# FerrisMind/candle-video

Measured on AMD Instinct MI355X. Metric: frames/sec end-to-end LTX-Video-2B 512x768x97; DiT step ms; VAE decode ms, higher is better.
Workload: dtype bf16; 1 GPU; LTX-Video-0.9.8-2B-distilled 512x768x97, 7 steps (configs.rs:223-240), untiled VAE decode; preset=0.9.8-2b-distilled, denoise_steps=7, parallelism=replicas x1 (no data-path collective)

## Files before the change

candle-video_amd/csrc/capi_ops.hip:

```cpp
#include "model_util.h"
#include "../../include/ltxhip_ops.h"

static inline int dtc(int d) { return d == 1 ? LTX_DT_BF16 : LTX_DT_F32; }

extern "C" int ltx_op_linear(const void* x, const void* w, const void* bias, void* y, int M, int N, int K, int dtype, int epi,
                             const void* resid, const float* gate, int rows_per_batch, ltx_stream stream) {
    if (!x || !w || !y) LTX_FAIL(LTX_ERR_ARG, "ltx_op_linear: null tensor");
    if (epi < 0 || epi > 3) LTX_FAIL(LTX_ERR_ARG, "ltx_op_linear: epi must be 0..3");
    if ((epi == 2 || epi == 3) && !resid) LTX_FAIL(LTX_ERR_ARG, "ltx_op_linear: residual epilogue needs resid");
    if (epi == 2 && (!gate || rows_per_batch < 1)) LTX_FAIL(LTX_ERR_ARG, "ltx_op_linear: gated epilogue needs gate");
    GemmArgs g; g.A = x; g.W = w; g.C = y; g.bias = bias; g.resid = resid; g.gate = gate;
    g.M = M; g.N = N; g.K = K; g.lda = K; g.ldc = N; g.ldr = N; g.rows_per_batch = rows_per_batch > 0 ? rows_per_batch : 1; g.gate_stride = N;
    return ltx_launch_gemm(g, dtc(dtype), epi, (hipStream_t)stream);
}

extern "C" int64_t ltx_op_ring_packed_bytes(int N, int K) { return (int64_t)ltx_ring_packed_bytes(N, K); }
extern "C" int ltx_op_ring_pack(const void* w, int N, int K, void* out, ltx_stream stream) { return ltx_pack_ring_weights(w, N, K, out, (hipStream_t)stream); }
extern "C" int ltx_op_linear_packed(const void* x, const void* w, const void* w_packed, const void* bias, void* y, int M, int N, int K, int epi,
                                    const void* resid, const float* gate, int rows_per_batch, ltx_stream stream) {
    if (!x || !w || !w_packed || !y) LTX_FAIL(LTX_ERR_ARG, "ltx_op_linear_packed: null tensor");
    if (epi < 0 || epi > 3) LTX_FAIL(LTX_ERR_ARG, "ltx_op_linear_packed: epi must be 0..3");
    if ((epi == 2 || epi == 3) && !resid) LTX_FAIL(LTX_ERR_ARG, "ltx_op_linear_packed: residual epilogue needs resid");
    if (epi == 2 && (!gate || rows_per_batch < 1)) LTX_FAIL(LTX_ERR_ARG, "ltx_op_linear_packed: gated epilogue needs gate");
    GemmArgs g; g.A = x; g.W = w; g.Wp = w_packed; g.C = y; g.bias = bias; g.resid = resid; g.gate = gate;
// ... 24 lines not shown
    return g;
}
GemmArgs fold_in_args(const void* x, const void* w, void* y, const float* rs_sq, int rs_n, int rs_D, float eps, const float* cvec, int cvec_stride,
                      int M, int N, int K, int rows_per_batch) {
    GemmArgs g; g.A = x; g.W = w; g.C = y; g.M = M; g.N = N; g.K = K; g.lda = K; g.ldc = N;
    g.rows_per_batch = rows_per_batch > 0 ? rows_per_batch : 1;
    g.rs_sq = rs_sq; g.rs_n = rs_n; g.rs_D = rs_D; g.rs_eps = eps; g.cvec = cvec; g.cvec_stride = cvec_stride;
    return g;
}
}

extern "C" int ltx_op_linear_fold_out(const void* x, const void* w, const void* bias, void* y, void* y2, float* rowsq, const float* scale2, int scale2_stride,
                                      int M, int N, int K, int epi, const void* resid, const float* gate, int rows_per_batch, ltx_stream stream) {
    if (!x || !w || !y || !y2 || !rowsq || !scale2 || !resid) LTX_FAIL(LTX_ERR_ARG, "ltx_op_linear_fold_out: null tensor");
    if (epi != 2 && epi != 3) LTX_FAIL(LTX_ERR_ARG, "ltx_op_linear_fold_out: epi must be 2 or 3 (the second output rides on the residual epilogues)");
    if (epi == 2 && !gate) LTX_FAIL(LTX_ERR_ARG, "ltx_op_linear_fold_out: gated epilogue needs gate");
    const GemmArgs g = fold_out_args(x, w, bias, y, y2, rowsq, scale2, scale2_stride, M, N, K, resid, gate, rows_per_batch);
    if (!ltx_gemm_fold_ok(g, epi)) LTX_FAIL(LTX_ERR_ARG, "ltx_op_linear_fold_out: not a call the norm fold serves (ltx_op_linear_fold_ok)");
    return ltx_launch_gemm(g, LTX_DT_BF16, epi, (hipStream_t)stream);
}

extern "C" int ltx_op_linear_fold_in(const void* x, const void* w, void* y, const float* rs_sq, int rs_n, int rs_D, float eps, const float* cvec, int cvec_stride,
                                     int M, int N, int K, int epi, int rows_per_batch, ltx_stream stream) {
    if (!x || !w || !y || !rs_sq || !cvec) LTX_FAIL(LTX_ERR_ARG, "ltx_op_linear_fold_in: null tensor");
    if (epi != 0 && epi != 1) LTX_FAIL(LTX_ERR_ARG, "ltx_op_linear_fold_in: epi must be 0 or 1 (the row scale rides on the bias / GELU epilogues)");
    const GemmArgs g = fold_in_args(x, w, y, rs_sq, rs_n, rs_D, eps, cvec, cvec_stride, M, N, K, rows_per_batch);
    if (!ltx_gemm_fold_ok(g, epi)) LTX_FAIL(LTX_ERR_ARG, "ltx_op_linear_fold_in: not a call the norm fold serves (ltx_op_linear_fold_ok)");
    return ltx_launch_gemm(g, LTX_DT_BF16, epi, (hipStream_t)stream);
}

extern "C" int ltx_op_linear_fold_ok(int M, int N, int K, int epi, int consumer, int rs_n, int vec_stride, int rows_per_batch) {
    if (M < 1 || N < 1 || K < 1) return 0;
    void* const p = reinterpret_cast<void*>((uintptr_t)4096); float* const f = reinterpret_cast<float*>(p);
    if (consumer) return ltx_gemm_fold_ok(fold_in_args(p, p, p, f, rs_n, K, 1e-6f, f, vec_stride, M, N, K, rows_per_batch), epi) ? 1 : 0;
    return ltx_gemm_fold_ok(fold_out_args(p, p, p, p, p, f, f, vec_stride, M, N, K, p, f, rows_per_batch), epi) ? 1 : 0;
}

extern "C" int ltx_op_shift_gemv(const void* w, const void* bias, const float* shift, int shift_stride, int B, int N, int K, float* cvec, int cvec_stride, ltx_stream stream) {
    return ltx_launch_shift_gemv(w, bias, shift, shift_stride, B, N, K, cvec, cvec_stride, (hipStream_t)stream);
}
extern "C" int ltx_op_mod_scale(const void* h, const float* scale, int scale_stride, void* y, int B, int64_t rows_per_batch, int D, int dtype, ltx_stream stream) {
    if (!h || !scale || !y || B < 1 || rows_per_batch < 1 || D < 1) LTX_FAIL(LTX_ERR_ARG, "ltx_op_mod_scale: bad argument");
    return ltx_launch_mod_scale(h, scale, scale_stride, y, B, rows_per_batch, D, dtc(dtype), (hipStream_t)stream);
}
extern "C" int ltx_op_scale_cols(const void* w, const float* scale, void* out, int64_t N, int K, int dtype, ltx_stream stream) {
    if (!w || !scale || !out || N < 1 || K < 1) LTX_FAIL(LTX_ERR_ARG, "ltx_op_scale_cols: bad argument");
    return ltx_launch_scale_cols(w, scale, out, N, K, dtc(dtype), (hipStream_t)stream);
}

extern "C" int ltx_op_linear_segmented(const void* x, const void* w, const void* bias, void* y, int M, int N, int K, int seg_width,
                                       int dtype, ltx_stream stream) {
    if (!x || !w || !y) LTX_FAIL(LTX_ERR_ARG, "ltx_op_linear_segmented: null tensor");
    if (seg_width <= 0 || (seg_width & (seg_width - 1)) || N % seg_width) LTX_FAIL(LTX_ERR_ARG, "ltx_op_linear_segmented: seg_width must be a power of two dividing N");
    GemmArgs g; g.A = x; g.W = w; g.C = y; g.bias = bias;
    g.M = M; g.N = N; g.K = K; g.lda = K; g.ldc = seg_width;
    g.c_seg_shift = __builtin_ctz((unsigned)seg_width); g.c_seg_stride = (int64_t)M * seg_width;
    return ltx_launch_gemm(g, dtc(dtype), EPI_BIAS, (hipStream_t)stream);
}

extern "C" int ltx_op_rownorm(const void* x, void* y, int64_t rows, int D, int kind, float eps, const void* weight,
                              const float* scale, const float* shift, int64_t rows_per_batch, int mod_stride, int act,
                              int dtype, ltx_stream stream) {
    if (!x || !y) LTX_FAIL(LTX_ERR_ARG, "ltx_op_rownorm: null tensor");
    RowNormArgs a; a.x = x; a.y = y; a.rows = rows; a.D = D; a.ldx = D; a.ldy = D; a.kind = kind; a.eps = eps; a.weight = weight;
    a.scale = scale; a.shift = shift; a.rows_per_batch = rows_per_batch > 0 ? rows_per_batch : 1; a.mod_stride = mod_stride; a.act = act;
    return ltx_launch_rownorm(a, dtc(dtype), (hipStream_t)stream);
}

extern "C" int ltx_attention_fallback_counts(unsigned long long counts[2], int reset) {
    if (!counts) LTX_FAIL(LTX_ERR_ARG, "ltx_attention_fallback_counts: null output");
    LTX_TRY(ltx_q64_fallback_read(&counts[0], reset));
    return ltx_q128_fallback_read(&counts[1], reset);
}

extern "C" int ltx_op_linear_split_factor(int M, int N, int K) {
    GemmArgs g; g.M = M; g.N = N; g.K = K; g.lda = K; g.ldc = N;
    return ltx_gemm_split_factor(g);
}
extern "C" int ltx_op_linear_deferred(const void* x, const void* w, float* parts, int M, int N, int K, ltx_stream stream) {
    if (!x || !w || !parts) LTX_FAIL(LTX_ERR_ARG, "ltx_op_linear_deferred: null tensor");
    GemmArgs g; g.A = x; g.W = w; g.C = parts; g.M = M; g.N = N; g.K = K; g.lda = K; g.ldc = N; g.defer_parts = parts;
    if (!ltx_gemm_defer_ok(g, EPI_GATE_RESID)) LTX_FAIL(LTX_ERR_ARG, "ltx_op_linear_deferred: bf16 linear layers of at most 512 rows, N % 8 == 0, K % 8 == 0");
    return ltx_launch_gemm(g, LTX_DT_BF16, EPI_BIAS, (hipStream_t)stream);
}
extern "C" int ltx_op_rownorm_deferred(const float* parts, int nparts, const void* bias, const void* resid, const float* gate, int gate_stride, void* h_out,
                                       void* y, int64_t rows, int D, int kind, float eps, const float* scale, const float* shift, int64_t rows_per_batch,
                                       int mod_stride, int dtype, ltx_stream stream) {
    if (!parts || !resid || !h_out || !y) LTX_FAIL(LTX_ERR_ARG, "ltx_op_rownorm_deferred: null tensor");
    RowNormArgs a; a.x = resid; a.y = y; a.rows = rows; a.D = D; a.ldx = D; a.ldy = D; a.kind = kind; a.eps = eps;
    a.scale = scale; a.shift = shift; a.rows_per_batch = rows_per_batch > 0 ? rows_per_batch : 1; a.mod_stride = mod_stride;
    a.parts = parts; a.nparts = nparts; a.part_stride = rows * D; a.d_bias = bias; a.d_gate = gate; a.d_gate_stride = gate_stride; a.x_out = h_out;
    return ltx_launch_rownorm(a, dtc(dtype), (hipStream_t)stream);
}

extern "C" int ltx_op_rownorm_presum(const void* x, void* y, int64_t rows, int D, float eps, const void* weight,
                                     const float* scale, const float* shift, int64_t rows_per_batch, int mod_stride, int act,
                                     const float* presum, int presum_n, int dtype, ltx_stream stream) {
    if (!x || !y || !presum) LTX_FAIL(LTX_ERR_ARG, "ltx_op_rownorm_presum: null tensor");
    RowNormArgs a; a.x = x; a.y = y; a.rows = rows; a.D = D; a.ldx = D; a.ldy = D; a.kind = 0; a.eps = eps; a.weight = weight;
    a.scale = scale; a.shift = shift; a.rows_per_batch = rows_per_batch > 0 ? rows_per_batch : 1; a.mod_stride = mod_stride; a.act = act;
    a.presum = presum; a.presum_n = presum_n;
    return ltx_launch_rownorm(a, dtc(dtype), (hipStream_t)stream);
}

extern "C" int ltx_op_timestep_embedding(const float* timesteps_host, int n, int vae_flavour, float multiplier, int dtype, void* out, ltx_stream stream) {
    if (!timesteps_host || !out) LTX_FAIL(LTX_ERR_ARG, "ltx_op_timestep_embedding: null argument");
    if (n < 1 || n > 8) LTX_FAIL(LTX_ERR_ARG, "ltx_op_timestep_embedding: batch must be 1..8");
    float tab[128]; ltx_sinusoid_table(vae_flavour, tab);
    float* dtab = nullptr;
    HIP_TRY(hipMalloc((void**)&dtab, sizeof(tab)));
    int rc = LTX_OK;
    if (hipMemcpy(dtab, tab, sizeof(tab), hipMemcpyHostToDevice) != hipSuccess) rc = LTX_ERR_HIP;
    if (rc == LTX_OK) {
        TimeVec tv; tv.n = n;
        for (int i = 0; i < n; ++i) tv.t[i] = timesteps_host[i];
        rc = ltx_launch_sinusoid(out, dtc(dtype), tv, dtab, 128, dtc(dtype) == LTX_DT_BF16, multiplier, (hipStream_t)stream);
        if (rc == LTX_OK && hipStreamSynchronize((hipStream_t)stream) != hipSuccess) rc = LTX_ERR_HIP;
    }
    (void)hipFree(dtab);
    return rc;
}

extern "C" int ltx_op_qknorm_rope(void* x, int64_t rows, int D, int ld, const void* weight, float eps,
                                  const float* cos, const float* sin, int dtype, ltx_stream stream) {
    if (!x || !weight) LTX_FAIL(LTX_ERR_ARG, "ltx_op_qknorm_rope: null tensor");
    QkNormRopeArgs a; a.x = x; a.rows = rows; a.D = D; a.ld = ld; a.nseg = 1; a.w0 = weight; a.eps = eps; a.cos = cos; a.sin = sin;
    return ltx_launch_qknorm_rope(a, dtc(dtype), (hipStream_t)stream);
}

extern "C" int ltx_op_rope_table(float* cos, float* sin, const float* coords, int B, int F, int H, int W, int D,
                                 const float* rope_scale_host, ltx_stream stream) {
    if (!cos || !sin) LTX_FAIL(LTX_ERR_ARG, "ltx_op_rope_table: null tensor");
    int steps = D / 6; if (steps < 1) steps = 1;
    std::vector<float> fr(steps);
    const float theta_ln = (float)std::log(10000.0);
    for (int i = 0; i < steps; ++i) {
        float lin = steps <= 1 ? 0.0f : (float)i * (float)(1.0 / (double)(steps - 1));
        fr[i] = (float)std::exp((double)(lin * theta_ln)) * (float)(M_PI / 2.0);
    }
    float* dfr = nullptr;
    HIP_TRY(hipMalloc((void**)&dfr, sizeof(float) * steps));
    HIP_TRY(hipMemcpy(dfr, fr.data(), sizeof(float) * steps, hipMemcpyHostToDevice));
    RopeTableArgs r; r.cos = cos; r.sin = sin; r.freqs = dfr; r.B = B; r.D = D;
    if (coords) { r.use_coords = 1; r.coords = coords; r.F = 1; r.H = 1; r.W = F * H * W;
                  r.gscale[0] = (float)(1.0 / 20.0); r.gscale[1] = (float)(1.0 / 2048.0); r.gscale[2] = (float)(1.0 / 2048.0); }
    else { r.F = F; r.H = H; r.W = W;
           if (rope_scale_host) { r.gscale[0] = (float)((double)rope_scale_host[0] / 20.0); r.gscale[1] = (float)((double)rope_scale_host[1] / 2048.0); r.gscale[2] = (float)((double)rope_scale_host[2] / 2048.0); } }
    int rc = ltx_launch_rope_table(r, (hipStream_t)stream);
    hipError_t e = hipStreamSynchronize((hipStream_t)stream);
    (void)hipFree(dfr);
    if (rc != LTX_OK) return rc;
    if (e != hipSuccess) { ltx_set_error(hipGetErrorString(e)); return LTX_ERR_HIP; }
    return LTX_OK;
}

extern "C" int ltx_op_attention(const void* q, const void* k, const void* v, void* o, int B, int Sq, int Sk, int heads, int hd,
                                int ldq, int ldk, int ldv, int ldo, float scale, const float* key_bias, int dtype, ltx_stream stream) {
    if (!q || !k || !v || !o) LTX_FAIL(LTX_ERR_ARG, "ltx_op_attention: null tensor");
    AttnArgs a; a.q = q; a.k = k; a.v = v; a.o = o; a.ldq = ldq; a.ldk = ldk; a.ldv = ldv; a.ldo = ldo;
    a.B = B; a.Sq = Sq; a.Sk = Sk; a.heads = heads; a.hd = hd; a.scale = scale; a.bias = key_bias;
    return ltx_launch_attention(a, dtc(dtype), (hipStream_t)stream);
}

extern "C" int ltx_op_attention_rowsq(const void* q, const void* k, const void* v, void* o, int B, int Sq, int Sk, int heads, int hd,
                                      int ldq, int ldk, int ldv, int ldo, float scale, const float* key_bias,
                                      const float* q_rowsq, int q_rowsq_n, int q_rowsq_D, float q_rowsq_eps, ltx_stream stream) {
    if (!q || !k || !v || !o || !q_rowsq) LTX_FAIL(LTX_ERR_ARG, "ltx_op_attention_rowsq: null tensor");
    AttnArgs a; a.q = q; a.k = k; a.v = v; a.o = o; a.ldq = ldq; a.ldk = ldk; a.ldv = ldv; a.ldo = ldo;
    a.B = B; a.Sq = Sq; a.Sk = Sk; a.heads = heads; a.hd = hd; a.scale = scale; a.bias = key_bias;
    a.q_rowsq = q_rowsq; a.q_rowsq_n = q_rowsq_n; a.q_rowsq_D = q_rowsq_D; a.q_rowsq_eps = q_rowsq_eps;
    return ltx_launch_attention(a, LTX_DT_BF16, (hipStream_t)stream);
}

extern "C" int ltx_op_attention_compact(const void* q, const void* k, const void* v, void* o, int B, int Sq, int Sk, int heads, int hd,
                                        int ldq, int ldk, int ldv, int ldo, float scale, const float* key_bias,
                                        const float* q_rowsq, int q_rowsq_n, int q_rowsq_D, float q_rowsq_eps, int* counts_out, ltx_stream stream) {
    if (!q || !k || !v || !o || !key_bias) LTX_FAIL(LTX_ERR_ARG, "ltx_op_attention_compact: null tensor");
    if (!ltx_attention_cross64_ok(hd, Sk) || B < 1 || ldk != heads * hd || ldv != heads * hd) LTX_FAIL(LTX_ERR_ARG, "ltx_op_attention_compact: bf16, head_dim 64, at most 128 keys, dense k / v rows");
    hipStream_t s = (hipStream_t)stream;
    const int D = heads * hd;
    void *kc = nullptr, *vc = nullptr, *bc = nullptr, *idx = nullptr, *cnt = nullptr;
    auto free_all = [&]() { for (void* p : {kc, vc, bc, idx, cnt}) if (p) (void)hipFree(p); };
    const size_t rows = (size_t)B * Sk;
    if (hipMalloc(&kc, rows * D * 2) != hipSuccess || hipMalloc(&vc, rows * D * 2) != hipSuccess || hipMalloc(&bc, rows * 4) != hipSuccess ||
        hipMalloc(&idx, rows * 4) != hipSuccess || hipMalloc(&cnt, (size_t)B * 4) != hipSuccess) { free_all(); LTX_FAIL(LTX_ERR_HIP, "hipMalloc"); }
    int rc = ltx_launch_key_compact(key_bias, B, Sk, (int*)idx, (int*)cnt, (float*)bc, s);
    if (rc == LTX_OK) rc = ltx_launch_gather_rows(k, kc, (const int*)idx, (const int*)cnt, 1, B, Sk, D * 2, s);
    if (rc == LTX_OK) rc = ltx_launch_gather_rows(v, vc, (const int*)idx, (const int*)cnt, 1, B, Sk, D * 2, s);
    if (rc == LTX_OK) {
        AttnArgs a; a.q = q; a.k = kc; a.v = vc; a.o = o; a.ldq = ldq; a.ldk = D; a.ldv = D; a.ldo = ldo;
        a.B = B; a.Sq = Sq; a.Sk = Sk; a.heads = heads; a.hd = hd; a.scale = scale; a.bias = (const float*)bc; a.k_count = (const int*)cnt;
        if (q_rowsq) { a.q_rowsq = q_rowsq; a.q_rowsq_n = q_rowsq_n; a.q_rowsq_D = q_rowsq_D; a.q_rowsq_eps = q_rowsq_eps; }
        rc = ltx_launch_attention(a, LTX_DT_BF16, s);
    }
    if (rc == LTX_OK && counts_out && hipMemcpyAsync(counts_out, cnt, (size_t)B * 4, hipMemcpyDeviceToDevice, s) != hipSuccess) rc = LTX_ERR_HIP;
    const hipError_t e = hipStreamSynchronize(s);
    free_all();
    if (rc != LTX_OK) return rc;
    if (e != hipSuccess) { ltx_set_error(hipGetErrorString(e)); return LTX_ERR_HIP; }
    return LTX_OK;
}

extern "C" int ltx_op_attention_prescaled(const void* q, const void* k, const void* v, void* o, int B, int Sq, int Sk, int heads, int hd,
                                          int ldq, int ldk, int ldv, int ldo, ltx_stream stream) {
    if (!q || !k || !v || !o) LTX_FAIL(LTX_ERR_ARG, "ltx_op_attention_prescaled: null tensor");
    AttnArgs a; a.q = q; a.k = k; a.v = v; a.o = o; a.ldq = ldq; a.ldk = ldk; a.ldv = ldv; a.ldo = ldo;
    a.B = B; a.Sq = Sq; a.Sk = Sk; a.heads = heads; a.hd = hd; a.scale = 1.0f; a.q_prescaled = 1;
    return ltx_launch_attention(a, LTX_DT_BF16, (hipStream_t)stream);
}

namespace {
int conv_common(const void* x, const void* w, const void* bias, int wdtype, void* y, const void* resid,
                int B, int T, int H, int W, int Cin, int Cout, int causal, int dtype, int epi, int mode, int post, hipStream_t s) {
    if (!x || !w || !bias || !y) LTX_FAIL(LTX_ERR_ARG, "conv: null tensor");
    const int dt = dtc(dtype); const size_t esz = ltx_dt_size(dt);
    void *pw = nullptr, *pb = nullptr;
    HIP_TRY(hipMalloc(&pw, (size_t)Cout * Cin * 27 * esz));
    if (hipMalloc(&pb, (size_t)Cout * esz + 16) != hipSuccess) { (void)hipFree(pw); LTX_FAIL(LTX_ERR_HIP, "hipMalloc"); }
    const int Cf = Cout / 8;
    int rc = ltx_pack_conv(w, dtc(wdtype), pw, dt, Cout, Cin, 27, mode, Cf, s);
    if (rc == LTX_OK) rc = ltx_pack_conv(bias, dtc(wdtype), pb, dt, Cout, 1, 1, mode, Cf, s);
    if (rc == LTX_OK) {
        GemmArgs g; g.A = x; g.W = pw; g.C = y; g.bias = pb; g.resid = resid;
        g.M = B * T * H * W; g.N = Cout; g.K = Cin; g.ldc = Cout; g.ldr = Cout;
        g.conv = 1; g.B = B; g.T = T; g.H = H; g.Wd = W; g.Cin = Cin; g.ntaps = 27; g.kh = 3; g.kw = 3; g.pad_t = causal ? 2 : 1; g.post = post;
        if (epi == EPI_D2S) { g.Cf = Cf; g.Cr = Cin / 8; g.To = 2 * T - 1; g.Ho = 2 * H; g.Wo = 2 * W; }
        rc = ltx_launch_gemm(g, dt, epi, s);
    }
    hipError_t e = hipStreamSynchronize(s);
    (void)hipFree(pw); (void)hipFree(pb);
    if (rc != LTX_OK) return rc;
    if (e != hipSuccess) { ltx_set_error(hipGetErrorString(e)); return LTX_ERR_HIP; }
    return LTX_OK;
}
}

extern "C" int ltx_op_conv3d(const void* x, const void* w, const void* bias, int wdtype, void* y, const void* resid,
                             int B, int T, int H, int W, int Cin, int Cout, int causal, int dtype, ltx_stream stream) {
    return conv_common(x, w, bias, wdtype, y, resid, B, T, H, W, Cin, Cout, causal, dtype, resid ? EPI_RESID : EPI_BIAS, LTX_PERM_NONE, 0, (hipStream_t)stream);
}
extern "C" int ltx_op_upsample3d(const void* x, const void* w, const void* bias, int wdtype, void* y,
                                 int B, int T, int H, int W, int Cin, int Cout, int causal, int residual, int dtype, ltx_stream stream) {
    if (Cout % 8 != 0 || Cin % 8 != 0) LTX_FAIL(LTX_ERR_ARG, "upsample3d: channels must be multiples of 8");
    return conv_common(x, w, bias, wdtype, y, residual ? x : nullptr, B, T, H, W, Cin, Cout, causal, dtype, EPI_D2S, LTX_PERM_D2S, 0, (hipStream_t)stream);
}
extern "C" int ltx_op_conv_out_unpatchify(const void* x, const void* w, const void* bias, int wdtype, float* y,
                                          int B, int T, int H, int W, int Cin, int Cout, int causal, int postprocess, int dtype, ltx_stream stream) {
    if (Cout % 16 != 0) LTX_FAIL(LTX_ERR_ARG, "conv_out: Cout must be a multiple of 16 (patch 4x4)");
    return conv_common(x, w, bias, wdtype, y, nullptr, B, T, H, W, Cin, Cout, causal, dtype, EPI_UNPATCH, LTX_PERM_UNPATCH, postprocess, (hipStream_t)stream);
}

extern "C" int ltx_op_blend(const float* a, float* b, int BC, int at, int ah, int aw, int bt, int bh, int bw, int dim, int blend_extent, ltx_stream stream) {
    if (!a || !b || dim < 2 || dim > 4) LTX_FAIL(LTX_ERR_ARG, "ltx_op_blend: bad argument");
    const int ad[3] = {at, ah, aw}, bd[3] = {bt, bh, bw};
    BlendArgs ba; ba.a = a; ba.b = b; ba.dst = b; ba.BC = BC;
    ba.at = at; ba.ah = ah; ba.aw = aw; ba.a_len = ad[dim - 2];
    ba.bt = ba.dt = bt; ba.bh = ba.dh = bh; ba.bw = ba.dw = bw;
    ba.dim = dim; ba.blend = std::min(blend_extent, std::min(ad[dim - 2], bd[dim - 2]));
    ba.et = std::min(at, bt); ba.eh = std::min(ah, bh); ba.ew = std::min(aw, bw);
    if (dim == 2) ba.et = ba.blend; else if (dim == 3) ba.eh = ba.blend; else ba.ew = ba.blend;
    return ltx_launch_blend(ba, (hipStream_t)stream);
}

const char* ltx_gemm_plan_name(int M, int N, int K, int conv, int ntaps, int T, int H, int W);
extern "C" int ltx_op_gemm_plan(int M, int N, int K, int conv, int ntaps, int T, int H, int W, char* name, int cap) {
    if (!name || cap < 1) LTX_FAIL(LTX_ERR_ARG, "ltx_op_gemm_plan: bad argument");
    const char* n = ltx_gemm_plan_name(M, N, K, conv, ntaps, T, H, W);
    snprintf(name, (size_t)cap, "%s", n);
    return LTX_OK;
}

extern "C" int ltx_op_gemm_route(int M, int N, int K, int conv, int ntaps, int B, int T, int H, int W, int epi, int dtype, int flags, char* name, int cap) {
    if (!name || cap < 1 || M < 1 || N < 1 || K < 1 || epi < EPI_BIAS || epi > EPI_S2D) LTX_FAIL(LTX_ERR_ARG, "ltx_op_gemm_route: bad argument");
    if (conv && (ntaps < 1 || B < 1 || T < 1 || H < 1 || W < 1 || (int64_t)B * T * H * W != M)) LTX_FAIL(LTX_ERR_ARG, "ltx_op_gemm_route: conv calls need M = B T H W");
    void* const p = reinterpret_cast<void*>((uintptr_t)4096); float* const f = reinterpret_cast<float*>(p);
    const bool res = epi == EPI_GATE_RESID || epi == EPI_RESID;
    GemmArgs g;
    if (flags & LTX_ROUTE_FOLD_IN) g = fold_in_args(p, p, p, f, 16, K, 1e-6f, f, N, M, N, K, M);
    else if (flags & LTX_ROUTE_FOLD_OUT) g = fold_out_args(p, p, p, p, p, f, f, N, M, N, K, p, epi == EPI_GATE_RESID ? f : nullptr, M);
    else {
        g.A = p; g.W = p; g.C = p; g.M = M; g.N = N; g.K = K; g.lda = K; g.ldc = N; g.ldr = N; g.rows_per_batch = M; g.gate_stride = N;
        if (flags & LTX_ROUTE_DEFER) g.defer_parts = f;
        else { g.bias = p; if (res || epi == EPI_S2D) g.resid = p; if (epi == EPI_GATE_RESID) g.gate = f; }
    }
    if (conv) {
        g.conv = 1; g.B = B; g.T = T; g.H = H; g.Wd = W; g.Cin = K; g.ntaps = ntaps; g.kh = g.kw = ntaps == 27 ? 3 : 1; g.pad_t = 2;
        if (epi == EPI_D2S) { g.Cf = N / 8; g.Cr = K / 8; g.To = 2 * T - 1; g.Ho = 2 * H; g.Wo = 2 * W; }
        if (epi == EPI_S2D) { g.s2_st = g.s2_sh = g.s2_sw = 2; g.To = (T + 1) / 2; g.Ho = H / 2; g.Wo = W / 2; }
        if (flags & LTX_ROUTE_PN) { g.pn_on = 1; g.pn_eps = 1e-6f; g.pn_act = 1; }
    }
    GemmRoute r;
    LTX_TRY(ltx_gemm_route(g, dtc(dtype), epi, nullptr, false, &r));
    if (const char* why = ltx_gemm_route_refusal(g, r)) LTX_FAIL(LTX_ERR_ARG, why);
    snprintf(name, (size_t)cap, "%s", ltx_gemm_route_name(r));
    return LTX_OK;
}

extern "C" int ltx_op_dit_plan(int heads, int head_dim, int model_dtype, int io_dtype, int B, int S, int K, int G, int skip_mask, int64_t* out) {
    if (!out || heads < 1 || head_dim < 1 || B < 1 || B > 8 || S < 1 || K < 1 || G < 1 || S % G != 0) LTX_FAIL(LTX_ERR_ARG, "ltx_op_dit_plan: bad argument");
    ltx_dit_config c; ltx_dit_config_default(&c);
    c.num_attention_heads = heads; c.attention_head_dim = head_dim; c.cross_attention_dim = heads * head_dim;
    const DitPlan p = ltx_dit_plan(c, dtc(model_dtype), dtc(io_dtype), B, S, K, G, skip_mask != 0);
    const int64_t v[LTX_DIT_PLAN_FIELDS] = {p.M, p.MK, p.NB, p.Sg, p.seg, p.ldqkv, p.fold_q2, p.presum, p.nfold, p.defer_ff2, p.ff2_parts, p.dense_qkv, p.fold_q};
    for (int i = 0; i < LTX_DIT_PLAN_FIELDS; ++i) out[i] = v[i];
    return LTX_OK;
}
// ... 1 lines not shown
```

candle-video_amd/csrc/dit.hip:

```cpp
#include <cstring>
#include <deque>
#include "model_util.h"
#include "options.h"
#include "../../include/ltxhip_cond.h"
#include "lora.h"

struct DitBlock {
    LinearW qkv1, o1, q2, kv2, o2, ff1, ff2;
    void *nq1 = nullptr, *nk1 = nullptr, *nq2 = nullptr, *nk2 = nullptr;
};

struct DitCtx {
    const void* enc = nullptr; const float* mask = nullptr;
    int B = 0, K = 0, iodt = 0; bool valid = false;
    bool fold_q2 = false;
    DevBuf kv, bias;
    bool compact = false;
    DevBuf kvc, biasc, kidx, kcount;
    void release() { kv.release(); bias.release(); kvc.release(); biasc.release(); kidx.release(); kcount.release(); valid = false; }
};

struct DitTimeEntry {
    float t[8] = {0}; int B = 0; hipStream_t stream = nullptr; bool valid = false; uint64_t used = 0;
    DevBuf ada, adaf;
    DevBuf cfold; bool cfold_valid = false;
    void release() { ada.release(); adaf.release(); cfold.release(); valid = cfold_valid = false; }
};
struct DitWfold {
    float t = 0.f; hipStream_t stream = nullptr; bool valid = false; uint64_t used = 0; DevBuf w;
    void release() { w.release(); valid = false; }
};
constexpr int kDitTimeEntries = 64;
struct DitGroupEntry {
    std::vector<float> t; int B = 0, G = 0; hipStream_t stream = nullptr; bool valid = false; uint64_t used = 0;
    DevBuf ada, adaf, cfold; bool cfold_valid = false;
    void release() { ada.release(); adaf.release(); cfold.release(); valid = cfold_valid = false; }
};
constexpr int kDitGroupEntries = 8;

struct ltx_dit {
    ltx_dit_config cfg{};
    int dtype = LTX_DT_BF16;
    int device = 0;
    int D = 0;
    LinearW proj_in, te1, te2, te_lin, cap1, cap2, proj_out;
    void* sst_final = nullptr;
    void* sst_blocks = nullptr;
    std::vector<DitBlock> blocks;
    float* rope_freqs = nullptr;
    float* inv_freq = nullptr;
    std::vector<int> skip_blocks;
    std::deque<DitCtx> ctxs;
    bool ctx_mode = false;
    std::deque<DitTimeEntry> tcache; uint64_t tclock = 0;
    std::deque<DitWfold> wcache;
    std::deque<DitGroupEntry> gcache;
    bool wfold_off = false;
    struct { bool valid = false; const float* coords = nullptr; float rs[3] = {0, 0, 0}; bool has_rs = false; int B = 0, S = 0, F = 0, H = 0, W = 0; hipStream_t stream = nullptr; } rope_key;
    void invalidate_weight_derived() {
        for (auto& e : wcache) e.valid = false;
        for (auto& e : ctxs) e.valid = false;
        for (auto& e : tcache) e.cfold_valid = false;
        for (auto& e : gcache) e.cfold_valid = false;
    }
    void release_scaled_weights() { for (auto& e : wcache) e.release(); }
    void release_caches() { auto all = [](auto& c) { for (auto& e : c) e.release(); c.clear(); }; all(ctxs); all(tcache); all(wcache); all(gcache); }
    std::vector<void*> owned;
    struct LoraSlots { void* base[7] = {nullptr}; void* merged[7] = {nullptr}; };
    std::vector<LoraSlots> lora_w;
    int n_adapters = 0;
    DevBuf xin, encin, h, n, qkv, attn, ff, c1, encp, kv2, tproj, e1, emb, embs, temb, ada, adaf, cosb, sinb, bias, orig, orig_hsq, outT, rsq, hsq, parts;
    void free_all() {
        for (void* p : owned) if (p) (void)hipFree(p);
        owned.clear();
        for (auto& ls : lora_w) for (void*& p : ls.merged) if (p) { (void)hipFree(p); p = nullptr; }
        lora_w.clear();
        DevBuf* bs[] = {&xin, &encin, &h, &n, &qkv, &attn, &ff, &c1, &encp, &kv2, &tproj, &e1, &emb, &embs, &temb, &ada, &adaf, &cosb, &sinb, &bias, &orig, &orig_hsq, &outT, &rsq, &hsq, &parts};
        for (DevBuf* b : bs) b->release();
        release_caches();
    }
};

namespace {

int own_linear(ltx_dit* m, const WeightMap& wm, const std::string& prefix, int in, int out, LinearW* l) {
    LTX_TRY(ltx_load_linear(wm, prefix, in, out, m->dtype, l));
    m->owned.push_back(l->w); if (l->b) m->owned.push_back(l->b);
    return LTX_OK;
}
int own_tensor(ltx_dit* m, const WeightMap& wm, const std::string& name, int64_t numel, void** out) {
    LTX_TRY(ltx_load_tensor(wm, name, numel, m->dtype, out));
    m->owned.push_back(*out);
    return LTX_OK;
}
int own_fused(ltx_dit* m, const WeightMap& wm, const std::vector<std::string>& prefixes, int in, int out_each, LinearW* l) {
    const int n = (int)prefixes.size();
    const size_t esz = ltx_dt_size(m->dtype);
    l->in = in; l->out = out_each * n;
    HIP_TRY(hipMalloc(&l->w, (size_t)l->out * in * esz)); m->owned.push_back(l->w);
    bool has_bias = wm.find(prefixes[0] + ".bias") != nullptr;
    if (has_bias) { HIP_TRY(hipMalloc(&l->b, (size_t)l->out * esz)); m->owned.push_back(l->b); }
    for (int i = 0; i < n; ++i) {
        const ltx_weight* w = wm.find(prefixes[i] + ".weight");
        if (!w) LTX_FAIL(LTX_ERR_MISSING_WEIGHT, "missing weight '" + prefixes[i] + ".weight'");
        LTX_TRY(ltx_upload_cast(w, (char*)l->w + (size_t)i * out_each * in * esz, m->dtype, (int64_t)out_each * in, prefixes[i] + ".weight"));
        if (has_bias) {
            const ltx_weight* b = wm.find(prefixes[i] + ".bias");
            if (!b) LTX_FAIL(LTX_ERR_MISSING_WEIGHT, "missing weight '" + prefixes[i] + ".bias'");
            LTX_TRY(ltx_upload_cast(b, (char*)l->b + (size_t)i * out_each * esz, m->dtype, out_each, prefixes[i] + ".bias"));
        }
    }
    return LTX_OK;
}

int build(ltx_dit* m, const ltx_weight* weights, size_t n_weights) {
    const ltx_dit_config& c = m->cfg;
    const int D = m->D, L = c.num_layers;
    WeightMap wm(weights, n_weights);
    LTX_TRY(own_linear(m, wm, "proj_in", c.in_channels, D, &m->proj_in));
    LTX_TRY(own_tensor(m, wm, "scale_shift_table", 2 * (int64_t)D, &m->sst_final));
    LTX_TRY(own_linear(m, wm, "time_embed.emb.timestep_embedder.linear_1", 256, D, &m->te1));
    LTX_TRY(own_linear(m, wm, "time_embed.emb.timestep_embedder.linear_2", D, D, &m->te2));
    LTX_TRY(own_linear(m, wm, "time_embed.linear", D, 6 * D, &m->te_lin));
    LTX_TRY(own_linear(m, wm, "caption_projection.linear_1", c.caption_channels, D, &m->cap1));
    LTX_TRY(own_linear(m, wm, "caption_projection.linear_2", D, D, &m->cap2));
    LTX_TRY(own_linear(m, wm, "proj_out", D, c.out_channels, &m->proj_out));
    const size_t esz = ltx_dt_size(m->dtype);
    HIP_TRY(hipMalloc(&m->sst_blocks, (size_t)L * 6 * D * esz)); m->owned.push_back(m->sst_blocks);
    m->blocks.resize(L);
    for (int i = 0; i < L; ++i) {
        const std::string p = "transformer_blocks." + std::to_string(i) + ".";
        DitBlock& b = m->blocks[i];
        LTX_TRY(own_fused(m, wm, {p + "attn1.to_q", p + "attn1.to_k", p + "attn1.to_v"}, D, D, &b.qkv1));
        LTX_TRY(own_linear(m, wm, p + "attn1.to_out.0", D, D, &b.o1));
        LTX_TRY(own_tensor(m, wm, p + "attn1.norm_q.weight", D, &b.nq1));
        LTX_TRY(own_tensor(m, wm, p + "attn1.norm_k.weight", D, &b.nk1));
        LTX_TRY(own_linear(m, wm, p + "attn2.to_q", D, D, &b.q2));
        LTX_TRY(own_fused(m, wm, {p + "attn2.to_k", p + "attn2.to_v"}, c.cross_attention_dim, D, &b.kv2));
        LTX_TRY(own_linear(m, wm, p + "attn2.to_out.0", D, D, &b.o2));
        LTX_TRY(own_tensor(m, wm, p + "attn2.norm_q.weight", D, &b.nq2));
        LTX_TRY(own_tensor(m, wm, p + "attn2.norm_k.weight", D, &b.nk2));
        LTX_TRY(own_linear(m, wm, p + "ff.net.0.proj", D, 4 * D, &b.ff1));
        LTX_TRY(own_linear(m, wm, p + "ff.net.2", 4 * D, D, &b.ff2));
        const ltx_weight* t = wm.find(p + "scale_shift_table");
        if (!t) LTX_FAIL(LTX_ERR_MISSING_WEIGHT, "missing weight '" + p + "scale_shift_table'");
        LTX_TRY(ltx_upload_cast(t, (char*)m->sst_blocks + (size_t)i * 6 * D * esz, m->dtype, 6 * (int64_t)D, p + "scale_shift_table"));
    }
    {
        int steps = D / 6; if (steps < 1) steps = 1;
        std::vector<float> fr(steps);
        const float theta_ln = (float)std::log(10000.0);
        for (int i = 0; i < steps; ++i) {
            float lin = steps <= 1 ? 0.0f : (float)i * (float)(1.0 / (double)(steps - 1));
            float x = lin * theta_ln;
            float e = (float)std::exp((double)x);
            fr[i] = e * (float)(M_PI / 2.0);
        }
        HIP_TRY(hipMalloc((void**)&m->rope_freqs, sizeof(float) * steps)); m->owned.push_back(m->rope_freqs);
        HIP_TRY(hipMemcpy(m->rope_freqs, fr.data(), sizeof(float) * steps, hipMemcpyHostToDevice));
        std::vector<float> inv(128);
        ltx_sinusoid_table(0, inv.data());
        HIP_TRY(hipMalloc((void**)&m->inv_freq, sizeof(float) * 128)); m->owned.push_back(m->inv_freq);
        HIP_TRY(hipMemcpy(m->inv_freq, inv.data(), sizeof(float) * 128, hipMemcpyHostToDevice));
    }
    return LTX_OK;
}

LinearW* dit_slot(DitBlock& b, int slot) {
    LinearW* const ws[7] = {&b.qkv1, &b.o1, &b.q2, &b.kv2, &b.o2, &b.ff1, &b.ff2};
    return ws[slot];
}
constexpr int kLoraSlot[kLoraLinears] = {0, 0, 0, 1, 2, 3, 3, 4, 5, 6}, kLoraPart[kLoraLinears] = {0, 1, 2, 0, 0, 0, 1, 0, 0, 0};
constexpr int kSlotParts[7] = {3, 1, 1, 2, 1, 1, 1}, kSlotFirst[7] = {0, 3, 4, 5, 7, 8, 9};

}

extern "C" int ltx_dit_create(const ltx_dit_config* cfg, const ltx_weight* weights, size_t n_weights,
                              ltx_dtype model_dtype, int device, ltx_dit** out) {
    if (!cfg || !weights || !out) LTX_FAIL(LTX_ERR_ARG, "ltx_dit_create: null argument");
    *out = nullptr;
    const int hd = cfg->attention_head_dim;
    if (hd != 16 && hd != 32 && hd != 64 && hd != 128) LTX_FAIL(LTX_ERR_UNSUPPORTED, "attention_head_dim must be 16/32/64/128");
    const int D = cfg->num_attention_heads * hd;
    if (D % 8 != 0 || cfg->in_channels % 8 != 0 || cfg->out_channels % 8 != 0 || cfg->caption_channels % 8 != 0 || cfg->cross_attention_dim % 8 != 0)
        LTX_FAIL(LTX_ERR_UNSUPPORTED, "channel dims must be multiples of 8");
    if (cfg->cross_attention_dim != D) LTX_FAIL(LTX_ERR_UNSUPPORTED, "cross_attention_dim must equal inner_dim (caption projection output feeds attn2)");
    if (cfg->num_layers < 1) LTX_FAIL(LTX_ERR_ARG, "num_layers must be >= 1");
    HIP_TRY(hipSetDevice(device));
    ltx_dit* m = new ltx_dit();
    m->cfg = *cfg; m->dtype = model_dtype == LTX_BF16 ? LTX_DT_BF16 : LTX_DT_F32; m->device = device; m->D = D;
    int rc = build(m, weights, n_weights);
    if (rc == LTX_OK && cfg->attention_head_dim == 128 && m->dtype == LTX_DT_BF16) rc = ltx_attention_q128_prepare();
    if (rc != LTX_OK) { m->free_all(); delete m; return rc; }
    m->lora_w.resize(m->blocks.size());
    for (size_t l = 0; l < m->blocks.size(); ++l)
        for (int slot = 0; slot < 7; ++slot) m->lora_w[l].base[slot] = dit_slot(m->blocks[l], slot)->w;
    *out = m;
    return LTX_OK;
}

extern "C" void ltx_dit_destroy(ltx_dit* m) {
    if (!m) return;
    (void)hipSetDevice(m->device);
    (void)hipDeviceSynchronize();
    m->free_all();
    delete m;
}

extern "C" int ltx_dit_set_skip_blocks(ltx_dit* m, const int* blocks, int n) {
    if (!m || n < 0 || (n > 0 && !blocks)) LTX_FAIL(LTX_ERR_ARG, "ltx_dit_set_skip_blocks: bad argument");
    m->skip_blocks.assign(blocks, blocks + n);
    return LTX_OK;
}

extern "C" int ltx_dit_get_config(const ltx_dit* m, ltx_dit_config* out) {
    if (!m || !out) LTX_FAIL(LTX_ERR_ARG, "ltx_dit_get_config: null argument");
    *out = m->cfg;
    return LTX_OK;
}

namespace {
enum DitForm { kPass,
               kFold1,
               kFold2,
               kDefer };
struct DitOperands {
    void *h, *n, *qkv, *attn, *ff; float *rsq, *hsq, *parts;
    const float* ada;
    const float* ada_next;
    const float* cfold;
// ... 72 lines not shown

namespace {
template <class E, class Match>
E* cache_slot(std::deque<E>& c, size_t cap, Match match, bool* hit) {
    E *found = nullptr, *lru = nullptr;
    for (auto& e : c) if (e.valid && match(e)) found = &e;
    if ((*hit = found != nullptr)) return found;
    for (auto& e : c) if (!e.valid) return &e;
    if (c.size() < cap) { c.emplace_back(); return &c.back(); }
    for (auto& e : c) if (!lru || e.used < lru->used) lru = &e;
    return lru;
}
struct DitTables { const float *ada = nullptr, *adaf = nullptr, *cfold = nullptr; };
int time_tables(ltx_dit* m, const DitPlan& p, const float* vals, int nv, hipStream_t s, DitTables* t) {
    const int D = p.D, L = m->cfg.num_layers, dt = p.dt;
    TimeVec tv; tv.n = nv; for (int i = 0; i < 8; ++i) tv.t[i] = i < nv ? vals[i] : 0.f;
    bool hit;
    DitTimeEntry* te = cache_slot(m->tcache, kDitTimeEntries, [&](const DitTimeEntry& e) { return e.B == nv && e.stream == s && !memcmp(e.t, tv.t, sizeof(float) * nv); }, &hit);
    if (!hit) {
        te->valid = false; te->cfold_valid = false;
        LTX_TRY(te->ada.ensure((size_t)L * nv * 6 * D * sizeof(float))); LTX_TRY(te->adaf.ensure((size_t)2 * nv * D * sizeof(float)));
        LTX_TRY(ltx_launch_sinusoid(m->tproj.p, dt, tv, m->inv_freq, 128, dt == LTX_DT_BF16, 1.0f, s));
        LTX_TRY(ltx_linear(m->te1, m->tproj.p, 256, m->e1.p, D, nv, dt, EPI_BIAS, s));
        LTX_TRY(ltx_launch_silu(m->e1.p, m->e1.p, (int64_t)nv * D, dt, s));
        LTX_TRY(ltx_linear(m->te2, m->e1.p, D, m->emb.p, D, nv, dt, EPI_BIAS, s));
        LTX_TRY(ltx_launch_silu(m->emb.p, m->embs.p, (int64_t)nv * D, dt, s));
        LTX_TRY(ltx_linear(m->te_lin, m->embs.p, D, m->temb.p, 6 * D, nv, dt, EPI_BIAS, s));
        LTX_TRY(ltx_launch_ada(te->ada.as<float>(), m->sst_blocks, m->temb.p, L, nv, 6 * D, dt, s));
        LTX_TRY(ltx_launch_ada(te->adaf.as<float>(), m->sst_final, m->emb.p, 2, nv, D, dt, s));
        memcpy(te->t, tv.t, sizeof(te->t)); te->B = nv; te->stream = s; te->valid = true;
    }
    te->used = ++m->tclock;
    if (p.nfold && !te->cfold_valid) {
        LTX_TRY(te->cfold.ensure((size_t)L * nv * 7 * D * sizeof(float)));
        for (int l = 0; l < L; ++l) {
            const float* ada = te->ada.as<float>() + (size_t)l * nv * 6 * D;
            float* cq = te->cfold.as<float>() + (size_t)l * nv * 7 * D;
            LTX_TRY(ltx_launch_shift_gemv(m->blocks[l].qkv1.w, m->blocks[l].qkv1.b, ada, 6 * D, nv, 3 * D, D, cq, 3 * D, s));
            LTX_TRY(ltx_launch_shift_gemv(m->blocks[l].ff1.w, m->blocks[l].ff1.b, ada + 3 * D, 6 * D, nv, 4 * D, D, cq + (size_t)nv * 3 * D, 4 * D, s));
        }
        te->cfold_valid = true;
    }
    *t = DitTables{te->ada.as<float>(), te->adaf.as<float>(), p.nfold ? te->cfold.as<float>() : nullptr};
    return LTX_OK;
}
int group_tables(ltx_dit* m, const DitPlan& p, const float* timestep, hipStream_t s, DitTables* t) {
    const int D = p.D, L = m->cfg.num_layers, NB = p.NB, B = p.B, G = NB / B;
    bool hit;
    DitGroupEntry* ge = cache_slot(m->gcache, kDitGroupEntries, [&](const DitGroupEntry& e) { return e.B == B && e.G == G && e.stream == s && !memcmp(e.t.data(), timestep, sizeof(float) * NB); }, &hit);
    if (!hit && ge->valid && ge->stream != s) HIP_TRY(hipStreamSynchronize(ge->stream));
    if (!hit || (p.nfold && !ge->cfold_valid)) {
        ge->valid = false; ge->cfold_valid = false;
        std::vector<float> distinct; std::vector<int> idx((size_t)NB);
        for (int i = 0; i < NB; ++i) {
            size_t j = 0;
            while (j < distinct.size() && memcmp(&distinct[j], &timestep[i], sizeof(float)) != 0) ++j;
            if (j == distinct.size()) distinct.push_back(timestep[i]);
            idx[i] = (int)j;
        }
        LTX_TRY(ge->ada.ensure((size_t)L * NB * 6 * D * sizeof(float))); LTX_TRY(ge->adaf.ensure((size_t)2 * NB * D * sizeof(float)));
        if (p.nfold) LTX_TRY(ge->cfold.ensure((size_t)L * NB * 7 * D * sizeof(float)));
        const int nd = (int)distinct.size();
        for (int c0 = 0; c0 < nd; c0 += 8) {
            const int nc = nd - c0 < 8 ? nd - c0 : 8;
            DitTables te;
            LTX_TRY(time_tables(m, p, distinct.data() + c0, nc, s, &te));
            const int* gi = idx.data();
            LTX_TRY(ltx_launch_group_gather(ge->ada.as<float>(), (int64_t)NB * 6 * D, te.ada, (int64_t)nc * 6 * D, gi, c0, nc, L, NB, 6 * D, s));
            LTX_TRY(ltx_launch_group_gather(ge->adaf.as<float>(), (int64_t)NB * D, te.adaf, (int64_t)nc * D, gi, c0, nc, 2, NB, D, s));
            if (p.nfold) {
                LTX_TRY(ltx_launch_group_gather(ge->cfold.as<float>(), (int64_t)NB * 7 * D, te.cfold, (int64_t)nc * 7 * D, gi, c0, nc, L, NB, 3 * D, s));
                LTX_TRY(ltx_launch_group_gather(ge->cfold.as<float>() + (size_t)NB * 3 * D, (int64_t)NB * 7 * D, te.cfold + (size_t)nc * 3 * D, (int64_t)nc * 7 * D, gi, c0, nc, L, NB, 4 * D, s));
            }
        }
        ge->t.assign(timestep, timestep + NB); ge->B = B; ge->G = G; ge->stream = s; ge->valid = true; ge->cfold_valid = p.nfold;
    }
    ge->used = ++m->tclock;
    *t = DitTables{ge->ada.as<float>(), ge->adaf.as<float>(), p.nfold ? ge->cfold.as<float>() : nullptr};
    return LTX_OK;
}
int give_up_scaled_weights(ltx_dit* m, hipStream_t s) {
    m->wfold_off = true;
    HIP_TRY(hipStreamSynchronize(s));
    m->release_scaled_weights();
    return LTX_OK;
}
int scaled_weights(ltx_dit* m, const DitPlan& p, const float* timestep, const float* ada_all, hipStream_t s, const DitWfold** out) {
    *out = nullptr;
    bool wf = p.NB == p.B && p.nfold && ltx_opt().norm_fold == 2 && !m->wfold_off;
    for (int i = 1; i < p.B; ++i) wf = wf && timestep[i] == timestep[0];
    if (!wf) return LTX_OK;
    const int D = p.D, L = m->cfg.num_layers, cap = ltx_opt().norm_fold_copies > 0 ? ltx_opt().norm_fold_copies : 1;
    const size_t esz = ltx_dt_size(p.dt), per_layer = (size_t)7 * D * D * esz;
    const float t0 = timestep[0];
    bool hit;
    DitWfold* we = cache_slot(m->wcache, (size_t)cap, [&](const DitWfold& e) { return e.t == t0 && e.stream == s; }, &hit);
    if (!hit) {
        if (we->valid) {
            if (m->tclock - we->used < (uint64_t)4 * cap) return give_up_scaled_weights(m, s);
            if (we->stream != s) HIP_TRY(hipStreamSynchronize(we->stream));
            we->valid = false;
        }
        if (we->w.ensure((size_t)L * per_layer) != LTX_OK) {
            (void)hipGetLastError();
            return give_up_scaled_weights(m, s);
        }
        for (int l = 0; l < L; ++l) {
            const float* ada = ada_all + (size_t)l * p.NB * 6 * D;
            char* wl = (char*)we->w.p + (size_t)l * per_layer;
            LTX_TRY(ltx_launch_scale_cols(m->blocks[l].qkv1.w, ada + D, wl, 3 * D, D, p.dt, s));
            LTX_TRY(ltx_launch_scale_cols(m->blocks[l].ff1.w, ada + 4 * D, wl + (size_t)3 * D * D * esz, 4 * D, D, p.dt, s));
        }
        we->t = t0; we->stream = s; we->valid = true;
    }
    we->used = m->tclock;
    *out = we;
    return LTX_OK;
}
int text_context(ltx_dit* m, const DitPlan& p, const void* enc, const float* enc_mask, hipStream_t s, DitCtx** out) {
    const ltx_dit_config& c = m->cfg;
    const int D = p.D, L = c.num_layers, dt = p.dt, B = p.B, K = p.K;
    const int64_t MK = p.MK; const size_t esz = ltx_dt_size(dt);
    DitCtx* ctx = nullptr;
    for (auto& e : m->ctxs) if (e.valid && e.enc == enc && e.mask == enc_mask && e.B == B && e.K == K && e.iodt == p.iodt && e.fold_q2 == p.fold_q2) ctx = &e;
    *out = ctx;
    if (ctx) return LTX_OK;
    if (m->ctxs.size() >= 4 || !m->ctx_mode) { for (auto& e : m->ctxs) e.valid = false; }
    for (auto& e : m->ctxs) if (!e.valid) { ctx = &e; break; }
    if (!ctx) { m->ctxs.emplace_back(); ctx = &m->ctxs.back(); }
    ctx->enc = enc; ctx->mask = enc_mask; ctx->B = B; ctx->K = K; ctx->iodt = p.iodt; ctx->fold_q2 = p.fold_q2;
    LTX_TRY(ctx->kv.ensure((size_t)L * MK * 2 * D * esz)); LTX_TRY(ctx->bias.ensure(MK * sizeof(float)));
    LTX_TRY(ltx_launch_cast(enc, p.iodt, m->encin.p, dt, MK * c.caption_channels, s));
    LTX_TRY(ltx_linear(m->cap1, m->encin.p, c.caption_channels, m->c1.p, D, (int)MK, dt, EPI_GELU, s));
    LTX_TRY(ltx_linear(m->cap2, m->c1.p, D, m->encp.p, D, (int)MK, dt, EPI_BIAS, s));
    if (enc_mask) LTX_TRY(ltx_launch_mask_bias(ctx->bias.as<float>(), enc_mask, MK, s));
    for (int l = 0; l < L; ++l) {
        void* kvl = (char*)ctx->kv.p + (size_t)l * MK * 2 * D * esz;
        LTX_TRY(ltx_linear(m->blocks[l].kv2, m->encp.p, D, kvl, 2 * D, (int)MK, dt, EPI_BIAS, s));
        QkNormRopeArgs k2; k2.x = kvl; k2.rows = MK; k2.D = D; k2.ld = 2 * D; k2.nseg = 1; k2.w0 = m->blocks[l].nk2; k2.eps = 1e-5f;
        if (p.fold_q2) k2.w0b = m->blocks[l].nq2;
        LTX_TRY(ltx_launch_qknorm_rope(k2, dt, s));
    }
    ctx->compact = enc_mask && dt == LTX_DT_BF16 && ltx_attention_cross64_ok(c.attention_head_dim, K) && ltx_opt().xattn_compact;
    if (ctx->compact) {
        LTX_TRY(ctx->kvc.ensure((size_t)L * MK * 2 * D * esz)); LTX_TRY(ctx->biasc.ensure(MK * sizeof(float)));
        LTX_TRY(ctx->kidx.ensure(MK * sizeof(int))); LTX_TRY(ctx->kcount.ensure((size_t)B * sizeof(int)));
        LTX_TRY(ltx_launch_key_compact(ctx->bias.as<float>(), B, K, ctx->kidx.as<int>(), ctx->kcount.as<int>(), ctx->biasc.as<float>(), s));
        LTX_TRY(ltx_launch_gather_rows(ctx->kv.p, ctx->kvc.p, ctx->kidx.as<int>(), ctx->kcount.as<int>(), L, B, K, (int)(2 * D * esz), s));
    }
    ctx->valid = true;
    *out = ctx;
    return LTX_OK;
}
int rope_tables(ltx_dit* m, const DitPlan& p, int num_frames, int height, int width, const float* rope_scale, const float* video_coords, hipStream_t s) {
    const ltx_dit_config& c = m->cfg;
    auto& rk = m->rope_key;
    const bool same = m->ctx_mode && rk.valid && rk.coords == video_coords && rk.B == p.B && rk.S == p.S && rk.F == num_frames && rk.H == height && rk.W == width &&
                      rk.stream == s && rk.has_rs == (rope_scale != nullptr) && (!rope_scale || !memcmp(rk.rs, rope_scale, sizeof(rk.rs)));
    if (same) return LTX_OK;
    rk.valid = false;
    RopeTableArgs r;
    r.cos = m->cosb.as<float>(); r.sin = m->sinb.as<float>(); r.freqs = m->rope_freqs;
    r.B = p.B; r.D = p.D;
    if (video_coords) {
        r.use_coords = 1; r.coords = video_coords; r.F = 1; r.H = 1; r.W = p.S;
        r.gscale[0] = (float)(1.0 / 20.0); r.gscale[1] = (float)(1.0 / 2048.0); r.gscale[2] = (float)(1.0 / 2048.0);
    } else {
        r.F = num_frames; r.H = height; r.W = width;
        if (rope_scale) {
            r.gscale[0] = (float)((double)rope_scale[0] * c.patch_size_t / 20.0);
            r.gscale[1] = (float)((double)rope_scale[1] * c.patch_size / 2048.0);
            r.gscale[2] = (float)((double)rope_scale[2] * c.patch_size / 2048.0);
        }
    }
    LTX_TRY(ltx_launch_rope_table(r, s));
    rk.coords = video_coords; rk.B = p.B; rk.S = p.S; rk.F = num_frames; rk.H = height; rk.W = width; rk.stream = s;
    rk.has_rs = rope_scale != nullptr; if (rope_scale) memcpy(rk.rs, rope_scale, sizeof(rk.rs));
    rk.valid = m->ctx_mode;
    return LTX_OK;
}

struct DitCarry {
    bool hsq_valid = false;
    bool hs_valid = false;
    bool hsq_saved = false;
    bool pending = false; const float* pend_gate = nullptr; const void* pend_bias = nullptr;
    void take_pending(RowNormArgs& rn, const ltx_dit* m, const DitPlan& p) {
        if (!pending) return;
        rn.parts = m->parts.as<float>(); rn.nparts = p.ff2_parts; rn.part_stride = p.M * p.D; rn.d_bias = pend_bias; rn.d_gate = pend_gate; rn.d_gate_stride = 6 * p.D;
        rn.x_out = m->h.p; pending = false;
    }
};
struct DitLayerIn { DitTables tab; const DitWfold* we = nullptr; const DitCtx* ctx = nullptr; const float* skip_layer_mask = nullptr; };
bool block_runs(const ltx_dit* m, const float* skip_layer_mask, int B, int l) {
    for (int sb : m->skip_blocks) if (sb == l) return false;
    bool all = skip_layer_mask != nullptr;
    for (int b = 0; all && b < B; ++b) all = skip_layer_mask[(size_t)l * B + b] == 1.f;
    return !all;
}
int next_block(const ltx_dit* m, const float* skip_layer_mask, int B, int l) {
    for (int n = l + 1; n < m->cfg.num_layers; ++n) if (block_runs(m, skip_layer_mask, B, n)) return n;
    return -1;
}

int dit_block(ltx_dit* m, const DitPlan& p, int l, const DitLayerIn& in, DitCarry& st, hipStream_t s) {
    const ltx_dit_config& c = m->cfg;
    const int dt = p.dt, D = p.D, B = p.B, S = p.S, NB = p.NB, H = c.num_attention_heads, hd = c.attention_head_dim;
    const int64_t M = p.M; const size_t esz = ltx_dt_size(dt);
    const bool wf = in.we != nullptr, fold_out = p.nfold && !wf;
    const DitBlock& b = m->blocks[l];
    TimeVec mv; mv.n = B; bool any = false;
    for (int i = 0; i < 8; ++i) mv.t[i] = 0.f;
    if (in.skip_layer_mask) for (int bb = 0; bb < B; ++bb) { mv.t[bb] = in.skip_layer_mask[(size_t)l * B + bb]; any |= mv.t[bb] != 0.f; }
    if (any) {
        HIP_TRY(hipMemcpyAsync(m->orig.p, m->h.p, M * D * esz, hipMemcpyDeviceToDevice, s));
        st.hsq_saved = p.presum && st.hsq_valid;
        if (st.hsq_saved) { LTX_TRY(m->orig_hsq.ensure(M * (D / 128) * sizeof(float))); HIP_TRY(hipMemcpyAsync(m->orig_hsq.p, m->hsq.p, M * (D / 128) * sizeof(float), hipMemcpyDeviceToDevice, s)); }
    }
    const int ln = fold_out ? next_block(m, in.skip_layer_mask, B, l) : -1;
    const float* ada = in.tab.ada + (size_t)l * NB * 6 * D;
    DitOperands x{m->h.p, m->n.p, m->qkv.p, m->attn.p, m->ff.p, m->rsq.as<float>(), m->hsq.as<float>(), m->parts.as<float>(), ada,
                  ln >= 0 ? in.tab.ada + (size_t)ln * NB * 6 * D : nullptr, p.nfold ? in.tab.cfold + (size_t)l * NB * 7 * D : nullptr,
                  wf ? (const char*)in.we->w.p + (size_t)l * 7 * D * D * esz : nullptr, c.norm_eps};
    const DitForm fold_in_form = wf ? kFold2 : kFold1;
    RowNormArgs rn; rn.x = m->h.p; rn.y = m->n.p; rn.rows = M; rn.D = D; rn.ldx = D; rn.ldy = D;
    rn.kind = 0; rn.eps = c.norm_eps; rn.shift = ada; rn.scale = ada + D; rn.rows_per_batch = p.Sg; rn.mod_stride = 6 * D;
    if (p.presum && st.hsq_valid) { rn.presum = m->hsq.as<float>(); rn.presum_n = D / 128; }
    const bool fold1 = p.nfold && st.hsq_valid && (wf || st.hs_valid);
    if (!fold1) { st.take_pending(rn, m, p); LTX_TRY(ltx_launch_rownorm(rn, dt, s)); }
    st.hs_valid = false;
    rn.parts = nullptr; rn.nparts = 0; rn.x_out = nullptr; rn.d_bias = nullptr; rn.d_gate = nullptr;
    LTX_TRY(ltx_launch_gemm(gemm_qkv1(p, fold1 ? fold_in_form : kPass, b, x), dt, EPI_BIAS, s));
    const float attn_scale = 1.0f / std::sqrt((float)hd);
    QkNormRopeArgs qa; qa.x = m->qkv.p; qa.rows = M; qa.D = D; qa.ld = p.ldqkv; qa.seg_stride = p.seg; qa.nseg = 2; qa.w0 = b.nq1; qa.w1 = b.nk1;
    qa.eps = 1e-5f; qa.cos = m->cosb.as<float>(); qa.sin = m->sinb.as<float>();
    if (p.fold_q) qa.out_scale0 = attn_scale * 1.4426950408889634f;
    LTX_TRY(ltx_launch_qknorm_rope(qa, dt, s));
    AttnArgs at; at.q = m->qkv.p; at.k = (char*)m->qkv.p + (size_t)p.seg * esz; at.v = (char*)m->qkv.p + (size_t)2 * p.seg * esz; at.o = m->attn.p;
    at.ldq = at.ldk = at.ldv = p.ldqkv; at.ldo = D; at.B = B; at.Sq = S; at.Sk = S; at.heads = H; at.hd = hd; at.scale = attn_scale;
    at.q_prescaled = p.fold_q ? 1 : 0;
    LTX_TRY(ltx_launch_attention(at, dt, s));
    LTX_TRY(ltx_linear(b.o1, m->attn.p, D, m->h.p, D, (int)M, dt, EPI_GATE_RESID, s, m->h.p, D, ada + 2 * D, 6 * D, p.Sg));
    st.hsq_valid = false;
    const DitCtx* ctx = in.ctx;
    const char* kvl = (const char*)(ctx->compact ? ctx->kvc.p : ctx->kv.p) + (size_t)l * p.MK * 2 * D * esz;
    AttnArgs ax; ax.q = m->qkv.p; ax.k = kvl; ax.v = kvl + (size_t)D * esz; ax.o = m->attn.p;
    ax.ldq = D; ax.ldk = ax.ldv = 2 * D; ax.ldo = D; ax.B = B; ax.Sq = S; ax.Sk = p.K; ax.heads = H; ax.hd = hd; ax.scale = attn_scale;
    ax.bias = ctx->mask ? ctx->bias.as<float>() : nullptr;
    if (ctx->compact) { ax.bias = ctx->biasc.as<float>(); ax.k_count = ctx->kcount.as<int>(); }
    if (p.fold_q2) {
        LTX_TRY(ltx_launch_gemm(gemm_q2(p, b, x), dt, EPI_BIAS, s));
        ax.q_rowsq = m->rsq.as<float>(); ax.q_rowsq_n = D / 128; ax.q_rowsq_D = D; ax.q_rowsq_eps = 1e-5f;
    } else {
        LTX_TRY(linear_of(b.q2, gemm_q2(p, b, x), dt, EPI_BIAS, s));
        QkNormRopeArgs q2; q2.x = m->qkv.p; q2.rows = M; q2.D = D; q2.ld = D; q2.nseg = 1; q2.w0 = b.nq2; q2.eps = 1e-5f;
        LTX_TRY(ltx_launch_qknorm_rope(q2, dt, s));
    }
    LTX_TRY(ltx_launch_attention(ax, dt, s));
    if (fold_out) { LTX_TRY(ltx_launch_gemm(gemm_o2(p, kFold1, b, x), dt, EPI_RESID, s)); st.hs_valid = true; }
    else LTX_TRY(linear_of(b.o2, gemm_o2(p, kPass, b, x), dt, EPI_RESID, s));
    st.hsq_valid = p.presum;
    if (p.nfold && st.hsq_valid && (wf || st.hs_valid)) LTX_TRY(ltx_launch_gemm(gemm_ff1(p, fold_in_form, b, x), dt, EPI_GELU, s));
    else {
        rn.shift = ada + 3 * D; rn.scale = ada + 4 * D;
        rn.presum = nullptr; rn.presum_n = 0;
        if (p.presum && st.hsq_valid) { rn.presum = m->hsq.as<float>(); rn.presum_n = D / 128; }
        LTX_TRY(ltx_launch_rownorm(rn, dt, s));
        LTX_TRY(linear_of(b.ff1, gemm_ff1(p, kPass, b, x), dt, EPI_GELU, s));
    }
    st.hs_valid = false;
    if (p.defer_ff2) {
        LTX_TRY(ltx_launch_gemm(gemm_ff2(p, kDefer, b, x), dt, EPI_BIAS, s));
        st.pending = true; st.pend_gate = ada + 5 * D; st.pend_bias = b.ff2.b;
    } else if (ln >= 0) { LTX_TRY(ltx_launch_gemm(gemm_ff2(p, kFold1, b, x), dt, EPI_GATE_RESID, s)); st.hs_valid = true; }
    else LTX_TRY(linear_of(b.ff2, gemm_ff2(p, kPass, b, x), dt, EPI_GATE_RESID, s));
    st.hsq_valid = p.presum;
    if (!any) return LTX_OK;
    LTX_TRY(ltx_launch_skip_blend(m->h.p, m->orig.p, mv, S, D, dt, s));
    bool binary = true;
    for (int bb = 0; bb < B; ++bb) binary &= mv.t[bb] == 0.f || mv.t[bb] == 1.f;
    if (st.hsq_valid && st.hsq_saved && binary) {
        const size_t rowb = (size_t)S * (D / 128) * sizeof(float);
        for (int bb = 0; bb < B; ++bb)
            if (mv.t[bb] == 1.f) HIP_TRY(hipMemcpyAsync((char*)m->hsq.p + bb * rowb, (const char*)m->orig_hsq.p + bb * rowb, rowb, hipMemcpyDeviceToDevice, s));
    } else st.hsq_valid = false;
    st.hs_valid = false;
    if (fold_out && st.hsq_valid && ln >= 0) { LTX_TRY(ltx_launch_mod_scale(m->h.p, x.ada_next + D, 6 * D, m->n.p, NB, p.Sg, D, dt, s)); st.hs_valid = true; }
    return LTX_OK;
}

int dit_forward_b8(ltx_dit* m, const void* hidden, const void* enc, const float* timestep, int G,
                   const float* enc_mask, int B, int S, int K, int num_frames, int height, int width,
                   const float* rope_scale, const float* video_coords, const float* skip_layer_mask,
                   ltx_dtype io_dtype, void* out, ltx_stream stream) {
    if (B < 1 || B > 8) LTX_FAIL(LTX_ERR_ARG, "ltx_dit_forward: internal batch chunk must be 1..8");
    if (S < 1 || K < 1) LTX_FAIL(LTX_ERR_ARG, "ltx_dit_forward: empty sequence");
    if (!video_coords && (int64_t)num_frames * height * width != S)
        LTX_FAIL(LTX_ERR_ARG, "ltx_dit_forward: num_frames*height*width must equal S when video_coords is absent");
    HIP_TRY(hipSetDevice(m->device));
    if (G < 1 || S % G != 0) LTX_FAIL(LTX_ERR_ARG, "ltx_dit_forward: the modulation groups must divide the sequence");
    hipStream_t s = (hipStream_t)stream;
    const ltx_dit_config& c = m->cfg;
    const DitPlan p = ltx_dit_plan(c, m->dtype, io_dtype == LTX_BF16 ? LTX_DT_BF16 : LTX_DT_F32, B, S, K, G, skip_layer_mask != nullptr);
    const int dt = p.dt, D = p.D, L = c.num_layers;
    const int64_t M = p.M, MK = p.MK; const size_t esz = ltx_dt_size(dt);
    const size_t nte = p.NB == p.B ? (size_t)p.B : 8;
    const size_t MD = M * D * esz, KD = MK * D * esz, part = M * (D / 128) * sizeof(float), rope = M * (D / 2) * sizeof(float);
    const std::pair<DevBuf*, size_t> ws[] = {
        {&m->xin, M * c.in_channels * esz}, {&m->encin, MK * c.caption_channels * esz}, {&m->h, MD}, {&m->n, MD}, {&m->qkv, 3 * MD}, {&m->attn, MD}, {&m->ff, 4 * MD},
        {&m->c1, KD}, {&m->encp, KD}, {&m->kv2, 2 * KD}, {&m->tproj, nte * 256 * esz}, {&m->e1, nte * D * esz}, {&m->emb, nte * D * esz}, {&m->embs, nte * D * esz},
        {&m->temb, nte * 6 * D * esz}, {&m->cosb, rope}, {&m->sinb, rope}, {&m->bias, MK * sizeof(float)}, {&m->outT, M * c.out_channels * esz},
        {&m->rsq, p.fold_q2 ? part : 0}, {&m->hsq, p.presum ? part : 0}, {&m->parts, p.defer_ff2 ? (size_t)p.ff2_parts * M * D * sizeof(float) : 0}, {&m->orig, skip_layer_mask ? MD : 0}};
    for (const auto& w : ws) LTX_TRY(w.first->ensure(w.second));

    LTX_TRY(ltx_launch_cast(hidden, p.iodt, m->xin.p, dt, p.M * c.in_channels, s));
    LTX_TRY(ltx_linear(m->proj_in, m->xin.p, c.in_channels, m->h.p, D, (int)p.M, dt, EPI_BIAS, s));

    DitLayerIn in; in.skip_layer_mask = skip_layer_mask;
    LTX_TRY(G == 1 ? time_tables(m, p, timestep, B, s, &in.tab) : group_tables(m, p, timestep, s, &in.tab));
    LTX_TRY(scaled_weights(m, p, timestep, in.tab.ada, s, &in.we));
    DitCtx* ctx = nullptr;
    LTX_TRY(text_context(m, p, enc, enc_mask, s, &ctx)); in.ctx = ctx;
    LTX_TRY(rope_tables(m, p, num_frames, height, width, rope_scale, video_coords, s));

    DitCarry st;
    for (int l = 0; l < L; ++l)
        if (block_runs(m, skip_layer_mask, B, l)) LTX_TRY(dit_block(m, p, l, in, st, s));

    RowNormArgs rn; rn.x = m->h.p; rn.y = m->n.p; rn.rows = p.M; rn.D = D; rn.ldx = D; rn.ldy = D;
    rn.kind = 1; rn.eps = 1e-6f; rn.shift = in.tab.adaf; rn.scale = in.tab.adaf + (size_t)p.NB * D;
    rn.rows_per_batch = p.Sg; rn.mod_stride = D;
    st.take_pending(rn, m, p);
    LTX_TRY(ltx_launch_rownorm(rn, dt, s));
    void* dst = p.iodt == dt ? out : m->outT.p;
    LTX_TRY(ltx_linear(m->proj_out, m->n.p, D, dst, c.out_channels, (int)p.M, dt, EPI_BIAS, s));
    if (p.iodt != dt) LTX_TRY(ltx_launch_cast(m->outT.p, dt, out, p.iodt, p.M * c.out_channels, s));
    if (!m->ctx_mode) ctx->valid = false;
    return LTX_OK;
}

int dit_forward_chunks(ltx_dit* m, const void* hidden, const void* enc, const float* timestep, int F,
                       const float* enc_mask, int B, int S, int K, int num_frames, int height, int width,
                       const float* rope_scale, const float* video_coords, const float* skip_layer_mask,
                       ltx_dtype io_dtype, void* out, ltx_stream stream) {
    const size_t esz = io_dtype == LTX_BF16 ? 2 : 4;
    const int L = m->cfg.num_layers;
    std::vector<float> mask_chunk;
    float t_row[8];
    for (int b0 = 0; b0 < B; b0 += 8) {
        const int bc = B - b0 < 8 ? B - b0 : 8;
        const float* slm = skip_layer_mask;
        if (skip_layer_mask && bc != B) {
            mask_chunk.resize((size_t)L * bc);
            for (int l = 0; l < L; ++l) for (int b = 0; b < bc; ++b) mask_chunk[(size_t)l * bc + b] = skip_layer_mask[(size_t)l * B + b0 + b];
            slm = mask_chunk.data();
        }
        const float* tc = timestep + (size_t)b0 * (F ? F : 1);
        int G = 1;
        if (F) {
            bool uniform = true;
            for (int b = 0; b < bc; ++b) for (int f = 1; f < F; ++f) uniform = uniform && memcmp(&tc[(size_t)b * F + f], &tc[(size_t)b * F], sizeof(float)) == 0;
            if (uniform) { for (int b = 0; b < bc; ++b) t_row[b] = tc[(size_t)b * F]; tc = t_row; } else G = F;
        }
        LTX_TRY(dit_forward_b8(m, (const char*)hidden + (size_t)b0 * S * m->cfg.in_channels * esz, (const char*)enc + (size_t)b0 * K * m->cfg.caption_channels * esz,
                               tc, G, enc_mask ? enc_mask + (size_t)b0 * K : nullptr, bc, S, K, num_frames, height, width, rope_scale,
                               video_coords ? video_coords + (size_t)b0 * S * 3 : nullptr, slm, io_dtype,
                               (char*)out + (size_t)b0 * S * m->cfg.out_channels * esz, stream));
    }
    return LTX_OK;
}

}

extern "C" int ltx_dit_forward(ltx_dit* m, const void* hidden, const void* enc, const float* timestep,
                               const float* enc_mask, int B, int S, int K, int num_frames, int height, int width,
                               const float* rope_scale, const float* video_coords, const float* skip_layer_mask,
                               ltx_dtype io_dtype, void* out, ltx_stream stream) {
    if (!m || !hidden || !enc || !timestep || !out) LTX_FAIL(LTX_ERR_ARG, "ltx_dit_forward: null argument");
    if (B < 1) LTX_FAIL(LTX_ERR_ARG, "ltx_dit_forward: batch must be at least 1");
    return dit_forward_chunks(m, hidden, enc, timestep, 0, enc_mask, B, S, K, num_frames, height, width, rope_scale, video_coords, skip_layer_mask, io_dtype, out, stream);
}

extern "C" int ltx_dit_forward_frames(ltx_dit* m, const void* hidden, const void* enc, const float* timestep,
                                      const float* enc_mask, int B, int S, int K, int num_frames, int height, int width,
                                      const float* rope_scale, const float* video_coords, const float* skip_layer_mask,
                                      ltx_dtype io_dtype, void* out, ltx_stream stream) {
    if (!m || !hidden || !enc || !timestep || !out) LTX_FAIL(LTX_ERR_ARG, "ltx_dit_forward_frames: null argument");
    if (B < 1) LTX_FAIL(LTX_ERR_ARG, "ltx_dit_forward_frames: batch must be at least 1");
    if (num_frames < 1 || height < 1 || width < 1 || (int64_t)num_frames * height * width != S)
        LTX_FAIL(LTX_ERR_ARG, "ltx_dit_forward_frames: S must equal num_frames*height*width (tokens in pack order, with or without video_coords)");
    return dit_forward_chunks(m, hidden, enc, timestep, num_frames, enc_mask, B, S, K, num_frames, height, width, rope_scale, video_coords, skip_layer_mask, io_dtype, out, stream);
}

extern "C" int ltx_dit_context_cache(ltx_dit* m, int enable) {
    if (!m) LTX_FAIL(LTX_ERR_ARG, "ltx_dit_context_cache: null handle");
    for (auto& e : m->ctxs) e.valid = false;
    m->rope_key.valid = false;
    m->ctx_mode = enable != 0;
    return LTX_OK;
}

void ltx_dit_describe(const ltx_dit* m, ltx_dit_config* cfg, int* dtype, int* device) { *cfg = m->cfg; *dtype = m->dtype; *device = m->device; }

extern "C" int ltx_dit_adapter_count(const ltx_dit* m) { return m ? m->n_adapters : 0; }

extern "C" int ltx_dit_set_adapters(ltx_dit* m, const ltx_lora* const* loras, const float* scales, int n, ltx_stream stream) {
    if (!m) LTX_FAIL(LTX_ERR_ARG, "ltx_dit_set_adapters: null handle");
    if (n < 0 || n > kLoraMaxAdapters) LTX_FAIL(LTX_ERR_ARG, "ltx_dit_set_adapters: " + std::to_string(n) + " adapters (0..8)");
    if (n > 0 && (!loras || !scales)) LTX_FAIL(LTX_ERR_ARG, "ltx_dit_set_adapters: null adapter list or scales");
    const int L = m->cfg.num_layers;
    for (int i = 0; i < n; ++i) {
        const ltx_lora* l = loras[i];
        if (!l) LTX_FAIL(LTX_ERR_ARG, "ltx_dit_set_adapters: adapter " + std::to_string(i) + " is null");
        if (l->cfg.num_attention_heads * l->cfg.attention_head_dim != m->D || l->cfg.num_layers != L || l->cfg.cross_attention_dim != m->cfg.cross_attention_dim ||
            l->dtype != m->dtype || l->device != m->device)
            LTX_FAIL(LTX_ERR_ARG, "ltx_dit_set_adapters: adapter " + std::to_string(i) + " was built for another configuration (inner dim " +
                                  std::to_string(l->cfg.num_attention_heads * l->cfg.attention_head_dim) + ", " + std::to_string(l->cfg.num_layers) + " layers), dtype or device");
    }
    HIP_TRY(hipSetDevice(m->device));
    hipStream_t s = (hipStream_t)stream;
    const size_t esz = ltx_dt_size(m->dtype);
    std::vector<LoraMergeArgs> plan((size_t)L * kLoraLinears);
    for (int i = 0; i < n; ++i)
        for (const LoraEntry& e : loras[i]->entries) {
            LoraMergeArgs& p = plan[(size_t)e.block * kLoraLinears + e.which];
            p.At[p.n] = e.At; p.Bp[p.n] = e.Bp; p.r_pad[p.n] = e.r_pad; p.coef[p.n] = scales[i] * e.factor; ++p.n;
        }
    auto targeted = [&](int l, int slot) {
        for (int part = 0; part < kSlotParts[slot]; ++part) if (plan[(size_t)l * kLoraLinears + kSlotFirst[slot] + part].n > 0) return true;
        return false;
    };
    std::vector<void**> fresh;
    for (int l = 0; l < L; ++l)
        for (int slot = 0; slot < 7; ++slot) {
            if (!targeted(l, slot) || m->lora_w[l].merged[slot]) continue;
            const LinearW* lw = dit_slot(m->blocks[l], slot);
            void* p = nullptr;
            const hipError_t e = hipMalloc(&p, (size_t)lw->out * lw->in * esz);
            if (e != hipSuccess) {
                (void)hipGetLastError();
                for (void** q : fresh) { (void)hipFree(*q); *q = nullptr; }
                LTX_FAIL(LTX_ERR_HIP, std::string("ltx_dit_set_adapters: hipMalloc of a merged weight: ") + hipGetErrorString(e) + " (the handle is unchanged)");
            }
            m->lora_w[l].merged[slot] = p; fresh.push_back(&m->lora_w[l].merged[slot]);
        }
    m->invalidate_weight_derived();
    std::vector<void*> unused;
    int rc = LTX_OK;
    for (int l = 0; l < L; ++l)
        for (int slot = 0; slot < 7; ++slot) {
            LinearW* lw = dit_slot(m->blocks[l], slot);
            auto& ls = m->lora_w[l];
            if (!ls.merged[slot]) continue;
            lw->wp.reset(); lw->wp_tried = false;
            if (!targeted(l, slot)) { lw->w = ls.base[slot]; unused.push_back(ls.merged[slot]); ls.merged[slot] = nullptr; continue; }
            const int parts = kSlotParts[slot], rows = lw->out / parts;
            for (int part = 0; part < parts && rc == LTX_OK; ++part) {
                const size_t off = (size_t)part * rows * lw->in * esz;
                LoraMergeArgs a = plan[(size_t)l * kLoraLinears + kSlotFirst[slot] + part];
                if (a.n > 0) {
                    a.w0 = (const char*)ls.base[slot] + off; a.out = (char*)ls.merged[slot] + off; a.N = rows; a.K = lw->in;
                    rc = ltx_launch_lora_merge(a, m->dtype, s);
                } else if (hipMemcpyAsync((char*)ls.merged[slot] + off, (const char*)ls.base[slot] + off, (size_t)rows * lw->in * esz, hipMemcpyDeviceToDevice, s) != hipSuccess) {
                    ltx_set_error("ltx_dit_set_adapters: hipMemcpyAsync"); rc = LTX_ERR_HIP;
// ... 23 lines not shown
```

candle-video_amd/csrc/kernels.h:

```cpp
#pragma once
#include <hip/hip_runtime.h>
#include <hip/hip_ext.h>
#include <stdint.h>

enum { LTX_DT_F32 = 0, LTX_DT_BF16 = 1 };
static inline size_t ltx_dt_size(int dt) { return dt == LTX_DT_BF16 ? 2 : 4; }

enum { LTX_PROF_GEMM = 0, LTX_PROF_CONV = 1, LTX_PROF_ATTN_SELF = 2, LTX_PROF_ATTN_CROSS = 3, LTX_PROF_ROWNORM = 4, LTX_PROF_NKINDS = 5 };
bool ltx_prof_begin(int kind, double work, hipStream_t s, void** token);
void ltx_prof_end(void* token, hipStream_t s);
enum { LTX_PROFK_GEMM128 = 0, LTX_PROFK_GEMM_BIG = 1, LTX_PROFK_GEMM_P8 = 2, LTX_PROFK_CONV_HALO = 3, LTX_PROFK_GEMM_ASM = 4, LTX_PROFK_GEMM_ASM16 = 5, LTX_PROFK_GEMM_RING = 6, LTX_PROFK_N = 7 };
void ltx_prof_kernel(int which);
bool ltx_prof_kernel_events(hipEvent_t* a, hipEvent_t* b);
#define LTX_LAUNCH_TIMED(kernel, grid, block, shmem, stream, ...) do {                                           \
        hipEvent_t _pa = nullptr, _pb = nullptr;                                                                   \
        if (ltx_prof_kernel_events(&_pa, &_pb)) hipExtLaunchKernelGGL(kernel, grid, block, shmem, stream, _pa, _pb, 0, __VA_ARGS__); \
        else hipLaunchKernelGGL(kernel, grid, block, shmem, stream, __VA_ARGS__);                                  \
    } while (0)

enum { EPI_BIAS = 0, EPI_GELU = 1, EPI_GATE_RESID = 2, EPI_RESID = 3, EPI_D2S = 4, EPI_UNPATCH = 5, EPI_S2D = 6 };

struct GemmArgs {
    const void* A = nullptr;
    const void* W = nullptr;
    void* C = nullptr;
    const void* bias = nullptr;
    const void* resid = nullptr;
    const float* gate = nullptr;
    int M = 0, N = 0, K = 0;
    int lda = 0, ldc = 0, ldr = 0;
    int rows_per_batch = 1, gate_stride = 0;
    int conv = 0;
    int B = 1, T = 1, H = 1, Wd = 1, Cin = 0;
    int ntaps = 1, kh = 1, kw = 1, pad_t = 0;
    int Cf = 0, Cr = 0, To = 0, Ho = 0, Wo = 0, post = 0;
    int d2s_sp = 0;
    int s2_st = 1, s2_sh = 1, s2_sw = 1, s2_group = 1;
    int c_seg_shift = 0; int64_t c_seg_stride = 0;
    float* rowsq = nullptr;
    void* C2 = nullptr; const float* scale2 = nullptr; int scale2_stride = 0;
    const float* rs_sq = nullptr; int rs_n = 0, rs_D = 0; float rs_eps = 0.f; const float* cvec = nullptr; int cvec_stride = 0;
    const void* Wp = nullptr;
    int xcd_remap = 0;
    int group_m = 0;
    int wide_epi = 0;
    int pn_on = 0; float pn_eps = 0.f; int pn_act = 0; int pn_mod_stride = 0;
    const float* pn_scale = nullptr; const float* pn_shift = nullptr;
    int sk_full = 0, sk_sf = 1, sk_plain = 0;
    float* defer_parts = nullptr;
    float* sk_ws = nullptr;
    unsigned* sk_cnt = nullptr;
};
int ltx_launch_gemm(const GemmArgs& g, int dtype, int epi, hipStream_t s);
enum PlanFamily { kPlanBig, kPlanP8, kPlanHalo, kPlanAsm16, kPlanAsm16Conv, kPlanRing };
struct GemmPlan { int fam = -1, idx = 0; bool ok() const { return fam >= 0; } };
enum { LTX_ROUTE_GEMM128 = 0, LTX_ROUTE_ASM32 = 1, LTX_ROUTE_PLAN = 2 };
struct GemmRoute { int kind = LTX_ROUTE_GEMM128; GemmPlan plan; };
int ltx_gemm_route_kind(const GemmArgs& g, int dtype, int epi);
int ltx_gemm_route(const GemmArgs& g, int dtype, int epi, hipStream_t s, bool measure, GemmRoute* r);
const char* ltx_gemm_route_name(const GemmRoute& r);
const char* ltx_gemm_route_refusal(const GemmArgs& g, const GemmRoute& r);
int ltx_launch_gemm_plan(const GemmArgs& g, int epi, GemmPlan p, hipStream_t s);
int ltx_launch_rowsq(const void* x, int dtype, int64_t rows, int N, int ld, float* out, hipStream_t s);
void ltx_gemm_rowsq_done();
bool ltx_gemm_big_eligible(const GemmArgs& g, int dtype);
int ltx_gemm_split_factor(const GemmArgs& g);
bool ltx_gemm_defer_ok(const GemmArgs& g, int epi);
bool ltx_gemm_asm_eligible(const GemmArgs& g, int dtype, int epi);
int ltx_launch_gemm_asm(const GemmArgs& g, int epi, hipStream_t s);
bool ltx_gemm_fold_ok(const GemmArgs& g, int epi);
int ltx_launch_shift_gemv(const void* W, const void* bias, const float* shift, int shift_stride, int B, int N, int K, float* cvec, int cvec_stride, hipStream_t s);
bool ltx_gemm_asm16_fits(const GemmArgs& g, int epi);
int ltx_launch_gemm_asm16(const GemmArgs& g, int epi, int tile, hipStream_t s);
bool ltx_gemm_asm16_conv_fits(const GemmArgs& g, int epi);
int ltx_launch_gemm_asm16_conv(const GemmArgs& g, int epi, hipStream_t s);
int ltx_gemm_asm_pick_tile(int M, int N);
const char* ltx_gemm_asm_tile_name(int i);
int ltx_gemm_big_pick_tile(int M, int N);
int ltx_launch_gemm_p8(const GemmArgs& g, int epi, int bn, hipStream_t s);
bool ltx_gemm_p8_fits(const GemmArgs& g);
bool ltx_gemm_ring_fits(const GemmArgs& g, int epi);
bool ltx_gemm_ring_tile_fits(const GemmArgs& g, int epi, int tile);
int ltx_launch_gemm_ring(const GemmArgs& g, int epi, int tile, hipStream_t s);
int ltx_gemm_ring_tiles();
int ltx_gemm_ring_tile_bm(int i);
int ltx_gemm_ring_tile_bn(int i);
int ltx_gemm_ring_pick_tile(const GemmArgs& g);
int ltx_gemm_split_workspace(GemmArgs* g, int tiles, int bm, int bn, hipStream_t s);
size_t ltx_ring_packed_bytes(int N, int K);
int ltx_pack_ring_weights(const void* W, int N, int K, void* out, hipStream_t s);
bool ltx_gemm_big_fits(const GemmArgs& g);
bool ltx_conv_halo_eligible(const GemmArgs& g, int epi, int bn);
int ltx_launch_conv_halo(const GemmArgs& g, int epi, int bn, hipStream_t s);

struct RowNormArgs {
    const void* x = nullptr; void* y = nullptr;
    int64_t rows = 0; int D = 0; int ldx = 0, ldy = 0;
    int kind = 0;
    float eps = 1e-6f;
    const void* weight = nullptr;
    const float* scale = nullptr;
    const float* shift = nullptr;
    int64_t rows_per_batch = 1; int mod_stride = 0;
    int act = 0;
    const float* presum = nullptr; int presum_n = 0;
    const float* parts = nullptr; int nparts = 0; int64_t part_stride = 0;
    const void* d_bias = nullptr; const float* d_gate = nullptr; int d_gate_stride = 0; void* x_out = nullptr;
};
int ltx_launch_rownorm(const RowNormArgs& a, int dtype, hipStream_t s);

struct QkNormRopeArgs {
    void* x = nullptr;
    int64_t rows = 0; int D = 0; int ld = 0; int nseg = 1;
    int64_t seg_stride = 0;
    const void* w0 = nullptr; const void* w1 = nullptr;
    const void* w0b = nullptr;
    float eps = 1e-5f;
    const float* cos = nullptr; const float* sin = nullptr;
    float out_scale0 = 1.f;
};
int ltx_launch_qknorm_rope(const QkNormRopeArgs& a, int dtype, hipStream_t s);

struct RopeTableArgs {
    float* cos = nullptr; float* sin = nullptr;
    const float* coords = nullptr;
    const float* freqs = nullptr;
    int B = 1, F = 1, H = 1, W = 1, D = 0;
    int use_coords = 0;
    float gscale[3] = {1.f, 1.f, 1.f};
};
int ltx_launch_rope_table(const RopeTableArgs& a, hipStream_t s);

struct AttnArgs {
    const void* q = nullptr; const void* k = nullptr; const void* v = nullptr; void* o = nullptr;
    int ldq = 0, ldk = 0, ldv = 0, ldo = 0;
    int B = 1, Sq = 0, Sk = 0, heads = 0, hd = 0;
    float scale = 1.f;
    const float* bias = nullptr;
    const float* bias2d = nullptr;
    int q_prescaled = 0;
    int xcd_heads = 0;
    int wide_o = 0;
    const float* q_rowsq = nullptr; int q_rowsq_n = 0, q_rowsq_D = 0; float q_rowsq_eps = 0.f;
    const int* k_count = nullptr;
    const int* gate_flag = nullptr; int gate_ticket = 0;
};
bool ltx_attention_q128_fits(const AttnArgs& a);
int ltx_launch_attention_q128(const AttnArgs& a, hipStream_t s, int** flag_out, int* ticket_out);
int ltx_q64_fallback_read(unsigned long long* out, int reset);
int ltx_q128_fallback_read(unsigned long long* out, int reset);
int ltx_attention_q128_prepare();
int ltx_launch_attention(const AttnArgs& a, int dtype, hipStream_t s);
int ltx_launch_attention_q64(const AttnArgs& a, hipStream_t s);
bool ltx_attention_q64_fits(const AttnArgs& a);
bool ltx_attention_prescale_ok(int hd);
bool ltx_attention_cross64_ok(int hd, int Sk);
bool ltx_attention_rowsq_ok(int hd, int Sk, int D);

constexpr int LTX_MAX_BATCH = 16;
struct TimeVec { float t[LTX_MAX_BATCH]; int n; };
int ltx_launch_gguf_dequant(const void* blocks_dev, int ggml_type, int64_t numel, void* dst, int dst_dtype, hipStream_t s);
int ltx_launch_sinusoid(void* out, int dtype, const TimeVec& tv, const float* tab, int half, int round_t, float tmul, hipStream_t s);
int ltx_launch_silu(const void* x, void* y, int64_t n, int dtype, hipStream_t s);
int ltx_launch_noise_inject(const void* x, void* y, const float* noise, const void* scale, const void* resid, int64_t rows, int C, int64_t HW, int dtype, hipStream_t s);
int ltx_launch_cast(const void* x, int xdt, void* y, int ydt, int64_t n, hipStream_t s);
int ltx_launch_ada(float* out, const void* tables, const void* temb, int nl, int B, int width, int dtype, hipStream_t s);
int ltx_launch_mask_bias(float* out, const float* mask, int64_t n, hipStream_t s);
int ltx_launch_key_compact(const float* bias, int B, int K, int* idx, int* count, float* bias_c, hipStream_t s);
int ltx_launch_gather_rows(const void* src, void* dst, const int* idx, const int* count, int nl, int B, int K, int row_bytes, hipStream_t s);
int ltx_launch_skip_blend(void* h, const void* orig, const TimeVec& m, int64_t rows_per_batch, int D, int dtype, hipStream_t s);
int ltx_launch_scale_cols(const void* W, const float* scale, void* out, int64_t N, int K, int dtype, hipStream_t s);
int ltx_launch_mod_scale(const void* h, const float* scale, int scale_stride, void* y, int B, int64_t rows_per_batch, int D, int dtype, hipStream_t s);

struct GroupIdx { int v[128]; };
int ltx_launch_group_gather(float* dst, int64_t dst_stride, const float* src, int64_t src_stride, const int* idx_host, int c0, int nc, int nl, int ngroups, int width, hipStream_t s);

struct GuidanceArgs {
    const void* text = nullptr; const void* uncond = nullptr; const void* pert = nullptr;
    int pred_dtype = LTX_DT_F32;
    float* latents = nullptr;
    float* noise_out = nullptr;
    int B = 1; int64_t n_per_batch = 0;
    float guidance_scale = 1.f, guidance_rescale = 0.f, stg_scale = 0.f, dt = 0.f;
    double* stats = nullptr;
    const float* step_noise = nullptr;
    float sigma = 0.f, sigma_next = 0.f;
    const unsigned char* hold = nullptr; int num_frames = 1; int64_t frame_elems = 0;
};
int ltx_launch_guidance_step(const GuidanceArgs& a, hipStream_t s);
int ltx_launch_guidance_step_held(const GuidanceArgs& a, hipStream_t s);
int ltx_launch_cond_apply(float* latents, const float* cond, int Fc, const unsigned char* hold_dev, int B, int F, int64_t frame_elems, hipStream_t s);

int ltx_launch_denorm_mix(const float* lat, const float* mean, const float* std_, float inv_sf, const float* noise,
                          const TimeVec& nscale, void* out, int dtype, int B, int64_t S, int C, hipStream_t s);
int ltx_launch_ncthw_to_cl(const void* x, int xdt, void* y, int ydt, int B, int C, int64_t S, hipStream_t s);
struct BlendArgs {
    const float* a = nullptr; const float* b = nullptr; float* dst = nullptr;
    int BC = 1;
    int at = 1, ah = 1, aw = 1;
    int a_len = 1;
    int bt = 1, bh = 1, bw = 1;
    int dt = 1, dh = 1, dw = 1;
    int ot = 0, oh = 0, ow = 0;
    int et = 1, eh = 1, ew = 1;
    int dim = 3, blend = 0;
    float inv_blend = 0.f;
};
int ltx_launch_blend(const BlendArgs& a, hipStream_t s);
int ltx_launch_copy_window(const float* src, int t, int h, int w, float* dst, int T, int H, int W, int BC,
                           int st, int sh, int sw, int ot, int oh, int ow, hipStream_t s);
int ltx_launch_postprocess(float* x, int64_t n, hipStream_t s);
```

candle-video_amd/csrc/options.cpp:

```cpp
#include "options.h"
#include <atomic>
#include <cstdio>
#include <cstdlib>
#include <cstring>
#include <map>
#include <mutex>
#include <string>
#include "errors.h"

namespace {
std::mutex g_mu;
LtxOptions g_opt;
std::atomic<bool> g_loaded{false};
std::map<std::string, int> g_exp;

struct ListBit { const char* name; unsigned bit; };
const ListBit kFam[] = {{"asm16", LTX_FAM_ASM16}, {"ring", LTX_FAM_RING}, {"p8", LTX_FAM_P8}, {"halo", LTX_FAM_HALO}, {"halo_out", LTX_FAM_HALO_OUT}, {"big", LTX_FAM_BIG}};
const ListBit kAttn[] = {{"q64", LTX_ATTN_Q64}, {"q128", LTX_ATTN_Q128}, {"cross", LTX_ATTN_CROSS}, {"pipe", LTX_ATTN_PIPE}};

template <size_t N> bool parse_list(const char* v, const ListBit (&tab)[N], unsigned* out) {
    unsigned bits = 0;
    std::string s(v ? v : "");
    size_t p = 0;
    while (p < s.size()) {
        size_t q = s.find('+', p); if (q == std::string::npos) q = s.size();
        const std::string item = s.substr(p, q - p);
        bool ok = item.empty();
        for (const auto& t : tab) if (item == t.name) { bits |= t.bit; ok = true; }
        if (!ok) return false;
        p = q + 1;
    }
    *out = bits;
    return true;
}

struct IntField { const char* name; int LtxOptions::*field; };
const IntField kInts[] = {
    {"gemm_tune", &LtxOptions::gemm_tune}, {"gemm_wide_epi", &LtxOptions::gemm_wide_epi}, {"gemm_trace", &LtxOptions::gemm_trace},
    {"attn_q64_big", &LtxOptions::attn_q64_big}, {"vae_tile_batch", &LtxOptions::vae_tile_batch}, {"prof_kernel_events", &LtxOptions::prof_kernel_events}, {"ff2_defer", &LtxOptions::ff2_defer},
    {"gemm_splitk", &LtxOptions::gemm_splitk}, {"q2_fold", &LtxOptions::q2_fold}, {"norm_presum", &LtxOptions::norm_presum}, {"norm_lean", &LtxOptions::norm_lean},
    {"xattn_compact", &LtxOptions::xattn_compact}, {"dense_qkv", &LtxOptions::dense_qkv}, {"vae_fuse_norm", &LtxOptions::vae_fuse_norm}, {"t5_attn_mfma", &LtxOptions::t5_attn_mfma}, {"guidance_batch", &LtxOptions::guidance_batch}, {"norm_fold", &LtxOptions::norm_fold}, {"norm_fold_copies", &LtxOptions::norm_fold_copies}, {"attn_q64_stream", &LtxOptions::attn_q64_stream},
};

bool set_one(LtxOptions& o, const std::string& key, const char* value) {
    static const LtxOptions dflt;
    for (const auto& f : kInts) if (key == f.name) {
        if (!value) { o.*(f.field) = dflt.*(f.field); return true; }
        char* end = nullptr; const long v = strtol(value, &end, 10);
        if (end == value || *end) return false;
        o.*(f.field) = (int)v; return true;
    }
    if (key == "gemm_plan") {
        if (!value) { o.gemm_plan[0] = 0; return true; }
        if (strlen(value) >= sizeof(o.gemm_plan)) return false;
        strcpy(o.gemm_plan, value); return true;
    }
    if (key == "gemm_off") return value ? parse_list(value, kFam, &o.gemm_off) : (o.gemm_off = 0, true);
    if (key == "attn_off") return value ? parse_list(value, kAttn, &o.attn_off) : (o.attn_off = 0, true);
    if (key.rfind("x_", 0) == 0) {
        if (!value) { g_exp.erase(key); return true; }
        char* end = nullptr; const long v = strtol(value, &end, 10);
        if (end == value || *end) return false;
        g_exp[key] = (int)v; return true;
    }
    return false;
}

bool parse_string(LtxOptions& o, const char* text, std::string* bad) {
    std::string s(text ? text : "");
    size_t p = 0;
    while (p < s.size()) {
        size_t q = s.find(',', p); if (q == std::string::npos) q = s.size();
        const std::string item = s.substr(p, q - p);
        p = q + 1;
        if (item.empty()) continue;
        const size_t eq = item.find('=');
        if (eq == std::string::npos || !set_one(o, item.substr(0, eq), item.c_str() + eq + 1)) { if (bad) *bad = item; return false; }
    }
    return true;
}

void load_locked() {
    g_opt = LtxOptions(); g_exp.clear();
    std::string bad;
    if (!parse_string(g_opt, getenv("LTX_OPTIONS"), &bad))
        fprintf(stderr, "[ltx] LTX_OPTIONS: entry '%s' not understood (see include/ltxhip.h); it and what follows it are ignored\n", bad.c_str());
    g_loaded.store(true, std::memory_order_release);
}
}

const LtxOptions& ltx_opt() {
    if (!g_loaded.load(std::memory_order_acquire)) { std::lock_guard<std::mutex> lock(g_mu); if (!g_loaded.load(std::memory_order_relaxed)) load_locked(); }
    return g_opt;
}

int ltx_exp_lookup(const char* name, int dflt) {
    (void)ltx_opt();
    std::lock_guard<std::mutex> lock(g_mu);
    auto it = g_exp.find(std::string("x_") + name);
    return it == g_exp.end() ? dflt : it->second;
}

extern "C" int ltx_set_option(const char* key, const char* value) {
    if (!key) LTX_FAIL(LTX_ERR_ARG, "ltx_set_option: null key");
    (void)ltx_opt();
    std::lock_guard<std::mutex> lock(g_mu);
    if (!set_one(g_opt, key, value)) LTX_FAIL(LTX_ERR_ARG, std::string("ltx_set_option: unknown option or bad value: ") + key + "=" + (value ? value : "(default)"));
    return LTX_OK;
}

extern "C" int ltx_get_option(const char* key, char* out, int n) {
    if (!key || !out || n < 2) LTX_FAIL(LTX_ERR_ARG, "ltx_get_option: null key / buffer");
    (void)ltx_opt();
    std::lock_guard<std::mutex> lock(g_mu);
    const std::string k(key);
    std::string v; bool found = false;
    for (const auto& f : kInts) if (k == f.name) { v = std::to_string(g_opt.*(f.field)); found = true; }
    auto list = [&](unsigned bits, const ListBit* tab, size_t cnt) { for (size_t i = 0; i < cnt; ++i) if (bits & tab[i].bit) { if (!v.empty()) v += "+"; v += tab[i].name; } found = true; };
    if (k == "gemm_plan") { v = g_opt.gemm_plan; found = true; }
    if (k == "gemm_off") list(g_opt.gemm_off, kFam, sizeof(kFam) / sizeof(kFam[0]));
    if (k == "attn_off") list(g_opt.attn_off, kAttn, sizeof(kAttn) / sizeof(kAttn[0]));
    if (k.rfind("x_", 0) == 0) { auto it = g_exp.find(k); if (it == g_exp.end()) LTX_FAIL(LTX_ERR_ARG, "ltx_get_option: experiment knob not set: " + k); v = std::to_string(it->second); found = true; }
    if (!found) LTX_FAIL(LTX_ERR_ARG, "ltx_get_option: unknown option: " + k);
    if ((int)v.size() + 1 > n) LTX_FAIL(LTX_ERR_ARG, "ltx_get_option: buffer too small");
    memcpy(out, v.c_str(), v.size() + 1);
    return LTX_OK;
}

extern "C" int ltx_reset_options(void) {
    std::lock_guard<std::mutex> lock(g_mu);
    load_locked();
    return LTX_OK;
}

extern "C" int ltx_has_experiments(void) {
#ifdef LTX_EXPERIMENTS
    return 1;
#else
    return 0;
#endif
}
```

candle-video_amd/csrc/options.h:

```cpp
#pragma once

enum { LTX_FAM_ASM16 = 1, LTX_FAM_RING = 2, LTX_FAM_P8 = 4, LTX_FAM_HALO = 8, LTX_FAM_HALO_OUT = 16, LTX_FAM_BIG = 32 };
enum { LTX_ATTN_Q64 = 1, LTX_ATTN_Q128 = 2, LTX_ATTN_CROSS = 4, LTX_ATTN_PIPE = 8 };

struct LtxOptions {
    int gemm_tune = 1;
    char gemm_plan[40] = {0};
    unsigned gemm_off = 0;
    int gemm_wide_epi = 1;
    int gemm_trace = 0;
    int attn_q64_big = -1;
    int vae_tile_batch = 0;
    int prof_kernel_events = 1;
    int ff2_defer = 1;
    int gemm_splitk = 1;
    int q2_fold = 1;
    int norm_presum = 1;
    int norm_lean = 1;
    int xattn_compact = 1;
    int attn_q64_stream = 0;
    int norm_fold = 2;
    int norm_fold_copies = 10;
    int guidance_batch = 1;
    int dense_qkv = 1;
    int vae_fuse_norm = 1;
    int t5_attn_mfma = 1;
    unsigned attn_off = 0;
};

const LtxOptions& ltx_opt();
int ltx_exp_lookup(const char* name, int dflt);
#ifdef LTX_EXPERIMENTS
#define ltx_exp(name, dflt) ltx_exp_lookup(name, dflt)
#else
#define ltx_exp(name, dflt) (dflt)
#endif
```

candle-video_amd/csrc/rownorm.hip:

```cpp
#include <type_traits>
#include "common.h"
#include "kernels.h"
#include "gemm_common.h"
#include "options.h"

namespace {

constexpr int NSLOT = 8;

__device__ __forceinline__ float group_sum(float v, int lpr) {
    for (int o = lpr >> 1; o > 0; o >>= 1) v += __shfl_xor(v, o);
    return v;
}

template <typename T>
__device__ __forceinline__ void finish_chunk(const RowNormArgs& a, const float* f_in, float mean, float rinv, int c, const float* sc,
                                             const float* sh, T* y, bool active) {
    constexpr int CH = ElemTraits<T>::CHUNK;
    const T* w = reinterpret_cast<const T*>(a.weight);
    float f[CH], wv[CH], scv[CH], shv[CH];
    if (w) { Chunk16 wc; wc.u = *reinterpret_cast<const u32x4*>(w + c * CH); chunk_to_f32<T>(wc, wv); }
    if (sc) {
#pragma unroll
        for (int q = 0; q < CH / 4; ++q) {
            f32x4 a4 = *reinterpret_cast<const f32x4*>(sc + c * CH + 4 * q), b4 = *reinterpret_cast<const f32x4*>(sh + c * CH + 4 * q);
#pragma unroll
            for (int i = 0; i < 4; ++i) { scv[4 * q + i] = a4[i]; shv[4 * q + i] = b4[i]; }
        }
    }
#pragma unroll
    for (int i = 0; i < CH; ++i) {
        float n = (f_in[i] - mean) * rinv;
        if (w) n *= wv[i];
        if (sc) n = n * (1.0f + scv[i]) + shv[i];
        if (a.act == 1) n = silu_f(n);
        f[i] = n;
    }
    Chunk16 o; f32_to_chunk<T>(f, o);
    if (active) *reinterpret_cast<u32x4*>(y + c * CH) = o.u;
}

template <typename T, bool NT = false>
__device__ __forceinline__ void finish_chunk_regs(const RowNormArgs& a, const float* f_in, float mean, float rinv, int c, bool has_w, bool has_mod,
                                                  const float* wv, const float* scv, const float* shv, T* y, bool active) {
    constexpr int CH = ElemTraits<T>::CHUNK;
    float f[CH];
#pragma unroll
    for (int i = 0; i < CH; ++i) {
        float n = (f_in[i] - mean) * rinv;
        if (has_w) n *= wv[i];
        if (has_mod) n = n * (1.0f + scv[i]) + shv[i];
        if (a.act == 1) n = silu_f(n);
        f[i] = n;
    }
    Chunk16 o; f32_to_chunk<T>(f, o);
    if (active) {
        if constexpr (NT) __builtin_nontemporal_store(o.u, reinterpret_cast<u32x4*>(y + c * CH));
        else *reinterpret_cast<u32x4*>(y + c * CH) = o.u;
    }
}

template <typename T>
__device__ __forceinline__ void load_chunk_operands(const RowNormArgs& a, int c, int64_t b, float* wv, float* scv, float* shv) {
    constexpr int CH = ElemTraits<T>::CHUNK;
    const T* w = reinterpret_cast<const T*>(a.weight);
    if (w) { Chunk16 wc; wc.u = *reinterpret_cast<const u32x4*>(w + c * CH); chunk_to_f32<T>(wc, wv); }
    if (a.scale) {
        const float* sc = a.scale + b * a.mod_stride; const float* sh = a.shift + b * a.mod_stride;
#pragma unroll
        for (int q = 0; q < CH / 4; ++q) {
            f32x4 a4 = *reinterpret_cast<const f32x4*>(sc + c * CH + 4 * q), b4 = *reinterpret_cast<const f32x4*>(sh + c * CH + 4 * q);
#pragma unroll
            for (int i = 0; i < 4; ++i) { scv[4 * q + i] = a4[i]; shv[4 * q + i] = b4[i]; }
        }
    }
}

template <typename T, int NP = 0>
__device__ __forceinline__ Chunk16 deferred_chunk(const RowNormArgs& a, int64_t row, int64_t b, int c, bool active) {
    constexpr int CH = ElemTraits<T>::CHUNK;
    float v[CH];
    const float* pp = a.parts + row * a.D + c * CH;
    if constexpr (NP > 0) {
        f32x4 t[NP][CH / 4];
#pragma unroll
        for (int p = 0; p < NP; ++p)
#pragma unroll
            for (int q = 0; q < CH / 4; ++q) t[p][q] = *reinterpret_cast<const f32x4*>(pp + (int64_t)p * a.part_stride + 4 * q);
#pragma unroll
        for (int q = 0; q < CH / 4; ++q) {
            f32x4 acc = t[0][q];
#pragma unroll
            for (int p = 1; p < NP; ++p) acc += t[p][q];
            v[4 * q] = acc[0]; v[4 * q + 1] = acc[1]; v[4 * q + 2] = acc[2]; v[4 * q + 3] = acc[3];
        }
    } else {
#pragma unroll
        for (int q = 0; q < CH / 4; ++q) { const f32x4 t = *reinterpret_cast<const f32x4*>(pp + 4 * q); v[4 * q] = t[0]; v[4 * q + 1] = t[1]; v[4 * q + 2] = t[2]; v[4 * q + 3] = t[3]; }
        for (int p = 1; p < a.nparts; ++p) {
            const float* pq = pp + (int64_t)p * a.part_stride;
#pragma unroll
            for (int q = 0; q < CH / 4; ++q) { const f32x4 t = *reinterpret_cast<const f32x4*>(pq + 4 * q); v[4 * q] += t[0]; v[4 * q + 1] += t[1]; v[4 * q + 2] += t[2]; v[4 * q + 3] += t[3]; }
        }
    }
    if (a.d_bias) {
        Chunk16 bc; bc.u = *reinterpret_cast<const u32x4*>(reinterpret_cast<const T*>(a.d_bias) + c * CH);
        float bf[CH]; chunk_to_f32<T>(bc, bf);
#pragma unroll
        for (int i = 0; i < CH; ++i) v[i] += bf[i];
    }
    Chunk16 rc; rc.u = *reinterpret_cast<const u32x4*>(reinterpret_cast<const T*>(a.x) + row * a.ldx + c * CH);
    float r[CH]; chunk_to_f32<T>(rc, r);
    if (a.d_gate) {
        const float* gp = a.d_gate + b * a.d_gate_stride + c * CH;
#pragma unroll
        for (int q = 0; q < CH / 4; ++q) {
            const f32x4 gt = *reinterpret_cast<const f32x4*>(gp + 4 * q);
#pragma unroll
            for (int i = 0; i < 4; ++i) v[4 * q + i] = __builtin_fmaf(gt[i], v[4 * q + i], r[4 * q + i]);
        }
    } else {
#pragma unroll
        for (int i = 0; i < CH; ++i) v[i] += r[i];
    }
    Chunk16 o; f32_to_chunk<T>(v, o);
    if (active) *reinterpret_cast<u32x4*>(reinterpret_cast<T*>(a.x_out) + row * a.ldx + c * CH) = o.u;
    return o;
}

template <typename T, int MODE, int DEFER = 0>
__global__ __launch_bounds__(256) void rownorm_kernel(const RowNormArgs a, int lpr) {
    constexpr int CH = ElemTraits<T>::CHUNK;
    const int lane = threadIdx.x & 63, wave = threadIdx.x >> 6;
    const int rpw = 64 / lpr;
    const int sub = lane % lpr;
    const int nch = a.D / CH;
    const float invD = 1.0f / (float)a.D;
    if constexpr (MODE == 1) {
        const int64_t row0 = ((int64_t)blockIdx.x * 4 + wave) * (rpw * NSLOT) + lane / lpr;
        const bool has = sub < nch;
        const T* xp = reinterpret_cast<const T*>(a.x) + row0 * a.ldx + sub * CH;
        T* yp = reinterpret_cast<T*>(a.y) + row0 * a.ldy;
        const int64_t xs = (int64_t)rpw * a.ldx, ys = (int64_t)rpw * a.ldy;
        Chunk16 v[NSLOT];
#pragma unroll
        for (int i = 0; i < NSLOT; ++i) {
            v[i].u = (u32x4){0u, 0u, 0u, 0u};
            if (has && row0 + i * rpw < a.rows) v[i].u = *reinterpret_cast<const u32x4*>(xp + i * xs);
        }
        float wv[CH], scv[CH], shv[CH];
        const int64_t b0 = (row0 < a.rows ? row0 : a.rows - 1) / a.rows_per_batch;
        const int64_t b0_end = (b0 + 1) * a.rows_per_batch;
        if (has) load_chunk_operands<T>(a, sub, b0, wv, scv, shv);
#pragma unroll
        for (int i = 0; i < NSLOT; ++i) {
            const int64_t row = row0 + (int64_t)i * rpw;
            const bool active = row < a.rows;
            float f[CH]; chunk_to_f32<T>(v[i], f);
            float mean = 0.f;
            if (a.kind == 1) {
                float s = 0.f;
// ... 242 lines not shown
    const int sub = threadIdx.x / nch, c = threadIdx.x - sub * nch;
    const uint32_t row0 = ((uint32_t)blockIdx.x * (uint32_t)rpb + (uint32_t)sub) * R;
    const bf16_t* x = reinterpret_cast<const bf16_t*>(a.x) + (int64_t)row0 * a.ldx + c * 8;
    u32x4 v[R];
#pragma unroll
    for (int r = 0; r < R; ++r) v[r] = *reinterpret_cast<const u32x4*>(x + (int64_t)r * a.ldx);
    f32x4 pt[4];
    if (lane < R) {
        const float* ps = a.presum + (int64_t)(row0 + lane) * a.presum_n;
#pragma unroll
        for (int q = 0; q < 4; ++q) {
            const bool in = 4 * q < a.presum_n;
            const f32x4 u = *reinterpret_cast<const f32x4*>(ps + (in ? 4 * q : a.presum_n - 4));
            pt[q] = in ? u : (f32x4){0.f, 0.f, 0.f, 0.f};
        }
    }
    const uint32_t b = row0 / (uint32_t)a.rows_per_batch;
    const float* sc = a.scale + (int64_t)b * a.mod_stride + c * 8; const float* sh = a.shift + (int64_t)b * a.mod_stride + c * 8;
    const f32x4 s0 = *reinterpret_cast<const f32x4*>(sc), s1 = *reinterpret_cast<const f32x4*>(sc + 4);
    const f32x4 h0 = *reinterpret_cast<const f32x4*>(sh), h1 = *reinterpret_cast<const f32x4*>(sh + 4);
    float mine = 0.f;
    if (lane < R) {
        float ss = 0.f;
#pragma unroll
        for (int q = 0; q < 4; ++q) { ss += pt[q][0]; ss += pt[q][1]; ss += pt[q][2]; ss += pt[q][3]; }
        mine = 1.0f / sqrtf(ss * (1.0f / (float)a.D) + a.eps);
    }
    const float scv[8] = {s0[0], s0[1], s0[2], s0[3], s1[0], s1[1], s1[2], s1[3]};
    const float shv[8] = {h0[0], h0[1], h0[2], h0[3], h1[0], h1[1], h1[2], h1[3]};
    bf16_t* y = reinterpret_cast<bf16_t*>(a.y) + (int64_t)row0 * a.ldy + c * 8;
#pragma unroll
    for (int r = 0; r < R; ++r) {
        const float rinv = __builtin_bit_cast(float, __builtin_amdgcn_readlane(__builtin_bit_cast(int, mine), r));
        Chunk16 ch; ch.u = v[r];
        float f[8]; chunk_to_f32<bf16_t>(ch, f);
#pragma unroll
        for (int i = 0; i < 8; ++i) {
            float n = (f[i] - 0.f) * rinv;
            n = n * (1.0f + scv[i]) + shv[i];
            f[i] = n;
        }
        Chunk16 o; f32_to_chunk<bf16_t>(f, o);
        *reinterpret_cast<u32x4*>(y + (int64_t)r * a.ldy) = o.u;
    }
}

#ifdef LTX_NORM_DIAG
__global__ __launch_bounds__(256) void norm_diag_kernel(const u32x4* __restrict__ x, u32x4* __restrict__ y, int64_t nchunks, int var, int rowchunks) {
    const int64_t t = (int64_t)blockIdx.x * 256 + threadIdx.x;
    if (var == 0) { if (t < nchunks) y[t] = x[t]; return; }
    u32x4 v[4];
    if (var == 1) {
        const int64_t row0 = (t / rowchunks) * 4, c = t % rowchunks;
#pragma unroll
        for (int r = 0; r < 4; ++r) v[r] = x[(row0 + r) * rowchunks + c];
#pragma unroll
        for (int r = 0; r < 4; ++r) y[(row0 + r) * rowchunks + c] = v[r];
    } else {
        const int64_t base = (int64_t)blockIdx.x * 1024 + threadIdx.x;
#pragma unroll
        for (int r = 0; r < 4; ++r) v[r] = x[base + r * 256];
#pragma unroll
        for (int r = 0; r < 4; ++r) y[base + r * 256] = v[r];
    }
}
extern "C" int ltx_dbg_norm_diag(const void* x, void* y, long long nchunks, int var, int rowchunks, void* stream) {
    const unsigned grid = (unsigned)(var == 0 ? (nchunks + 255) / 256 : nchunks / 1024);
    hipLaunchKernelGGL(norm_diag_kernel, dim3(grid), dim3(256), 0, (hipStream_t)stream, (const u32x4*)x, (u32x4*)y, (int64_t)nchunks, var, rowchunks);
    return hipGetLastError() == hipSuccess ? 0 : -1;
}
#endif

template <typename T, bool CACHED>
__global__ __launch_bounds__(256) void qknorm_rope_kernel(const QkNormRopeArgs a, int lpr) {
    constexpr int CH = ElemTraits<T>::CHUNK;
    const int lane = threadIdx.x & 63, wave = threadIdx.x >> 6;
    const int rpw = 64 / lpr;
    const int64_t row = ((int64_t)blockIdx.x * 4 + wave) * rpw + lane / lpr;
    const int sub = lane % lpr;
    const bool active = row < a.rows;
    const int64_t rr = active ? row : a.rows - 1;
    const int nch = a.D / CH;
    const float* cs = a.cos ? a.cos + rr * (a.D / 2) : nullptr;
    const float* sn = a.sin ? a.sin + rr * (a.D / 2) : nullptr;
    auto finish = [&](Chunk16 v, int c, float rinv, const T* w, const T* wb, T* x) {
        float f[CH]; chunk_to_f32<T>(v, f);
        Chunk16 wc; wc.u = *reinterpret_cast<const u32x4*>(w + c * CH);
        float wv[CH]; chunk_to_f32<T>(wc, wv);
#pragma unroll
        for (int i = 0; i < CH; ++i) f[i] = f[i] * rinv * wv[i];
        if (wb) {
            Chunk16 wc2; wc2.u = *reinterpret_cast<const u32x4*>(wb + c * CH);
            float wv2[CH]; chunk_to_f32<T>(wc2, wv2);
#pragma unroll
            for (int i = 0; i < CH; ++i) f[i] *= wv2[i];
        }
        if (cs) {
            float co[CH / 2], si[CH / 2];
            if constexpr (CH == 8) {
                f32x4 c4 = *reinterpret_cast<const f32x4*>(cs + c * 4), s4 = *reinterpret_cast<const f32x4*>(sn + c * 4);
#pragma unroll
                for (int p = 0; p < 4; ++p) { co[p] = c4[p]; si[p] = s4[p]; }
            } else {
#pragma unroll
                for (int p = 0; p < CH / 2; ++p) { co[p] = cs[c * (CH / 2) + p]; si[p] = sn[c * (CH / 2) + p]; }
            }
#pragma unroll
            for (int p = 0; p < CH / 2; ++p) {
                float re = f[2 * p], im = f[2 * p + 1];
                f[2 * p] = re * co[p] - im * si[p];
                f[2 * p + 1] = im * co[p] + re * si[p];
            }
        }
        Chunk16 o; f32_to_chunk<T>(f, o);
        if (active) *reinterpret_cast<u32x4*>(x + c * CH) = o.u;
    };
    for (int seg = 0; seg < a.nseg; ++seg) {
        T* x = reinterpret_cast<T*>(a.x) + rr * a.ld + (int64_t)seg * (a.seg_stride ? a.seg_stride : a.D);
        const T* w = reinterpret_cast<const T*>(seg == 0 ? a.w0 : a.w1);
        const T* wb = seg == 0 ? reinterpret_cast<const T*>(a.w0b) : nullptr;
        const float oscale = seg == 0 ? a.out_scale0 : 1.0f;
        if constexpr (CACHED) {
            Chunk16 v[NSLOT];
#pragma unroll
            for (int i = 0; i < NSLOT; ++i) {
                int c = sub + i * lpr;
                v[i].u = (u32x4){0u, 0u, 0u, 0u};
                if (c < nch) v[i].u = *reinterpret_cast<const u32x4*>(x + c * CH);
            }
            float ss = 0.f;
#pragma unroll
            for (int i = 0; i < NSLOT; ++i) { float f[CH]; chunk_to_f32<T>(v[i], f);
#pragma unroll
                for (int j = 0; j < CH; ++j) ss += f[j] * f[j]; }
            ss = group_sum(ss, lpr);
            const float rinv = oscale / sqrtf(ss / (float)a.D + a.eps);
#pragma unroll
            for (int i = 0; i < NSLOT; ++i) { int c = sub + i * lpr; if (c < nch) finish(v[i], c, rinv, w, wb, x); }
        } else {
            float ss = 0.f;
            for (int c = sub; c < nch; c += lpr) {
                Chunk16 v; v.u = *reinterpret_cast<const u32x4*>(x + c * CH);
                float f[CH]; chunk_to_f32<T>(v, f);
#pragma unroll
                for (int i = 0; i < CH; ++i) ss += f[i] * f[i];
            }
            ss = group_sum(ss, lpr);
            const float rinv = oscale / sqrtf(ss / (float)a.D + a.eps);
            for (int c = sub; c < nch; c += lpr) { Chunk16 v; v.u = *reinterpret_cast<const u32x4*>(x + c * CH); finish(v, c, rinv, w, wb, x); }
        }
    }
}

template <typename T, int NS, int OCC = 5>
__global__ __launch_bounds__(256, OCC) void qknorm_rope_fused_kernel(const QkNormRopeArgs a, int lpr) {
    constexpr int CH = ElemTraits<T>::CHUNK;
    static_assert(CH == 8, "bf16 rows only");
    const int lane = threadIdx.x & 63, wave = threadIdx.x >> 6;
    const int rpw = 64 / lpr;
    const int64_t row = ((int64_t)blockIdx.x * 4 + wave) * rpw + lane / lpr;
    const int sub = lane % lpr;
    const bool active = row < a.rows;
    const int64_t rr = active ? row : a.rows - 1;
    const int nch = a.D / CH;
    const bool rope = a.cos != nullptr;
    const float* cs = rope ? a.cos + rr * (a.D / 2) : nullptr;
    const float* sn = rope ? a.sin + rr * (a.D / 2) : nullptr;
    T* x0 = reinterpret_cast<T*>(a.x) + rr * a.ld;
    const int64_t sst = a.seg_stride ? a.seg_stride : a.D;
    Chunk16 v[2][NS];
    f32x4 co[NS], si[NS];
#pragma unroll
    for (int i = 0; i < NS; ++i) {
        const int c = sub + i * lpr;
        const bool in = c < nch;
        v[0][i].u = (u32x4){0u, 0u, 0u, 0u}; v[1][i].u = (u32x4){0u, 0u, 0u, 0u};
        if (in) v[0][i].u = *reinterpret_cast<const u32x4*>(x0 + c * CH);
        if (in && a.nseg == 2) v[1][i].u = *reinterpret_cast<const u32x4*>(x0 + sst + c * CH);
        if (in && rope) { co[i] = *reinterpret_cast<const f32x4*>(cs + c * 4); si[i] = *reinterpret_cast<const f32x4*>(sn + c * 4); }
    }
    float rinv[2] = {0.f, 0.f};
#pragma unroll
    for (int seg = 0; seg < 2; ++seg) {
        if (seg >= a.nseg) break;
        float ss = 0.f;
#pragma unroll
        for (int i = 0; i < NS; ++i) { float f[CH]; chunk_to_f32<T>(v[seg][i], f);
#pragma unroll
            for (int j = 0; j < CH; ++j) ss += f[j] * f[j]; }
        ss = group_sum(ss, lpr);
        rinv[seg] = (seg == 0 ? a.out_scale0 : 1.0f) / sqrtf(ss / (float)a.D + a.eps);
    }
#pragma unroll
    for (int i = 0; i < NS; ++i) {
        const int c = sub + i * lpr;
        if (c >= nch) continue;
#pragma unroll
        for (int seg = 0; seg < 2; ++seg) {
            if (seg >= a.nseg) break;
            const T* w = reinterpret_cast<const T*>(seg == 0 ? a.w0 : a.w1);
            asm volatile("" : "+v"(v[seg][i].u));
            float f[CH]; chunk_to_f32<T>(v[seg][i], f);
            Chunk16 wc; wc.u = *reinterpret_cast<const u32x4*>(w + c * CH);
            float wv[CH]; chunk_to_f32<T>(wc, wv);
#pragma unroll
            for (int j = 0; j < CH; ++j) f[j] = f[j] * rinv[seg] * wv[j];
            if (seg == 0 && a.w0b) {
                Chunk16 wc2; wc2.u = *reinterpret_cast<const u32x4*>(reinterpret_cast<const T*>(a.w0b) + c * CH);
                float wv2[CH]; chunk_to_f32<T>(wc2, wv2);
#pragma unroll
                for (int j = 0; j < CH; ++j) f[j] *= wv2[j];
            }
            if (rope) {
#pragma unroll
                for (int p = 0; p < 4; ++p) {
                    const float re = f[2 * p], im = f[2 * p + 1];
                    f[2 * p] = re * co[i][p] - im * si[i][p];
                    f[2 * p + 1] = im * co[i][p] + re * si[i][p];
                }
            }
            Chunk16 o; f32_to_chunk<T>(f, o);
            if (active) *reinterpret_cast<u32x4*>(x0 + seg * sst + c * CH) = o.u;
            __builtin_amdgcn_sched_barrier(0);
        }
    }
}

__global__ void rope_table_kernel(const RopeTableArgs a) {
    const int half = a.D / 2;
    const int64_t S = (int64_t)a.F * a.H * a.W;
    const int64_t total = (int64_t)a.B * S * half;
    const int rem_pairs = (a.D % 6) / 2;
    for (int64_t i = (int64_t)blockIdx.x * blockDim.x + threadIdx.x; i < total; i += (int64_t)gridDim.x * blockDim.x) {
        const int p = (int)(i % half);
        const int64_t row = i / half;
        float co = 1.0f, si = 0.0f;
        if (p >= rem_pairs) {
            const int fi = p - rem_pairs;
            const int step = fi / 3, ax = fi - step * 3;
            float g;
            if (a.use_coords) {
                g = a.coords[row * 3 + ax] * a.gscale[ax];
            } else {
                const int64_t s = row % S;
                const int w = (int)(s % a.W); const int64_t t1 = s / a.W;
                const int h = (int)(t1 % a.H); const int f = (int)(t1 / a.H);
                const float idx = ax == 0 ? (float)f : (ax == 1 ? (float)h : (float)w);
                g = idx * a.gscale[ax];
            }
            const float ang = a.freqs[step] * (g * 2.0f - 1.0f);
            co = cosf(ang); si = sinf(ang);
        }
        a.cos[i] = co; a.sin[i] = si;
    }
}

template <typename T>
__global__ __launch_bounds__(256) void rowsq_kernel(const T* x, int64_t rows, int N, int ld, float* out) {
    __shared__ float leaves[4][64][33];
    const int lane = threadIdx.x & 63, wave = threadIdx.x >> 6, half = lane >> 5, cg = lane & 31;
    const int ng = (N + 127) / 128;
    const int64_t npairs = rows * ng;
    const int64_t p0 = ((int64_t)blockIdx.x * 4 + wave) * 64;
#pragma unroll 4
    for (int st = 0; st < 32; ++st) {
        const int64_t pr = p0 + 2 * st + half;
        float leaf = 0.f;
        if (pr < npairs) {
            const int64_t row = pr / ng; const int g = (int)(pr - row * ng);
            const int n = g * 128 + 4 * cg;
            if (n < N) {
                if constexpr (std::is_same<T, float>::value) leaf = ltx_rowsq_leaf(*reinterpret_cast<const f32x4*>(x + row * ld + n));
                else leaf = ltx_rowsq_leaf(*reinterpret_cast<const bf16x4*>(x + row * ld + n));
            }
        }
        leaves[wave][2 * st + half][cg] = leaf;
    }
    __syncthreads();
    const int64_t pr = p0 + lane;
    if (pr < npairs) {
        float s = leaves[wave][lane][0];
#pragma unroll
        for (int c = 1; c < 32; ++c) s += leaves[wave][lane][c];
        out[pr] = s;
    }
}

template <typename T, int DEFER>
__global__ __launch_bounds__(256) void rownorm_block_kernel(const RowNormArgs a) {
    constexpr int CH = ElemTraits<T>::CHUNK, NC = 2;
    __shared__ float red[2][4];
    const int tid = threadIdx.x, lane = tid & 63, wave = tid >> 6;
    const int64_t row = blockIdx.x;
    const int nch = a.D / CH;
    const float invD = 1.0f / (float)a.D;
    const T* x = reinterpret_cast<const T*>(a.x) + row * a.ldx;
    T* y = reinterpret_cast<T*>(a.y) + row * a.ldy;
    const int64_t b = row / a.rows_per_batch;
    const float* sc = a.scale ? a.scale + b * a.mod_stride : nullptr;
    const float* sh = a.shift ? a.shift + b * a.mod_stride : nullptr;
    Chunk16 v[NC];
#pragma unroll
    for (int i = 0; i < NC; ++i) {
        const int c = tid + i * 256;
        v[i].u = (u32x4){0u, 0u, 0u, 0u};
        if (c < nch) {
            if constexpr (DEFER != 0) v[i] = deferred_chunk<T, DEFER == 4 ? 4 : 0>(a, row, b, c, true);
            else v[i].u = *reinterpret_cast<const u32x4*>(x + c * CH);
        }
    }
    auto block_sum = [&](float t, int slot) {
        t = group_sum(t, 64);
        if (lane == 0) red[slot][wave] = t;
        __syncthreads();
        return ((red[slot][0] + red[slot][1]) + red[slot][2]) + red[slot][3];
    };
    float mean = 0.f;
    if (a.kind == 1) {
        float t = 0.f;
#pragma unroll
        for (int i = 0; i < NC; ++i) { float f[CH]; chunk_to_f32<T>(v[i], f);
#pragma unroll
            for (int j = 0; j < CH; ++j) t += f[j]; }
        mean = block_sum(t, 0) * invD;
    }
    float ss = 0.f;
#pragma unroll
    for (int i = 0; i < NC; ++i) {
        if (tid + i * 256 < nch) {
            float f[CH]; chunk_to_f32<T>(v[i], f);
#pragma unroll
            for (int j = 0; j < CH; ++j) { const float d = f[j] - mean; ss += d * d; }
        }
    }
    ss = block_sum(ss, 1);
    const float rinv = 1.0f / sqrtf(ss * invD + a.eps);
#pragma unroll
    for (int i = 0; i < NC; ++i) {
        const int c = tid + i * 256;
        if (c < nch) { float f[CH]; chunk_to_f32<T>(v[i], f); finish_chunk<T>(a, f, mean, rinv, c, sc, sh, y, true); }
    }
}

int pick_lpr(int nch) {
    int lpr = 1;
    while (lpr < nch && lpr < 64) lpr <<= 1;
    return lpr;
}

template <typename T>
void launch_rownorm_t(const RowNormArgs& a, int lpr, int nch, hipStream_t s) {
    const int rpw = 64 / lpr;
    if (nch <= lpr && a.rows >= (int64_t)rpw * NSLOT * 4 * 64) {
        const int64_t rows_per_block = (int64_t)4 * rpw * NSLOT;
        LTX_LAUNCH_TIMED((rownorm_kernel<T, 1>), dim3((unsigned)cdiv64(a.rows, rows_per_block)), dim3(256), 0, s, a, lpr);
    } else if (a.rows <= 512 && nch > 64 && nch <= 512) {
        const dim3 grid((unsigned)a.rows);
        if (a.parts && a.nparts == 4) LTX_LAUNCH_TIMED((rownorm_block_kernel<T, 4>), grid, dim3(256), 0, s, a);
        else if (a.parts) LTX_LAUNCH_TIMED((rownorm_block_kernel<T, 1>), grid, dim3(256), 0, s, a);
        else LTX_LAUNCH_TIMED((rownorm_block_kernel<T, 0>), grid, dim3(256), 0, s, a);
    } else {
        const int64_t rows_per_block = 4 * rpw;
        dim3 grid((unsigned)cdiv64(a.rows, rows_per_block));
#ifdef LTX_EXPERIMENTS
        if (lpr == 64 && nch <= 4 * 64 && a.rows >= 2048 && ltx_exp("rownorm_rows", 0) == 1) {
            constexpr int R = 4;
            const int waves = (int)cdiv64(a.rows, R);
            const int blocks = (waves + 3) / 4;
            LTX_LAUNCH_TIMED((rownorm_rows_kernel<T, 4, R, 2>), dim3((unsigned)blocks), dim3(256), 0, s, a, blocks * 4);
            return;
        }
#endif
        int shm = 0;
        { const int n = ltx_exp("rownorm_occ", 0); if (n >= 1 && n <= 8) shm = 163840 / n - 1024; }
        if (shm > 65536) {
            static std::atomic<unsigned long long> occ_devs{0};
            (void)ltx_set_max_dyn_smem(occ_devs, reinterpret_cast<const void*>(&rownorm_kernel<T, 0>), 163840);
        }
        if (a.parts && a.nparts == 4) LTX_LAUNCH_TIMED((rownorm_kernel<T, 0, 4>), grid, dim3(256), 0, s, a, lpr);
        else if (a.parts) LTX_LAUNCH_TIMED((rownorm_kernel<T, 0, 1>), grid, dim3(256), 0, s, a, lpr);
        else if (nch <= NSLOT * lpr) LTX_LAUNCH_TIMED((rownorm_kernel<T, 0>), grid, dim3(256), shm, s, a, lpr);
        else LTX_LAUNCH_TIMED((rownorm_kernel<T, 2>), grid, dim3(256), 0, s, a, lpr);
    }
}

}

int ltx_launch_rownorm(const RowNormArgs& a, int dtype, hipStream_t s) {
    const int ch = dtype == LTX_DT_BF16 ? 8 : 4;
    if (a.rows <= 0) return LTX_OK;
    if (a.D % ch != 0 || a.ldx % ch != 0 || a.ldy % ch != 0) LTX_FAIL(LTX_ERR_ARG, "rownorm: D/ld must be multiples of the 16-byte chunk");
    if ((a.scale == nullptr) != (a.shift == nullptr)) LTX_FAIL(LTX_ERR_ARG, "rownorm: scale and shift go together");
    const int nch = a.D / ch, lpr = pick_lpr(nch);
    if (a.parts) {
        const int rpw = 64 / lpr;
        const bool narrow = nch <= lpr && a.rows >= (int64_t)rpw * NSLOT * 4 * 64;
        const bool block_rows = a.rows <= 512 && nch > 64 && nch <= 512;
        if (a.presum || narrow || (nch > NSLOT * lpr && !block_rows) || a.nparts < 1 || a.nparts > 16 || !a.x_out || a.part_stride < a.rows * a.D || a.D % 8 ||
            ((uintptr_t)a.parts & 15) || (a.d_gate && (((uintptr_t)a.d_gate & 15) || a.d_gate_stride % 4)))
            LTX_FAIL(LTX_ERR_ARG, "rownorm: deferred rows need whole-row lanes (D of at most 64 x 8 chunks), 1..16 parts of [rows, D] f32 and an output for the finished rows");
    }
    if (a.presum && (a.kind != 0 || a.presum_n < 4 || a.presum_n % 4 != 0 || nch > 256 || (nch & (nch - 1)) || a.rows >= 2147483647LL || a.rows_per_batch >= 2147483647LL))
        LTX_FAIL(LTX_ERR_ARG, "rownorm: presum serves RMS rows of a power-of-two number (<= 256) of 16-byte chunks with a multiple of 4 partials");
    void* tok = nullptr;
    ltx_prof_begin(LTX_PROF_ROWNORM, 2.0 * (double)a.rows * a.D * (dtype == LTX_DT_BF16 ? 2 : 4), s, &tok);
    if (a.presum) {
        const int rpb = 256 / nch;
        int R = 4;
        { const int v = ltx_exp("norm_presum_r", 4); if (v == 2 || v == 4 || v == 8) R = v; }
        const dim3 grid((unsigned)cdiv64(a.rows, (int64_t)rpb * R));
        const bool wide = nch >= 64;
        const bool lean_on = ltx_opt().norm_lean != 0, nt = ltx_exp("norm_nt", 0) != 0;
        const bool lean = lean_on && dtype == LTX_DT_BF16 && wide && R == 4 && a.scale && !a.weight && a.act == 0 && a.presum_n <= 16 &&
                          a.rows % ((int64_t)rpb * 4) == 0 && a.rows_per_batch % 4 == 0 && !nt;
        if (lean) LTX_LAUNCH_TIMED((rownorm_presum_lean_kernel<4>), grid, dim3(256), 0, s, a, nch, rpb);
        else if (dtype == LTX_DT_BF16) {
            if (R == 2) { if (wide) LTX_LAUNCH_TIMED((rownorm_presum_kernel<bf16_t, 2, true>), grid, dim3(256), 0, s, a, nch, rpb); else LTX_LAUNCH_TIMED((rownorm_presum_kernel<bf16_t, 2, false>), grid, dim3(256), 0, s, a, nch, rpb); }
            else if (R == 4 && wide && nt) LTX_LAUNCH_TIMED((rownorm_presum_kernel<bf16_t, 4, true, true>), grid, dim3(256), 0, s, a, nch, rpb);
            else if (R == 4) { if (wide) LTX_LAUNCH_TIMED((rownorm_presum_kernel<bf16_t, 4, true>), grid, dim3(256), 0, s, a, nch, rpb); else LTX_LAUNCH_TIMED((rownorm_presum_kernel<bf16_t, 4, false>), grid, dim3(256), 0, s, a, nch, rpb); }
            else { if (wide) LTX_LAUNCH_TIMED((rownorm_presum_kernel<bf16_t, 8, true>), grid, dim3(256), 0, s, a, nch, rpb); else LTX_LAUNCH_TIMED((rownorm_presum_kernel<bf16_t, 8, false>), grid, dim3(256), 0, s, a, nch, rpb); }
        } else if (wide) LTX_LAUNCH_TIMED((rownorm_presum_kernel<float, 4, true>), dim3((unsigned)cdiv64(a.rows, (int64_t)rpb * 4)), dim3(256), 0, s, a, nch, rpb);
        else LTX_LAUNCH_TIMED((rownorm_presum_kernel<float, 4, false>), dim3((unsigned)cdiv64(a.rows, (int64_t)rpb * 4)), dim3(256), 0, s, a, nch, rpb);
    } else if (dtype == LTX_DT_BF16) launch_rownorm_t<bf16_t>(a, lpr, nch, s);
    else launch_rownorm_t<float>(a, lpr, nch, s);
    ltx_prof_end(tok, s);
    LTX_CHECK_LAUNCH();
    return LTX_OK;
}

namespace {
template <typename T>
__global__ __launch_bounds__(256) void qknorm_rope_block_kernel(const QkNormRopeArgs a) {
    constexpr int CH = ElemTraits<T>::CHUNK, NC = 2;
    static_assert(CH == 8, "bf16 rows only");
    __shared__ float red[2][4];
    const int tid = threadIdx.x, lane = tid & 63, wave = tid >> 6;
    const int64_t row = blockIdx.x;
    const int nch = a.D / CH;
    const bool rope = a.cos != nullptr;
    const float* cs = rope ? a.cos + row * (a.D / 2) : nullptr;
    const float* sn = rope ? a.sin + row * (a.D / 2) : nullptr;
    T* x0 = reinterpret_cast<T*>(a.x) + row * a.ld;
    const int64_t sst = a.seg_stride ? a.seg_stride : a.D;
    Chunk16 v[2][NC];
    f32x4 co[NC], si[NC];
#pragma unroll
    for (int i = 0; i < NC; ++i) {
        const int c = tid + i * 256;
        const bool in = c < nch;
        v[0][i].u = (u32x4){0u, 0u, 0u, 0u}; v[1][i].u = (u32x4){0u, 0u, 0u, 0u};
        if (in) v[0][i].u = *reinterpret_cast<const u32x4*>(x0 + c * CH);
        if (in && a.nseg == 2) v[1][i].u = *reinterpret_cast<const u32x4*>(x0 + sst + c * CH);
        if (in && rope) { co[i] = *reinterpret_cast<const f32x4*>(cs + c * 4); si[i] = *reinterpret_cast<const f32x4*>(sn + c * 4); }
    }
    float ss[2] = {0.f, 0.f};
#pragma unroll
    for (int seg = 0; seg < 2; ++seg) {
#pragma unroll
        for (int i = 0; i < NC; ++i) { float f[CH]; chunk_to_f32<T>(v[seg][i], f);
#pragma unroll
            for (int j = 0; j < CH; ++j) ss[seg] += f[j] * f[j]; }
        ss[seg] = group_sum(ss[seg], 64);
        if (lane == 0) red[seg][wave] = ss[seg];
    }
    __syncthreads();
    float rinv[2];
#pragma unroll
    for (int seg = 0; seg < 2; ++seg) {
        const float t = ((red[seg][0] + red[seg][1]) + red[seg][2]) + red[seg][3];
        rinv[seg] = (seg == 0 ? a.out_scale0 : 1.0f) / sqrtf(t / (float)a.D + a.eps);
    }
#pragma unroll
    for (int i = 0; i < NC; ++i) {
        const int c = tid + i * 256;
        if (c >= nch) continue;
#pragma unroll
        for (int seg = 0; seg < 2; ++seg) {
            if (seg >= a.nseg) break;
            const T* w = reinterpret_cast<const T*>(seg == 0 ? a.w0 : a.w1);
            float f[CH]; chunk_to_f32<T>(v[seg][i], f);
            Chunk16 wc; wc.u = *reinterpret_cast<const u32x4*>(w + c * CH);
            float wv[CH]; chunk_to_f32<T>(wc, wv);
#pragma unroll
            for (int j = 0; j < CH; ++j) f[j] = f[j] * rinv[seg] * wv[j];
            if (seg == 0 && a.w0b) {
                Chunk16 wc2; wc2.u = *reinterpret_cast<const u32x4*>(reinterpret_cast<const T*>(a.w0b) + c * CH);
                float wv2[CH]; chunk_to_f32<T>(wc2, wv2);
#pragma unroll
                for (int j = 0; j < CH; ++j) f[j] *= wv2[j];
            }
            if (rope) {
#pragma unroll
                for (int p = 0; p < 4; ++p) {
                    const float re = f[2 * p], im = f[2 * p + 1];
                    f[2 * p] = re * co[i][p] - im * si[i][p];
                    f[2 * p + 1] = im * co[i][p] + re * si[i][p];
                }
            }
            Chunk16 o; f32_to_chunk<T>(f, o);
            *reinterpret_cast<u32x4*>(x0 + seg * sst + c * CH) = o.u;
        }
    }
}
}

int ltx_launch_qknorm_rope(const QkNormRopeArgs& a, int dtype, hipStream_t s) {
    const int ch = dtype == LTX_DT_BF16 ? 8 : 4;
    if (a.rows <= 0) return LTX_OK;
    if (a.D % ch != 0 || a.ld % ch != 0) LTX_FAIL(LTX_ERR_ARG, "qknorm: D/ld must be multiples of the 16-byte chunk");
    if (a.nseg < 1 || a.nseg > 2 || !a.w0 || (a.nseg == 2 && !a.w1)) LTX_FAIL(LTX_ERR_ARG, "qknorm: bad segments/weights");
    const int nch = a.D / ch, lpr = pick_lpr(nch);
    const int64_t rows_per_block = 4 * (64 / lpr);
    dim3 grid((unsigned)cdiv64(a.rows, rows_per_block)), block(256);
    const bool cached = nch <= NSLOT * lpr;
    if (dtype == LTX_DT_BF16) {
        if (a.rows <= 512 && nch > 64 && nch <= 512) hipLaunchKernelGGL((qknorm_rope_block_kernel<bf16_t>), dim3((unsigned)a.rows), block, 0, s, a);
        else if (nch <= 4 * lpr) hipLaunchKernelGGL((qknorm_rope_fused_kernel<bf16_t, 4>), grid, block, 0, s, a, lpr);
        else if (nch <= 8 * lpr && ltx_exp("qknorm_fused8", 1)) hipLaunchKernelGGL((qknorm_rope_fused_kernel<bf16_t, 8, 2>), grid, block, 0, s, a, lpr);
        else if (cached) hipLaunchKernelGGL((qknorm_rope_kernel<bf16_t, true>), grid, block, 0, s, a, lpr);
        else hipLaunchKernelGGL((qknorm_rope_kernel<bf16_t, false>), grid, block, 0, s, a, lpr);
    } else {
        if (cached) hipLaunchKernelGGL((qknorm_rope_kernel<float, true>), grid, block, 0, s, a, lpr);
        else hipLaunchKernelGGL((qknorm_rope_kernel<float, false>), grid, block, 0, s, a, lpr);
    }
    LTX_CHECK_LAUNCH();
    return LTX_OK;
}

int ltx_launch_rowsq(const void* x, int dtype, int64_t rows, int N, int ld, float* out, hipStream_t s) {
    if (rows <= 0 || N <= 0) return LTX_OK;
    if (!x || !out || N % 4 != 0 || ld % 4 != 0 || ((uintptr_t)x & 7)) LTX_FAIL(LTX_ERR_ARG, "rowsq: N and ld must be multiples of 4 and x 8-byte aligned");
    const int64_t npairs = rows * ((N + 127) / 128);
    dim3 grid((unsigned)cdiv64(npairs, 256)), block(256);
    if (dtype == LTX_DT_BF16) hipLaunchKernelGGL(rowsq_kernel<bf16_t>, grid, block, 0, s, reinterpret_cast<const bf16_t*>(x), rows, N, ld, out);
    else hipLaunchKernelGGL(rowsq_kernel<float>, grid, block, 0, s, reinterpret_cast<const float*>(x), rows, N, ld, out);
    LTX_CHECK_LAUNCH();
    return LTX_OK;
}

namespace {
__global__ __launch_bounds__(256) void shift_gemv_kernel(const bf16_t* __restrict__ W, const bf16_t* __restrict__ bias, const float* __restrict__ shift, int shift_stride,
                                                          int B, int N, int K, float* __restrict__ out, int out_stride) {
    const int lane = threadIdx.x & 63, wave = threadIdx.x >> 6;
    const int n = blockIdx.x * 4 + wave;
    if (n >= N) return;
    float acc[8] = {0.f, 0.f, 0.f, 0.f, 0.f, 0.f, 0.f, 0.f};
    const bf16_t* wr = W + (int64_t)n * K;
    for (int c = lane; c < K / 8; c += 64) {
        const bf16x8 w = *reinterpret_cast<const bf16x8*>(wr + c * 8);
        float wf[8];
#pragma unroll
        for (int i = 0; i < 8; ++i) wf[i] = (float)w[i];
        for (int b = 0; b < B; ++b) {
            const float* sp = shift + (int64_t)b * shift_stride + c * 8;
            const f32x4 s0 = *reinterpret_cast<const f32x4*>(sp), s1 = *reinterpret_cast<const f32x4*>(sp + 4);
            float a = acc[b];
#pragma unroll
            for (int i = 0; i < 4; ++i) a = __builtin_fmaf(wf[i], s0[i], a);
#pragma unroll
            for (int i = 0; i < 4; ++i) a = __builtin_fmaf(wf[4 + i], s1[i], a);
            acc[b] = a;
        }
    }
    const float bn = bias ? (float)bias[n] : 0.f;
    for (int b = 0; b < B; ++b) {
        float a = acc[b];
#pragma unroll
        for (int off = 32; off >= 1; off >>= 1) a += __shfl_xor(a, off);
        if (lane == 0) out[(int64_t)b * out_stride + n] = a + bn;
    }
}
}

int ltx_launch_shift_gemv(const void* W, const void* bias, const float* shift, int shift_stride, int B, int N, int K, float* cvec, int cvec_stride, hipStream_t s) {
    if (!W || !shift || !cvec || B < 1 || B > 8 || N < 1 || K < 8 || K % 8 || shift_stride % 4 || ((uintptr_t)W & 15) || ((uintptr_t)shift & 15))
        LTX_FAIL(LTX_ERR_ARG, "shift_gemv: bf16 weights [N, K] with K % 8 == 0, f32 shift rows 16-byte aligned, 1..8 batch rows");
    hipLaunchKernelGGL(shift_gemv_kernel, dim3((unsigned)((N + 3) / 4)), dim3(256), 0, s, reinterpret_cast<const bf16_t*>(W), reinterpret_cast<const bf16_t*>(bias),
                       shift, shift_stride, B, N, K, cvec, cvec_stride);
    LTX_CHECK_LAUNCH();
    return LTX_OK;
}

int ltx_launch_rope_table(const RopeTableArgs& a, hipStream_t s) {
    if (a.D % 2 != 0 || a.D < 6) LTX_FAIL(LTX_ERR_ARG, "rope: dim must be even and >= 6");
    const int64_t total = (int64_t)a.B * a.F * a.H * a.W * (a.D / 2);
    int64_t blocks = cdiv64(total, 256); if (blocks > 8192) blocks = 8192;
    hipLaunchKernelGGL(rope_table_kernel, dim3((unsigned)blocks), dim3(256), 0, s, a);
    LTX_CHECK_LAUNCH();
    return LTX_OK;
}
```

candle-video_amd/ltxhip/__init__.py:

```python
from __future__ import annotations

import ctypes as C
import os
from dataclasses import dataclass, field
from typing import Dict, List, Optional, Sequence, Tuple

import torch

_HERE = os.path.dirname(os.path.abspath(__file__))
_LIB_PATH = os.environ.get("LTXHIP_LIB") or os.path.join(os.path.dirname(_HERE), "libltxhip.so")

if not os.path.exists(_LIB_PATH):
    raise ImportError(
        f"ltxhip: {_LIB_PATH} is missing — build it with `make -C candle-video_amd` "
        "(or `python -c 'import __graft_entry__ as g; g.build()'`). There is no CPU fallback.")
lib = C.CDLL(_LIB_PATH)

LTX_F32, LTX_BF16 = 0, 1


class LtxError(RuntimeError):
    pass


lib.ltx_last_error.restype = C.c_char_p


def _check(rc: int):
    if rc != 0:
        raise LtxError(f"[ltxhip rc={rc}] {lib.ltx_last_error().decode()}")


class _Weight(C.Structure):
    _fields_ = [("name", C.c_char_p), ("data", C.c_void_p), ("dtype", C.c_int), ("ndim", C.c_int),
                ("shape", C.c_int64 * 5), ("on_device", C.c_int)]


class DitConfigC(C.Structure):
    _fields_ = [(n, C.c_int) for n in ("in_channels", "out_channels", "patch_size", "patch_size_t",
                                       "num_attention_heads", "attention_head_dim", "cross_attention_dim", "num_layers")] + \
               [("norm_eps", C.c_float), ("caption_channels", C.c_int)]


class VaeConfigC(C.Structure):
    _fields_ = [("latent_channels", C.c_int), ("out_channels", C.c_int), ("n_blocks", C.c_int),
                ("decoder_block_out_channels", C.c_int * 4), ("decoder_layers_per_block", C.c_int * 5),
                ("decoder_upsample_factor", C.c_int * 4), ("patch_size", C.c_int), ("patch_size_t", C.c_int),
                ("timestep_conditioning", C.c_int), ("decoder_causal", C.c_int), ("scaling_factor", C.c_float),
                ("spatial_compression_ratio", C.c_int), ("temporal_compression_ratio", C.c_int),
                ("decoder_inject_noise", C.c_int * 5), ("decoder_upsample_residual", C.c_int * 4),
                ("decoder_spatiotemporal_scaling", C.c_int * 4), ("resnet_eps", C.c_float)]


class TilingC(C.Structure):
    _fields_ = [(n, C.c_int) for n in ("use_tiling", "use_framewise_decoding", "tile_sample_min_height", "tile_sample_min_width",
                                       "tile_sample_min_num_frames", "tile_sample_stride_height", "tile_sample_stride_width",
                                       "tile_sample_stride_num_frames")]


class PipelineParamsC(C.Structure):
    _fields_ = [("height", C.c_int), ("width", C.c_int), ("num_frames", C.c_int), ("frame_rate", C.c_int),
                ("num_inference_steps", C.c_int), ("sigmas", C.POINTER(C.c_float)),
                ("guidance_scale", C.c_float), ("guidance_rescale", C.c_float), ("stg_scale", C.c_float),
                ("skip_block_list", C.POINTER(C.c_int)), ("n_skip_blocks", C.c_int),
                ("decode_timestep", C.c_float), ("decode_noise_scale", C.c_float),
                ("output_latent", C.c_int), ("postprocess", C.c_int), ("tiling", C.POINTER(TilingC)),
                ("shift_terminal", C.c_float), ("use_shift_terminal", C.c_int),
                ("stochastic_sampling", C.c_int), ("step_noise", C.POINTER(C.c_float)),
                ("interrupt", C.POINTER(C.c_int)), ("on_step", C.c_void_p), ("on_step_user", C.c_void_p)]


StepFn = C.CFUNCTYPE(C.c_int, C.c_void_p, C.c_int, C.c_int, C.c_int64)


_vp, _i, _i64, _f, _sz = C.c_void_p, C.c_int, C.c_int64, C.c_float, C.c_size_t
_fp = C.POINTER(C.c_float)
_SIGS = {
    "ltx_dit_config_default": [_vp], "ltx_vae_config_default": [_vp], "ltx_tiling_default": [_vp],
    "ltx_dit_create": [_vp, _vp, _sz, _i, _i, _vp], "ltx_dit_destroy": [_vp],
    "ltx_dit_set_skip_blocks": [_vp, _vp, _i], "ltx_dit_context_cache": [_vp, _i], "ltx_dit_get_config": [_vp, _vp],
    "ltx_dit_forward": [_vp, _vp, _vp, _vp, _vp, _i, _i, _i, _i, _i, _i, _vp, _vp, _vp, _i, _vp, _vp],
    "ltx_vae_create": [_vp, _vp, _sz, _i, _i, _vp], "ltx_vae_destroy": [_vp], "ltx_vae_get_config": [_vp, _vp],
    "ltx_vae_set_noise_seed": [_vp, C.c_uint64], "ltx_vae_injects_noise": [_vp],
    "ltx_vae_latents_mean": [_vp], "ltx_vae_latents_std": [_vp],
    "ltx_vae_decode": [_vp, _vp, _i, _vp, _i, _i, _i, _i, _vp, _i, _vp, _vp],
    "ltx_vae_decode_tokens": [_vp, _vp, _vp, _vp, _vp, _i, _i, _i, _i, _vp, _i, _vp, _vp],
    "ltx_vae_prepare_latents": [_vp, _vp, _vp, _vp, _i, _i, _i, _i, _vp, _vp],
    "ltx_guidance_step": [_vp, _vp, _vp, _i, _vp, _vp, _i, _i64, _f, _f, _f, _f, _vp, _vp],
    "ltx_guidance_step_stochastic": [_vp, _vp, _vp, _i, _vp, _vp, _i, _i64, _f, _f, _f, _f, _f, _vp, _vp, _vp],
    "ltx_sched_set_timesteps": [_vp, _i, _f, _i, _f, _f, _i, _vp, _vp],
    "ltx_sched_set_timesteps_ex": [_vp, _i, _f, _i, _f, _f, _i, _i, _i, _vp, _vp],
    "ltx_calculate_shift": [_i, _i, _i, _f, _f],
    "ltx_pcg32_randn": [C.c_uint64, C.c_uint64, _sz, _vp],
    "ltx_pcg32_u32": [C.c_uint64, C.c_uint64, _sz, _vp],
    "ltx_device_alloc": [_sz, _i, _vp], "ltx_device_free": [_vp], "ltx_memcpy_h2d": [_vp, _vp, _sz, _vp], "ltx_memcpy_d2h": [_vp, _vp, _sz, _vp],
    "ltx_stream_synchronize": [_vp],
    "ltx_warmup": [_vp, _vp, _i, _i, _i, _i, _i, _vp], "ltx_set_autotune": [_i], "ltx_plan_save": [C.c_char_p], "ltx_plan_load": [C.c_char_p],
    "ltx_pipeline_last_steps": [C.POINTER(C.c_int), C.POINTER(C.c_int)], "ltx_attention_fallback_counts": [C.POINTER(C.c_ulonglong), C.c_int], "ltx_set_option": [C.c_char_p, C.c_char_p], "ltx_get_option": [C.c_char_p, C.c_char_p, C.c_int], "ltx_reset_options": [], "ltx_has_experiments": [],
    "ltx_build_video_coords": [_i, _i, _i, _i, _i, _i, _vp],
    "ltx_pipeline_params_default": [_vp],
    "ltx_pipeline_call": [_vp, _vp, _vp, _vp, _vp, _vp, _vp, _vp, _vp, _i, _i, _vp, _vp],
    "ltx_pipeline_last_timing": [_vp],
    "ltx_prof_enable": [_i], "ltx_prof_report": [_i, _vp, _vp, _vp], "ltx_prof_report_kernel": [_i, _i, _vp, _vp, _vp],
    "ltx_op_linear": [_vp, _vp, _vp, _vp, _i, _i, _i, _i, _i, _vp, _vp, _i, _vp],
    "ltx_op_linear_segmented": [_vp, _vp, _vp, _vp, _i, _i, _i, _i, _i, _vp],
    "ltx_op_ring_packed_bytes": [_i, _i], "ltx_op_ring_pack": [_vp, _i, _i, _vp, _vp],
    "ltx_op_linear_packed": [_vp, _vp, _vp, _vp, _vp, _i, _i, _i, _i, _vp, _vp, _i, _vp],
    "ltx_op_rownorm_presum": [_vp, _vp, _i64, _i, _f, _vp, _vp, _vp, _i64, _i, _i, _vp, _i, _i, _vp],
    "ltx_op_linear_rowsq": [_vp, _vp, _vp, _vp, _vp, _i, _i, _i, _i, _i, _vp, _vp, _i, _vp], "ltx_op_rowsq": [_vp, _i64, _i, _i, _vp, _i, _vp],
    "ltx_op_linear_fold_out": [_vp, _vp, _vp, _vp, _vp, _vp, _vp, _i, _i, _i, _i, _i, _vp, _vp, _i, _vp],
    "ltx_op_linear_fold_in": [_vp, _vp, _vp, _vp, _i, _i, _f, _vp, _i, _i, _i, _i, _i, _i, _vp],
    "ltx_op_linear_fold_ok": [_i, _i, _i, _i, _i, _i, _i, _i],
    "ltx_op_shift_gemv": [_vp, _vp, _vp, _i, _i, _i, _i, _vp, _i, _vp],
    "ltx_op_mod_scale": [_vp, _vp, _i, _vp, _i, _i64, _i, _i, _vp], "ltx_op_scale_cols": [_vp, _vp, _vp, _i64, _i, _i, _vp],
    "ltx_op_linear_split_factor": [_i, _i, _i], "ltx_op_linear_deferred": [_vp, _vp, _vp, _i, _i, _i, _vp],
    "ltx_op_rownorm_deferred": [_vp, _i, _vp, _vp, _vp, _i, _vp, _vp, _i64, _i, _i, _f, _vp, _vp, _i64, _i, _i, _vp],
    "ltx_op_attention_compact": [_vp, _vp, _vp, _vp, _i, _i, _i, _i, _i, _i, _i, _i, _i, _f, _vp, _vp, _i, _i, _f, _vp, _vp],
    "ltx_op_attention_rowsq": [_vp, _vp, _vp, _vp, _i, _i, _i, _i, _i, _i, _i, _i, _i, _f, _vp, _vp, _i, _i, _f, _vp],
    "ltx_op_rownorm": [_vp, _vp, _i64, _i, _i, _f, _vp, _vp, _vp, _i64, _i, _i, _i, _vp],
    "ltx_op_qknorm_rope": [_vp, _i64, _i, _i, _vp, _f, _vp, _vp, _i, _vp],
    "ltx_op_rope_table": [_vp, _vp, _vp, _i, _i, _i, _i, _i, _vp, _vp],
    "ltx_op_timestep_embedding": [_vp, _i, _i, _f, _i, _vp, _vp],
    "ltx_op_attention": [_vp, _vp, _vp, _vp, _i, _i, _i, _i, _i, _i, _i, _i, _i, _f, _vp, _i, _vp],
    "ltx_op_attention_prescaled": [_vp, _vp, _vp, _vp, _i, _i, _i, _i, _i, _i, _i, _i, _i, _vp],
    "ltx_op_conv3d": [_vp, _vp, _vp, _i, _vp, _vp, _i, _i, _i, _i, _i, _i, _i, _i, _vp],
    "ltx_op_upsample3d": [_vp, _vp, _vp, _i, _vp, _i, _i, _i, _i, _i, _i, _i, _i, _i, _vp],
    "ltx_op_conv_out_unpatchify": [_vp, _vp, _vp, _i, _vp, _i, _i, _i, _i, _i, _i, _i, _i, _i, _vp],
    "ltx_op_blend": [_vp, _vp, _i, _i, _i, _i, _i, _i, _i, _i, _i, _vp],
    "ltx_op_downsample3d": [_vp, _vp, _vp, _i, _vp, _i, _i, _i, _i, _i, _i, _i, _i, _vp],
    "ltx_op_gemm_plan": [_i, _i, _i, _i, _i, _i, _i, _i, C.c_char_p, _i],
    "ltx_op_gemm_route": [_i, _i, _i, _i, _i, _i, _i, _i, _i, _i, _i, _i, C.c_char_p, _i],
    "ltx_op_dit_plan": [_i, _i, _i, _i, _i, _i, _i, _i, _i, C.POINTER(C.c_int64)],
    "ltx_t5_config_default": [_vp], "ltx_t5_create": [_vp, _vp, _sz, _i, _i, _vp], "ltx_t5_destroy": [_vp],
    "ltx_t5_forward": [_vp, _vp, _i, _i, _i, _vp, _vp],
    "ltx_t5_create_from_gguf": [_vp, C.c_char_p, _i, _i, _vp], "ltx_t5_forward_masked": [_vp, _vp, _vp, _i, _i, _i, _vp, _vp],
    "ltx_gguf_open": [C.c_char_p, _vp], "ltx_gguf_close": [_vp], "ltx_gguf_count": [_vp], "ltx_gguf_find": [_vp, C.c_char_p],
    "ltx_gguf_tensor": [_vp, _sz, _vp, _vp, _vp, _vp, _vp, _vp], "ltx_gguf_type_info": [_i, _vp, _vp],
    "ltx_gguf_dequantize": [_i, _vp, _i, _i64, _i, _vp, _vp],
    "ltx_video_to_rgb8": [_vp, _i, _i, _i, _i, _vp, _vp], "ltx_write_png": [C.c_char_p, _vp, _i, _i],
    "ltx_save_frames_png": [_vp, _i, _i, _i, _i, C.c_char_p, _vp, _vp],
    "ltx_write_gif": [C.c_char_p, _vp, _i, _i, _i, _i, _i], "ltx_save_video_gif": [_vp, _i, _i, _i, _i, C.c_char_p, _vp],
    "ltx_preset_count": [], "ltx_preset_name": [_i], "ltx_preset_get": [C.c_char_p, _vp], "ltx_pipeline_params_from_preset": [_vp, _vp],
    "ltx_weights_detect_format": [C.c_char_p], "ltx_weights_remap_key": [C.c_char_p, C.c_char_p, _sz],
    "ltx_weights_is_transformer_key": [C.c_char_p], "ltx_weights_is_vae_key": [C.c_char_p],
    "ltx_name_mapper_create": [], "ltx_name_mapper_destroy": [_vp], "ltx_name_mapper_add": [_vp, _i, C.c_char_p, C.c_char_p],
    "ltx_name_mapper_has_mapping": [_vp, C.c_char_p], "ltx_name_mapper_map": [_vp, C.c_char_p, C.c_char_p, _sz],
    "ltx_weights_validate_names": [_vp, _sz, _vp, _sz, _vp, _vp],
    "ltx_safetensors_open": [C.c_char_p, _vp], "ltx_safetensors_close": [_vp], "ltx_safetensors_count": [_vp],
    "ltx_safetensors_tensor": [_vp, _sz, _vp, _vp, _vp, _vp, _vp, _vp],
    "ltx_weights_resolve": [C.c_char_p, C.c_char_p, _sz, _vp],
    "ltx_dit_create_from_files": [_vp, C.c_char_p, _i, _i, _i, _vp], "ltx_vae_create_from_files": [_vp, C.c_char_p, _i, _i, _i, _vp],
    "ltx_vae_config_from_json": [C.c_char_p, _vp], "ltx_vae_encoder_create_from_files": [_vp, C.c_char_p, _i, _i, _i, _vp],
    "ltx_team_unique_id": [_vp], "ltx_team_create": [_vp, _i, _i, _i, _vp], "ltx_team_destroy": [_vp], "ltx_team_size": [_vp], "ltx_team_rank": [_vp],
    "ltx_team_allgather_f32": [_vp, _vp, _vp, _sz, _vp], "ltx_team_exchange_f32": [_vp, _vp, _sz, _i, _vp, _sz, _i, _vp],
}
EXPORTED_SYMBOLS = sorted(list(_SIGS) + ["ltx_last_error"])
for _name, _sig in _SIGS.items():
    _fn = getattr(lib, _name)
    _fn.argtypes = _sig
    if _name not in ("ltx_calculate_shift", "ltx_vae_latents_mean", "ltx_vae_latents_std", "ltx_name_mapper_create",
                     "ltx_name_mapper_destroy", "ltx_safetensors_close", "ltx_safetensors_count", "ltx_team_destroy"):
        _fn.restype = C.c_int
lib.ltx_calculate_shift.restype = C.c_float
lib.ltx_op_ring_packed_bytes.restype = C.c_int64
lib.ltx_vae_latents_mean.restype = C.c_void_p
lib.ltx_vae_latents_std.restype = C.c_void_p
lib.ltx_name_mapper_create.restype = C.c_void_p
lib.ltx_name_mapper_destroy.restype = None
lib.ltx_safetensors_close.restype = None
lib.ltx_safetensors_count.restype = C.c_size_t
lib.ltx_gguf_close.restype = None
lib.ltx_gguf_count.restype = C.c_size_t


class VaeEncoderConfigC(C.Structure):
    _fields_ = [("in_channels", C.c_int), ("latent_channels", C.c_int), ("n_blocks", C.c_int),
                ("block_out_channels", C.c_int * 5), ("layers_per_block", C.c_int * 5),
                ("spatiotemporal_scaling", C.c_int * 4), ("downsample_types", C.c_int * 4),
                ("patch_size", C.c_int), ("patch_size_t", C.c_int), ("is_causal", C.c_int),
                ("spatial_compression_ratio", C.c_int), ("temporal_compression_ratio", C.c_int)]


class EncodeTilingC(C.Structure):
    _fields_ = [("use_framewise_encoding", C.c_int)]


_ENC_SIGS = {
    "ltx_vae_encoder_config_default": [_vp], "ltx_vae_encoder_config_from_preset": [_vp, _vp],
    "ltx_vae_encoder_create": [_vp, _vp, _sz, _i, _i, _vp], "ltx_vae_encoder_destroy": [_vp], "ltx_vae_encoder_get_config": [_vp, _vp],
    "ltx_vae_encode": [_vp, _vp, _i, _i, _i, _i, _i, _vp, _vp, _vp, _vp, _vp],
    "ltx_vae_posterior_sample": [_vp, _vp, _vp, _sz, _vp, _vp],
    "ltx_vae_encode_tokens": [_vp, _vp, _vp, _i, _i, _i, _i, _i, _vp, _vp, _vp, _vp, _vp],
    "ltx_vae_encoder_warmup": [_vp, _i, _i, _i, _i, _vp, _vp, _vp],
}
ENCODER_SYMBOLS = sorted(_ENC_SIGS)
for _name, _sig in _ENC_SIGS.items():
    _fn = getattr(lib, _name)
    _fn.argtypes = _sig
    _fn.restype = None if _name in ("ltx_vae_encoder_config_default", "ltx_vae_encoder_destroy") else C.c_int


class ConditioningC(C.Structure):
    _fields_ = [("hold", C.POINTER(C.c_ubyte))]


_COND_SIGS = {
    "ltx_dit_forward_frames": [_vp, _vp, _vp, _vp, _vp, _i, _i, _i, _i, _i, _i, _vp, _vp, _vp, _i, _vp, _vp],
    "ltx_guidance_step_held": [_vp, _vp, _vp, _i, _vp, _vp, _i, _i64, _f, _f, _f, _f, _vp, _vp, _i, _i64, _vp],
    "ltx_guidance_step_stochastic_held": [_vp, _vp, _vp, _i, _vp, _vp, _i, _i64, _f, _f, _f, _f, _f, _vp, _vp, _vp, _i, _i64, _vp],
    "ltx_cond_apply": [_vp, _vp, _i, _vp, _i, _i, _i, _i, _vp],
    "ltx_pipeline_call_cond": [_vp, _vp, _vp, _vp, _vp, _vp, _vp, _vp, _vp, _vp, _i, _i, _vp, _vp],
}
COND_SYMBOLS = sorted(_COND_SIGS)
for _name, _sig in _COND_SIGS.items():
    _fn = getattr(lib, _name)
    _fn.argtypes = _sig
    _fn.restype = C.c_int


_LORA_SIGS = {
    "ltx_lora_parse_key": [C.c_char_p, C.c_char_p, _sz, C.POINTER(C.c_int)],
    "ltx_lora_create": [_vp, _vp, _sz, _i, _vp, _vp], "ltx_lora_create_from_file": [_vp, C.c_char_p, _i, _vp, _vp], "ltx_lora_destroy": [_vp],
    "ltx_dit_set_adapters": [_vp, _vp, _vp, _i, _vp], "ltx_dit_adapter_count": [_vp], "ltx_dit_read_linear": [_vp, _i, _i, _vp, _vp],
    "ltx_op_lora_merge": [_vp, _vp, _i64, _i, _i, _vp, _vp, _vp, _vp, _i, _vp],
}
LORA_SYMBOLS = sorted(_LORA_SIGS)
for _name, _sig in _LORA_SIGS.items():
    _fn = getattr(lib, _name)
    _fn.argtypes = _sig
    _fn.restype = None if _name == "ltx_lora_destroy" else C.c_int
LORA_TARGETS = ("attn1.to_q", "attn1.to_k", "attn1.to_v", "attn1.to_out.0", "attn2.to_q", "attn2.to_k", "attn2.to_v", "attn2.to_out.0",
                "ff.net.0.proj", "ff.net.2")


def _dt(t: torch.dtype) -> int:
    if t == torch.float32:
        return LTX_F32
    if t == torch.bfloat16:
        return LTX_BF16
    raise LtxError(f"unsupported dtype {t}")


def _ptr(t: Optional[torch.Tensor]):
    return C.c_void_p(t.data_ptr()) if t is not None else None


def _stream():
    return C.c_void_p(torch.cuda.current_stream().cuda_stream)


def _dev(t: torch.Tensor, dtype=None) -> torch.Tensor:
    if not t.is_cuda:
        raise LtxError("tensor must live on the GPU (the library takes device pointers)")
    if dtype is not None and t.dtype != dtype:
        t = t.to(dtype)
    return t.contiguous()


def _expect(name: str, t: torch.Tensor, shape):
    if tuple(t.shape) != tuple(shape):
        raise LtxError(f"{name}: shape {tuple(t.shape)} does not match the call's geometry {tuple(shape)}")


def _make_weights(weights: Dict[str, torch.Tensor]):
    arr = (_Weight * len(weights))()
    keep = []
    for i, (name, t) in enumerate(weights.items()):
        if t.dtype not in (torch.float32, torch.bfloat16):
            t = t.float()
        t = t.contiguous()
        keep.append(t)
        nb = name.encode()
        keep.append(nb)
        arr[i].name = nb
# ... 1102 lines not shown
    def rowsq(x):
        M, N = x.shape
        rs = torch.empty(M, (N + 127) // 128, dtype=torch.float32, device=x.device)
        _check(lib.ltx_op_rowsq(_ptr(x.contiguous()), C.c_int64(M), N, N, _ptr(rs), _dt(x.dtype), _stream()))
        return rs

    @staticmethod
    def linear_fold_ok(M, N, K, epi, consumer, rs_n=0, vec_stride=None, rows_per_batch=None) -> bool:
        return bool(lib.ltx_op_linear_fold_ok(M, N, K, epi, int(bool(consumer)), rs_n, N if vec_stride is None else vec_stride,
                                              M if rows_per_batch is None else rows_per_batch))

    @staticmethod
    def linear_fold_out(x, w, bias, scale2, epi, resid, gate=None, rows_per_batch=1):
        M, K = x.shape
        N = w.shape[0]
        y = torch.empty(M, N, dtype=x.dtype, device=x.device); y2 = torch.empty_like(y)
        rs = torch.empty(M, (N + 127) // 128, dtype=torch.float32, device=x.device)
        _check(lib.ltx_op_linear_fold_out(_ptr(x.contiguous()), _ptr(w.contiguous()), _ptr(bias), _ptr(y), _ptr(y2), _ptr(rs), _ptr(scale2), scale2.shape[-1],
                                          M, N, K, epi, _ptr(resid), _ptr(gate), rows_per_batch, _stream()))
        return y, y2, rs

    @staticmethod
    def linear_fold_in(x, w, rs_sq, cvec, epi=0, rows_per_batch=1, rs_D=None, eps=1e-6):
        M, K = x.shape
        N = w.shape[0]
        y = torch.empty(M, N, dtype=x.dtype, device=x.device)
        _check(lib.ltx_op_linear_fold_in(_ptr(x.contiguous()), _ptr(w.contiguous()), _ptr(y), _ptr(rs_sq.contiguous()), rs_sq.shape[-1], K if rs_D is None else rs_D,
                                         C.c_float(eps), _ptr(cvec), cvec.shape[-1], M, N, K, epi, rows_per_batch, _stream()))
        return y

    @staticmethod
    def shift_gemv(w, bias, shift, K=None, out_stride=None):
        N, Kw = w.shape
        K = Kw if K is None else K
        B = shift.shape[0]
        out = torch.zeros(B, N if out_stride is None else out_stride, dtype=torch.float32, device=w.device)
        _check(lib.ltx_op_shift_gemv(_ptr(w.contiguous()), _ptr(bias), _ptr(shift), shift.shape[-1], B, N, K, _ptr(out), out.shape[-1], _stream()))
        return out

    @staticmethod
    def mod_scale(h, scale, rows_per_batch):
        rows, D = h.shape
        y = torch.empty_like(h)
        _check(lib.ltx_op_mod_scale(_ptr(h.contiguous()), _ptr(scale), scale.shape[-1], _ptr(y), rows // rows_per_batch, C.c_int64(rows_per_batch), D, _dt(h.dtype), _stream()))
        return y

    @staticmethod
    def scale_cols(w, scale):
        N, K = w.shape
        out = torch.empty_like(w)
        _check(lib.ltx_op_scale_cols(_ptr(w.contiguous()), _ptr(scale), _ptr(out), C.c_int64(N), K, _dt(w.dtype), _stream()))
        return out

    @staticmethod
    def lora_merge(w0, adapters):
        w0 = _dev(w0); N, K = w0.shape
        As = [_dev(a, w0.dtype) for a, _, _ in adapters]; Bs = [_dev(b, w0.dtype) for _, b, _ in adapters]
        for a, b in zip(As, Bs):
            _expect("A", a, (a.shape[0], K)); _expect("B", b, (N, a.shape[0]))
        n = len(adapters)
        out = torch.empty_like(w0)
        pa = (C.c_void_p * max(n, 1))(*[a.data_ptr() for a in As]); pb = (C.c_void_p * max(n, 1))(*[b.data_ptr() for b in Bs])
        rs = (C.c_int * max(n, 1))(*[a.shape[0] for a in As])
        _check(lib.ltx_op_lora_merge(_ptr(w0), _ptr(out), N, K, n, pa, pb, rs, _floats([c for _, _, c in adapters]) if n else None, _dt(w0.dtype), _stream()))
        return out

    @staticmethod
    def attention_rowsq(q, k, v, heads, scale, key_bias, q_rowsq, eps=1e-5):
        B, Sq, D = q.shape
        o = torch.empty_like(q)
        _check(lib.ltx_op_attention_rowsq(_ptr(q.contiguous()), _ptr(k.contiguous()), _ptr(v.contiguous()), _ptr(o), B, Sq, k.shape[1], heads, D // heads,
                                          D, D, D, D, C.c_float(scale), _ptr(key_bias), _ptr(q_rowsq), q_rowsq.shape[-1], D, C.c_float(eps), _stream()))
        return o

    @staticmethod
    def attention_compact(q, k, v, heads, scale, key_bias, q_rowsq=None, eps=1e-5):
        B, Sq, D = q.shape
        o = torch.empty_like(q)
        cnt = torch.zeros(B, dtype=torch.int32, device=q.device)
        _check(lib.ltx_op_attention_compact(_ptr(q.contiguous()), _ptr(k.contiguous()), _ptr(v.contiguous()), _ptr(o), B, Sq, k.shape[1], heads, D // heads,
                                            D, D, D, D, C.c_float(scale), _ptr(key_bias.contiguous()), _ptr(q_rowsq) if q_rowsq is not None else None,
                                            q_rowsq.shape[-1] if q_rowsq is not None else 0, D, C.c_float(eps), _ptr(cnt), _stream()))
        return o, cnt

    @staticmethod
    def linear_segmented(x, w, bias, seg_width):
        M, K = x.shape
        N = w.shape[0]
        y = torch.empty(N // seg_width, M, seg_width, dtype=x.dtype, device=x.device)
        _check(lib.ltx_op_linear_segmented(_ptr(x.contiguous()), _ptr(w.contiguous()), _ptr(bias), _ptr(y), M, N, K, seg_width,
                                           _dt(x.dtype), _stream()))
        return y

    @staticmethod
    def rownorm(x, kind=0, eps=1e-6, weight=None, scale=None, shift=None, rows_per_batch=1, act=0):
        rows, D = x.shape
        y = torch.empty_like(x)
        ms = scale.shape[-1] if scale is not None else 0
        _check(lib.ltx_op_rownorm(_ptr(x.contiguous()), _ptr(y), C.c_int64(rows), D, kind, C.c_float(eps), _ptr(weight),
                                  _ptr(scale), _ptr(shift), C.c_int64(rows_per_batch), ms, act, _dt(x.dtype), _stream()))
        return y

    @staticmethod
    def linear_deferred(x, w):
        M, K = x.shape
        N = w.shape[0]
        P = lib.ltx_op_linear_split_factor(M, N, K)
        parts = torch.empty(P, M, N, dtype=torch.float32, device=x.device)
        _check(lib.ltx_op_linear_deferred(_ptr(x.contiguous()), _ptr(w.contiguous()), _ptr(parts), M, N, K, _stream()))
        return parts

    @staticmethod
    def rownorm_deferred(parts, bias, resid, gate=None, kind=0, eps=1e-6, scale=None, shift=None, rows_per_batch=1):
        P, rows, D = parts.shape
        h = torch.empty_like(resid); y = torch.empty_like(resid)
        ms = scale.shape[-1] if scale is not None else 0
        _check(lib.ltx_op_rownorm_deferred(_ptr(parts), P, _ptr(bias), _ptr(resid.contiguous()), _ptr(gate), gate.shape[-1] if gate is not None else 0, _ptr(h),
                                           _ptr(y), C.c_int64(rows), D, kind, C.c_float(eps), _ptr(scale), _ptr(shift), C.c_int64(rows_per_batch), ms, _dt(resid.dtype), _stream()))
        return h, y

    @staticmethod
    def rownorm_presum(x, presum, eps=1e-6, weight=None, scale=None, shift=None, rows_per_batch=1, act=0):
        rows, D = x.shape
        y = torch.empty_like(x)
        ms = scale.shape[-1] if scale is not None else 0
        _check(lib.ltx_op_rownorm_presum(_ptr(x.contiguous()), _ptr(y), C.c_int64(rows), D, C.c_float(eps), _ptr(weight), _ptr(scale), _ptr(shift),
                                         C.c_int64(rows_per_batch), ms, act, _ptr(presum), presum.shape[-1], _dt(x.dtype), _stream()))
        return y

    @staticmethod
    def qknorm_rope(x, weight, eps=1e-5, cos=None, sin=None):
        x = x.clone().contiguous()
        rows, D = x.shape
        _check(lib.ltx_op_qknorm_rope(_ptr(x), C.c_int64(rows), D, D, _ptr(weight), C.c_float(eps), _ptr(cos), _ptr(sin),
                                      _dt(x.dtype), _stream()))
        return x

    @staticmethod
    def timestep_embedding(timesteps, vae_flavour=False, multiplier=1.0, dtype=torch.float32, device="cuda"):
        ts = [float(t) for t in timesteps]
        out = torch.empty(len(ts), 256, dtype=dtype, device=device)
        _check(lib.ltx_op_timestep_embedding(_floats(ts), len(ts), int(bool(vae_flavour)), C.c_float(multiplier), _dt(dtype), _ptr(out), _stream()))
        return out

    @staticmethod
    def rope_table(B, F, H, W, D, coords=None, rope_scale=None, device="cuda"):
        cos = torch.empty(B * F * H * W, D // 2, dtype=torch.float32, device=device)
        sin = torch.empty_like(cos)
        _check(lib.ltx_op_rope_table(_ptr(cos), _ptr(sin), _ptr(coords), B, F, H, W, D,
                                     _floats(rope_scale) if rope_scale is not None else None, _stream()))
        return cos, sin

    @staticmethod
    def attention(q, k, v, heads, scale, key_bias=None):
        B, Sq, D = q.shape
        Sk = k.shape[1]
        o = torch.empty_like(q)
        _check(lib.ltx_op_attention(_ptr(q.contiguous()), _ptr(k.contiguous()), _ptr(v.contiguous()), _ptr(o), B, Sq, Sk, heads, D // heads,
                                    D, D, D, D, C.c_float(scale), _ptr(key_bias), _dt(q.dtype), _stream()))
        return o

    @staticmethod
    def attention_prescaled(q, k, v, heads):
        B, Sq, D = q.shape
        def rows(t):
            return t if t.stride(2) == 1 and t.stride(0) == t.shape[1] * t.stride(1) and t.stride(1) % 8 == 0 else t.contiguous()
        q, k, v = rows(q), rows(k), rows(v)
        o = torch.empty(B, Sq, D, dtype=q.dtype, device=q.device)
        _check(lib.ltx_op_attention_prescaled(_ptr(q), _ptr(k), _ptr(v), _ptr(o), B, Sq, k.shape[1],
                                              heads, D // heads, q.stride(1), k.stride(1), v.stride(1), D, _stream()))
        return o

    @staticmethod
    def conv3d(x_cl, w, bias, causal=False, resid=None):
        B, T, H, W, Cin = x_cl.shape
        Cout = w.shape[0]
        y = torch.empty(B, T, H, W, Cout, dtype=x_cl.dtype, device=x_cl.device)
        _check(lib.ltx_op_conv3d(_ptr(x_cl.contiguous()), _ptr(w.contiguous()), _ptr(bias.to(w.dtype).contiguous()), _dt(w.dtype), _ptr(y), _ptr(resid),
                                 B, T, H, W, Cin, Cout, int(causal), _dt(x_cl.dtype), _stream()))
        return y

    @staticmethod
    def upsample3d(x_cl, w, bias, causal=False, residual=True):
        B, T, H, W, Cin = x_cl.shape
        Cout = w.shape[0]
        y = torch.empty(B, 2 * T - 1, 2 * H, 2 * W, Cout // 8, dtype=x_cl.dtype, device=x_cl.device)
        _check(lib.ltx_op_upsample3d(_ptr(x_cl.contiguous()), _ptr(w.contiguous()), _ptr(bias.to(w.dtype).contiguous()), _dt(w.dtype), _ptr(y),
                                     B, T, H, W, Cin, Cout, int(causal), int(residual), _dt(x_cl.dtype), _stream()))
        return y

    @staticmethod
    def downsample3d(x_cl, w, bias, down_type):
        B, T, H, W, Cin = x_cl.shape
        st, sh, sw = {1: (1, 2, 2), 2: (2, 1, 1), 3: (2, 2, 2)}.get(down_type, (2, 2, 2))
        Cout = w.shape[0] * st * sh * sw
        y = torch.empty(B, (T + st - 1) // st, H // sh, W // sw, Cout, dtype=x_cl.dtype, device=x_cl.device)
        _check(lib.ltx_op_downsample3d(_ptr(x_cl.contiguous()), _ptr(w.contiguous()), _ptr(bias.to(w.dtype).contiguous()), _dt(w.dtype), _ptr(y),
                                       B, T, H, W, Cin, Cout, down_type, _dt(x_cl.dtype), _stream()))
        return y

    @staticmethod
    def gemm_plan(M, N, K, conv=0, ntaps=1, T=1, H=1, W=1) -> str:
        buf = C.create_string_buffer(32)
        _check(lib.ltx_op_gemm_plan(M, N, K, conv, ntaps, T, H, W, buf, 32))
        return buf.value.decode()

    @staticmethod
    def gemm_route(M, N, K, conv=0, ntaps=1, B=1, T=1, H=1, W=1, epi=0, dtype=torch.bfloat16, pn=False, defer=False, fold_in=False, fold_out=False) -> str:
        buf = C.create_string_buffer(32)
        flags = (1 if pn else 0) | (2 if defer else 0) | (4 if fold_in else 0) | (8 if fold_out else 0)
        _check(lib.ltx_op_gemm_route(M, N, K, conv, ntaps, B, T, H, W, epi, _dt(dtype), flags, buf, 32))
        return buf.value.decode()

    DIT_PLAN_FIELDS = ("M", "MK", "NB", "Sg", "seg", "ldqkv", "fold_q2", "presum", "nfold", "defer_ff2", "ff2_parts", "dense_qkv", "fold_q")

    @staticmethod
    def dit_plan(heads, head_dim, B, S, K, G=1, dtype=torch.bfloat16, io_dtype=torch.float32, skip_mask=False) -> dict:
        out = (C.c_int64 * len(ops.DIT_PLAN_FIELDS))()
        _check(lib.ltx_op_dit_plan(heads, head_dim, _dt(dtype), _dt(io_dtype), B, S, K, G, int(bool(skip_mask)), out))
        return {k: (int(v) if i < 6 or k == "ff2_parts" else bool(v)) for i, (k, v) in enumerate(zip(ops.DIT_PLAN_FIELDS, out))}

    @staticmethod
    def blend(a, b, dim, blend_extent):
        a = a.contiguous(); b = b.clone().contiguous()
        BC = a.shape[0] * a.shape[1]
        _check(lib.ltx_op_blend(_ptr(a), _ptr(b), BC, a.shape[2], a.shape[3], a.shape[4], b.shape[2], b.shape[3], b.shape[4],
                                dim, blend_extent, _stream()))
        return b

    @staticmethod
    def conv_out_unpatchify(x_cl, w, bias, causal=False, postprocess=False):
        B, T, H, W, Cin = x_cl.shape
        Cout = w.shape[0]
        y = torch.empty(B, Cout // 16, T, 4 * H, 4 * W, dtype=torch.float32, device=x_cl.device)
        _check(lib.ltx_op_conv_out_unpatchify(_ptr(x_cl.contiguous()), _ptr(w.contiguous()), _ptr(bias.to(w.dtype).contiguous()), _dt(w.dtype), _ptr(y),
                                              B, T, H, W, Cin, Cout, int(causal), int(postprocess), _dt(x_cl.dtype), _stream()))
        return y


def prof_enable(on: bool):
    _check(lib.ltx_prof_enable(int(on)))


def prof_report(kind: int):
    ms, work, cnt = C.c_double(), C.c_double(), C.c_longlong()
    _check(lib.ltx_prof_report(kind, C.byref(ms), C.byref(work), C.byref(cnt)))
    return ms.value, work.value, cnt.value


PROF_KERNELS = ("gemm_kernel (128 x 128)", "gemm_big_kernel", "gemm_p8_kernel", "conv_halo_kernel", "gemm_asm_kernel (32x32x16)", "gemm_asm16_kernel", "gemm_ring_kernel")


def prof_report_kernel(kind: int, kernel: int):
    ms, work, cnt = C.c_double(), C.c_double(), C.c_longlong()
    _check(lib.ltx_prof_report_kernel(kind, kernel, C.byref(ms), C.byref(work), C.byref(cnt)))
    return ms.value, work.value, cnt.value
```

include/ltxhip_ops.h:

```cpp
#ifndef LTXHIP_OPS_H
#define LTXHIP_OPS_H
#include "ltxhip.h"
#ifdef __cplusplus
extern "C" {
#endif

int ltx_op_linear(const void* x, const void* w, const void* bias, void* y, int M, int N, int K, int dtype, int epi,
                  const void* resid, const float* gate, int rows_per_batch, ltx_stream stream);

int64_t ltx_op_ring_packed_bytes(int N, int K);
int ltx_op_ring_pack(const void* w, int N, int K, void* out, ltx_stream stream);
int ltx_op_linear_packed(const void* x, const void* w, const void* w_packed, const void* bias, void* y, int M, int N, int K, int epi,
                         const void* resid, const float* gate, int rows_per_batch, ltx_stream stream);
int ltx_op_linear_rowsq(const void* x, const void* w, const void* bias, void* y, float* rowsq, int M, int N, int K, int dtype, int epi,
                        const void* resid, const float* gate, int rows_per_batch, ltx_stream stream);
int ltx_op_rowsq(const void* x, int64_t rows, int N, int ld, float* rowsq, int dtype, ltx_stream stream);

int ltx_op_linear_fold_out(const void* x, const void* w, const void* bias, void* y, void* y2, float* rowsq, const float* scale2, int scale2_stride,
                           int M, int N, int K, int epi, const void* resid, const float* gate, int rows_per_batch, ltx_stream stream);
int ltx_op_linear_fold_in(const void* x, const void* w, void* y, const float* rs_sq, int rs_n, int rs_D, float eps, const float* cvec, int cvec_stride,
                          int M, int N, int K, int epi, int rows_per_batch, ltx_stream stream);
int ltx_op_linear_fold_ok(int M, int N, int K, int epi, int consumer, int rs_n, int vec_stride, int rows_per_batch);
int ltx_op_shift_gemv(const void* w, const void* bias, const float* shift, int shift_stride, int B, int N, int K, float* cvec, int cvec_stride, ltx_stream stream);
int ltx_op_mod_scale(const void* h, const float* scale, int scale_stride, void* y, int B, int64_t rows_per_batch, int D, int dtype, ltx_stream stream);
int ltx_op_scale_cols(const void* w, const float* scale, void* out, int64_t N, int K, int dtype, ltx_stream stream);

int ltx_op_linear_segmented(const void* x, const void* w, const void* bias, void* y, int M, int N, int K, int seg_width,
                            int dtype, ltx_stream stream);

int ltx_op_rownorm_presum(const void* x, void* y, int64_t rows, int D, float eps, const void* weight,
                          const float* scale, const float* shift, int64_t rows_per_batch, int mod_stride, int act,
                          const float* presum, int presum_n, int dtype, ltx_stream stream);

int ltx_op_linear_split_factor(int M, int N, int K);
int ltx_op_linear_deferred(const void* x, const void* w, float* parts, int M, int N, int K, ltx_stream stream);
int ltx_op_rownorm_deferred(const float* parts, int nparts, const void* bias, const void* resid, const float* gate, int gate_stride, void* h_out,
                            void* y, int64_t rows, int D, int kind, float eps, const float* scale, const float* shift, int64_t rows_per_batch,
                            int mod_stride, int dtype, ltx_stream stream);

int ltx_op_rownorm(const void* x, void* y, int64_t rows, int D, int kind, float eps, const void* weight,
                   const float* scale, const float* shift, int64_t rows_per_batch, int mod_stride, int act,
                   int dtype, ltx_stream stream);

int ltx_op_qknorm_rope(void* x, int64_t rows, int D, int ld, const void* weight, float eps,
                       const float* cos, const float* sin, int dtype, ltx_stream stream);

int ltx_op_timestep_embedding(const float* timesteps_host, int n, int vae_flavour, float multiplier, int dtype, void* out, ltx_stream stream);

int ltx_op_rope_table(float* cos, float* sin, const float* coords, int B, int F, int H, int W, int D,
                      const float* rope_scale_host, ltx_stream stream);

int ltx_op_attention(const void* q, const void* k, const void* v, void* o, int B, int Sq, int Sk, int heads, int hd,
                     int ldq, int ldk, int ldv, int ldo, float scale, const float* key_bias, int dtype, ltx_stream stream);
int ltx_attention_fallback_counts(unsigned long long counts[2], int reset);
int ltx_op_attention_rowsq(const void* q, const void* k, const void* v, void* o, int B, int Sq, int Sk, int heads, int hd,
                           int ldq, int ldk, int ldv, int ldo, float scale, const float* key_bias,
                           const float* q_rowsq, int q_rowsq_n, int q_rowsq_D, float q_rowsq_eps, ltx_stream stream);
int ltx_op_attention_compact(const void* q, const void* k, const void* v, void* o, int B, int Sq, int Sk, int heads, int hd,
                             int ldq, int ldk, int ldv, int ldo, float scale, const float* key_bias,
                             const float* q_rowsq, int q_rowsq_n, int q_rowsq_D, float q_rowsq_eps, int* counts_out, ltx_stream stream);
int ltx_op_attention_prescaled(const void* q, const void* k, const void* v, void* o, int B, int Sq, int Sk, int heads, int hd,
                               int ldq, int ldk, int ldv, int ldo, ltx_stream stream);

int ltx_op_conv3d(const void* x, const void* w, const void* bias, int wdtype, void* y, const void* resid,
                  int B, int T, int H, int W, int Cin, int Cout, int causal, int dtype, ltx_stream stream);

int ltx_op_upsample3d(const void* x, const void* w, const void* bias, int wdtype, void* y,
                      int B, int T, int H, int W, int Cin, int Cout, int causal, int residual, int dtype, ltx_stream stream);

int ltx_op_downsample3d(const void* x, const void* w, const void* bias, int wdtype, void* y,
                        int B, int T, int H, int W, int Cin, int Cout, int down_type, int dtype, ltx_stream stream);

int ltx_op_conv_out_unpatchify(const void* x, const void* w, const void* bias, int wdtype, float* y,
                               int B, int T, int H, int W, int Cin, int Cout, int causal, int postprocess, int dtype, ltx_stream stream);

int ltx_op_blend(const float* a, float* b, int BC, int at, int ah, int aw, int bt, int bh, int bw, int dim, int blend_extent, ltx_stream stream);

int ltx_op_gemm_plan(int M, int N, int K, int conv, int ntaps, int T, int H, int W, char* name, int cap);

enum { LTX_ROUTE_PN = 1,
       LTX_ROUTE_DEFER = 2,
       LTX_ROUTE_FOLD_IN = 4,
       LTX_ROUTE_FOLD_OUT = 8 };
int ltx_op_gemm_route(int M, int N, int K, int conv, int ntaps, int B, int T, int H, int W, int epi, int dtype, int flags, char* name, int cap);

enum { LTX_DIT_PLAN_FIELDS = 13 };
int ltx_op_dit_plan(int heads, int head_dim, int model_dtype, int io_dtype, int B, int S, int K, int G, int skip_mask, int64_t* out);

#ifdef __cplusplus
}
#endif
#endif
```

Baseline: 557.3 frames/sec.

## Replace per-token RoPE tables with a factorized per-axis dictionary in qknorm

Adds a small per-axis (F+H+W) cos/sin dictionary, built alongside the full rope tables, that the fused qk-norm+RoPE kernel indexes by decomposing the token index into frame, height and width. This is meant to cut the per-row reads of large per-token cos/sin tables. A check kernel verifies that the supplied coords actually follow a raster grid and otherwise sets a flag so the kernel falls back to the old tables. The cost is extra index arithmetic, a device flag read in the kernel, and a carefully ordered FMA rotation to keep numerics matching. The path is enabled by default.

```diff
diff --git a/candle-video_amd/csrc/capi_ops.hip b/candle-video_amd/csrc/capi_ops.hip
--- a/candle-video_amd/csrc/capi_ops.hip
+++ b/candle-video_amd/csrc/capi_ops.hip
@@ -200,6 +200,40 @@
     if (rc != LTX_OK) return rc;
     if (e != hipSuccess) { ltx_set_error(hipGetErrorString(e)); return LTX_ERR_HIP; }
     return LTX_OK;
+}
+
+extern "C" int ltx_op_rope_dict(float* dict, int* ok, const float* coords, int B, int S, int F, int H, int W, int D,
+                                const float* rope_scale_host, ltx_stream stream) {
+    if (!dict || !ok) LTX_FAIL(LTX_ERR_ARG, "ltx_op_rope_dict: null tensor");
+    int steps = D / 6; if (steps < 1) steps = 1;
+    std::vector<float> fr(steps);
+    const float theta_ln = (float)std::log(10000.0);
+    for (int i = 0; i < steps; ++i) {
+        float lin = steps <= 1 ? 0.0f : (float)i * (float)(1.0 / (double)(steps - 1));
+        fr[i] = (float)std::exp((double)(lin * theta_ln)) * (float)(M_PI / 2.0);
+    }
+    float* dfr = nullptr;
+    HIP_TRY(hipMalloc((void**)&dfr, sizeof(float) * steps));
+    HIP_TRY(hipMemcpy(dfr, fr.data(), sizeof(float) * steps, hipMemcpyHostToDevice));
+    RopeDictArgs r; r.dict = dict; r.ok = ok; r.coords = coords; r.freqs = dfr; r.B = B; r.S = S; r.F = F; r.H = H; r.W = W; r.D = D;
+    if (coords) { r.gscale[0] = (float)(1.0 / 20.0); r.gscale[1] = (float)(1.0 / 2048.0); r.gscale[2] = (float)(1.0 / 2048.0); }
+    else if (rope_scale_host) { r.gscale[0] = (float)((double)rope_scale_host[0] / 20.0); r.gscale[1] = (float)((double)rope_scale_host[1] / 2048.0); r.gscale[2] = (float)((double)rope_scale_host[2] / 2048.0); }
+    int rc = ltx_launch_rope_dict(r, (hipStream_t)stream);
+    hipError_t e = hipStreamSynchronize((hipStream_t)stream);
+    (void)hipFree(dfr);
+    if (rc != LTX_OK) return rc;
+    if (e != hipSuccess) { ltx_set_error(hipGetErrorString(e)); return LTX_ERR_HIP; }
+    return LTX_OK;
+}
+
+extern "C" int ltx_op_qknorm_rope_dict(void* x, int64_t rows, int D, int ld, int64_t seg_stride, int nseg, const void* w0, const void* w1, float eps,
+                                       const float* cos, const float* sin, float out_scale0, const float* dict, const int* dict_ok,
+                                       int F, int H, int W, int S, int dtype, ltx_stream stream) {
+    if (!x || !w0) LTX_FAIL(LTX_ERR_ARG, "ltx_op_qknorm_rope_dict: null tensor");
+    if (dict && (!dict_ok || !cos || !sin || F < 1 || H < 1 || W < 1 || S < 1)) LTX_FAIL(LTX_ERR_ARG, "ltx_op_qknorm_rope_dict: the dictionary needs its flag, the tables and the grid");
+    QkNormRopeArgs a; a.x = x; a.rows = rows; a.D = D; a.ld = ld; a.seg_stride = seg_stride; a.nseg = nseg; a.w0 = w0; a.w1 = w1; a.eps = eps;
+    a.cos = cos; a.sin = sin; a.out_scale0 = out_scale0; a.dict = dict; a.dict_ok = dict_ok; a.F = F; a.H = H; a.W = W; a.S = S;
+    return ltx_launch_qknorm_rope(a, dtc(dtype), (hipStream_t)stream);
 }
 
 extern "C" int ltx_op_attention(const void* q, const void* k, const void* v, void* o, int B, int Sq, int Sk, int heads, int hd,
diff --git a/candle-video_amd/csrc/dit.hip b/candle-video_amd/csrc/dit.hip
--- a/candle-video_amd/csrc/dit.hip
+++ b/candle-video_amd/csrc/dit.hip
@@ -69,13 +69,13 @@
     struct LoraSlots { void* base[7] = {nullptr}; void* merged[7] = {nullptr}; };
     std::vector<LoraSlots> lora_w;
     int n_adapters = 0;
-    DevBuf xin, encin, h, n, qkv, attn, ff, c1, encp, kv2, tproj, e1, emb, embs, temb, ada, adaf, cosb, sinb, bias, orig, orig_hsq, outT, rsq, hsq, parts;
+    DevBuf xin, encin, h, n, qkv, attn, ff, c1, encp, kv2, tproj, e1, emb, embs, temb, ada, adaf, cosb, sinb, ropedict, bias, orig, orig_hsq, outT, rsq, hsq, parts;
     void free_all() {
         for (void* p : owned) if (p) (void)hipFree(p);
         owned.clear();
         for (auto& ls : lora_w) for (void*& p : ls.merged) if (p) { (void)hipFree(p); p = nullptr; }
         lora_w.clear();
-        DevBuf* bs[] = {&xin, &encin, &h, &n, &qkv, &attn, &ff, &c1, &encp, &kv2, &tproj, &e1, &emb, &embs, &temb, &ada, &adaf, &cosb, &sinb, &bias, &orig, &orig_hsq, &outT, &rsq, &hsq, &parts};
+        DevBuf* bs[] = {&xin, &encin, &h, &n, &qkv, &attn, &ff, &c1, &encp, &kv2, &tproj, &e1, &emb, &embs, &temb, &ada, &adaf, &cosb, &sinb, &ropedict, &bias, &orig, &orig_hsq, &outT, &rsq, &hsq, &parts};
         for (DevBuf* b : bs) b->release();
         release_caches();
     }
@@ -454,6 +454,11 @@
     *out = ctx;
     return LTX_OK;
 }
+size_t rope_dict_size(const DitPlan& p, int F, int H, int W) {
+    const bool raster = F > 0 && H > 0 && W > 0 && (int64_t)F * H * W == p.S;
+    return (raster ? ltx_rope_dict_bytes(F, H, W, p.D) : 0) + sizeof(int);
+}
+int* rope_dict_ok(ltx_dit* m, const DitPlan& p, int F, int H, int W) { return reinterpret_cast<int*>((char*)m->ropedict.p + rope_dict_size(p, F, H, W) - sizeof(int)); }
 int rope_tables(ltx_dit* m, const DitPlan& p, int num_frames, int height, int width, const float* rope_scale, const float* video_coords, hipStream_t s) {
     const ltx_dit_config& c = m->cfg;
     auto& rk = m->rope_key;
@@ -476,6 +481,10 @@
         }
     }
     LTX_TRY(ltx_launch_rope_table(r, s));
+    RopeDictArgs rd; rd.dict = m->ropedict.as<float>(); rd.ok = rope_dict_ok(m, p, num_frames, height, width); rd.coords = video_coords; rd.freqs = m->rope_freqs;
+    rd.B = p.B; rd.S = p.S; rd.D = p.D; rd.F = num_frames; rd.H = height; rd.W = width;
+    for (int i = 0; i < 3; ++i) rd.gscale[i] = r.gscale[i];
+    LTX_TRY(ltx_launch_rope_dict(rd, s));
     rk.coords = video_coords; rk.B = p.B; rk.S = p.S; rk.F = num_frames; rk.H = height; rk.W = width; rk.stream = s;
     rk.has_rs = rope_scale != nullptr; if (rope_scale) memcpy(rk.rs, rope_scale, sizeof(rk.rs));
     rk.valid = m->ctx_mode;
@@ -537,6 +546,10 @@
     QkNormRopeArgs qa; qa.x = m->qkv.p; qa.rows = M; qa.D = D; qa.ld = p.ldqkv; qa.seg_stride = p.seg; qa.nseg = 2; qa.w0 = b.nq1; qa.w1 = b.nk1;
     qa.eps = 1e-5f; qa.cos = m->cosb.as<float>(); qa.sin = m->sinb.as<float>();
     if (p.fold_q) qa.out_scale0 = attn_scale * 1.4426950408889634f;
+    if (ltx_opt().rope_dict) {
+        const auto& rk = m->rope_key;
+        qa.dict = m->ropedict.as<float>(); qa.dict_ok = rope_dict_ok(m, p, rk.F, rk.H, rk.W); qa.F = rk.F; qa.H = rk.H; qa.W = rk.W; qa.S = S;
+    }
     LTX_TRY(ltx_launch_qknorm_rope(qa, dt, s));
     AttnArgs at; at.q = m->qkv.p; at.k = (char*)m->qkv.p + (size_t)p.seg * esz; at.v = (char*)m->qkv.p + (size_t)2 * p.seg * esz; at.o = m->attn.p;
     at.ldq = at.ldk = at.ldv = p.ldqkv; at.ldo = D; at.B = B; at.Sq = S; at.Sk = S; at.heads = H; at.hd = hd; at.scale = attn_scale;
@@ -611,7 +624,7 @@
     const std::pair<DevBuf*, size_t> ws[] = {
         {&m->xin, M * c.in_channels * esz}, {&m->encin, MK * c.caption_channels * esz}, {&m->h, MD}, {&m->n, MD}, {&m->qkv, 3 * MD}, {&m->attn, MD}, {&m->ff, 4 * MD},
         {&m->c1, KD}, {&m->encp, KD}, {&m->kv2, 2 * KD}, {&m->tproj, nte * 256 * esz}, {&m->e1, nte * D * esz}, {&m->emb, nte * D * esz}, {&m->embs, nte * D * esz},
-        {&m->temb, nte * 6 * D * esz}, {&m->cosb, rope}, {&m->sinb, rope}, {&m->bias, MK * sizeof(float)}, {&m->outT, M * c.out_channels * esz},
+        {&m->temb, nte * 6 * D * esz}, {&m->cosb, rope}, {&m->sinb, rope}, {&m->ropedict, rope_dict_size(p, num_frames, height, width)}, {&m->bias, MK * sizeof(float)}, {&m->outT, M * c.out_channels * esz},
         {&m->rsq, p.fold_q2 ? part : 0}, {&m->hsq, p.presum ? part : 0}, {&m->parts, p.defer_ff2 ? (size_t)p.ff2_parts * M * D * sizeof(float) : 0}, {&m->orig, skip_layer_mask ? MD : 0}};
     for (const auto& w : ws) LTX_TRY(w.first->ensure(w.second));
 
diff --git a/candle-video_amd/csrc/kernels.h b/candle-video_amd/csrc/kernels.h
--- a/candle-video_amd/csrc/kernels.h
+++ b/candle-video_amd/csrc/kernels.h
@@ -118,6 +118,8 @@
     float eps = 1e-5f;
     const float* cos = nullptr; const float* sin = nullptr;
     float out_scale0 = 1.f;
+    const float* dict = nullptr; const int* dict_ok = nullptr;
+    int F = 0, H = 0, W = 0, S = 0;
 };
 int ltx_launch_qknorm_rope(const QkNormRopeArgs& a, int dtype, hipStream_t s);
 
@@ -130,6 +132,16 @@
     float gscale[3] = {1.f, 1.f, 1.f};
 };
 int ltx_launch_rope_table(const RopeTableArgs& a, hipStream_t s);
+
+struct RopeDictArgs {
+    float* dict = nullptr; int* ok = nullptr;
+    const float* coords = nullptr;
+    const float* freqs = nullptr;
+    int B = 1, S = 0, F = 1, H = 1, W = 1, D = 0;
+    float gscale[3] = {1.f, 1.f, 1.f};
+};
+size_t ltx_rope_dict_bytes(int F, int H, int W, int D);
+int ltx_launch_rope_dict(const RopeDictArgs& a, hipStream_t s);
 
 struct AttnArgs {
     const void* q = nullptr; const void* k = nullptr; const void* v = nullptr; void* o = nullptr;
diff --git a/candle-video_amd/csrc/options.cpp b/candle-video_amd/csrc/options.cpp
--- a/candle-video_amd/csrc/options.cpp
+++ b/candle-video_amd/csrc/options.cpp
@@ -37,7 +37,7 @@
 struct IntField { const char* name; int LtxOptions::*field; };
 const IntField kInts[] = {
     {"gemm_tune", &LtxOptions::gemm_tune}, {"gemm_wide_epi", &LtxOptions::gemm_wide_epi}, {"gemm_trace", &LtxOptions::gemm_trace},
-    {"attn_q64_big", &LtxOptions::attn_q64_big}, {"vae_tile_batch", &LtxOptions::vae_tile_batch}, {"prof_kernel_events", &LtxOptions::prof_kernel_events}, {"ff2_defer", &LtxOptions::ff2_defer},
+    {"attn_q64_big", &LtxOptions::attn_q64_big}, {"vae_tile_batch", &LtxOptions::vae_tile_batch}, {"prof_kernel_events", &LtxOptions::prof_kernel_events}, {"ff2_defer", &LtxOptions::ff2_defer}, {"rope_dict", &LtxOptions::rope_dict},
     {"gemm_splitk", &LtxOptions::gemm_splitk}, {"q2_fold", &LtxOptions::q2_fold}, {"norm_presum", &LtxOptions::norm_presum}, {"norm_lean", &LtxOptions::norm_lean},
     {"xattn_compact", &LtxOptions::xattn_compact}, {"dense_qkv", &LtxOptions::dense_qkv}, {"vae_fuse_norm", &LtxOptions::vae_fuse_norm}, {"t5_attn_mfma", &LtxOptions::t5_attn_mfma}, {"guidance_batch", &LtxOptions::guidance_batch}, {"norm_fold", &LtxOptions::norm_fold}, {"norm_fold_copies", &LtxOptions::norm_fold_copies}, {"attn_q64_stream", &LtxOptions::attn_q64_stream},
 };
diff --git a/candle-video_amd/csrc/options.h b/candle-video_amd/csrc/options.h
--- a/candle-video_amd/csrc/options.h
+++ b/candle-video_amd/csrc/options.h
@@ -13,6 +13,7 @@
     int vae_tile_batch = 0;
     int prof_kernel_events = 1;
     int ff2_defer = 1;
+    int rope_dict = 1;
     int gemm_splitk = 1;
     int q2_fold = 1;
     int norm_presum = 1;
diff --git a/candle-video_amd/csrc/rownorm.hip b/candle-video_amd/csrc/rownorm.hip
--- a/candle-video_amd/csrc/rownorm.hip
+++ b/candle-video_amd/csrc/rownorm.hip
@@ -7,6 +7,7 @@
 namespace {
 
 constexpr int NSLOT = 8;
+typedef float f32x2 __attribute__((ext_vector_type(2)));
 
 __device__ __forceinline__ float group_sum(float v, int lpr) {
     for (int o = lpr >> 1; o > 0; o >>= 1) v += __shfl_xor(v, o);
@@ -555,7 +556,15 @@
     }
 }
 
-template <typename T, int NS, int OCC = 5>
+__device__ __forceinline__ void rope_pair(int p, float& re, float& im, float c, float s) {
+#pragma clang fp contract(off)
+    const float r = re, i = im;
+    const float is = i * s;
+    re = p == 0 ? r * c - is : __builtin_fmaf(r, c, -is);
+    im = p == 3 ? __builtin_fmaf(r, s, i * c) : __builtin_fmaf(i, c, r * s);
+}
+
+template <typename T, int NS, int OCC = 5, bool DICT = false>
 __global__ __launch_bounds__(256, OCC) void qknorm_rope_fused_kernel(const QkNormRopeArgs a, int lpr) {
     constexpr int CH = ElemTraits<T>::CHUNK;
     static_assert(CH == 8, "bf16 rows only");
@@ -573,6 +582,7 @@
     const int64_t sst = a.seg_stride ? a.seg_stride : a.D;
     Chunk16 v[2][NS];
     f32x4 co[NS], si[NS];
+    f32x2 e[DICT ? NS : 1][4];
 #pragma unroll
     for (int i = 0; i < NS; ++i) {
         const int c = sub + i * lpr;
@@ -580,7 +590,33 @@
         v[0][i].u = (u32x4){0u, 0u, 0u, 0u}; v[1][i].u = (u32x4){0u, 0u, 0u, 0u};
         if (in) v[0][i].u = *reinterpret_cast<const u32x4*>(x0 + c * CH);
         if (in && a.nseg == 2) v[1][i].u = *reinterpret_cast<const u32x4*>(x0 + sst + c * CH);
-        if (in && rope) { co[i] = *reinterpret_cast<const f32x4*>(cs + c * 4); si[i] = *reinterpret_cast<const f32x4*>(sn + c * 4); }
+        if constexpr (!DICT) if (in && rope) { co[i] = *reinterpret_cast<const f32x4*>(cs + c * 4); si[i] = *reinterpret_cast<const f32x4*>(sn + c * 4); }
+    }
+    if constexpr (DICT) {
+        if (*a.dict_ok != 0) {
+            const unsigned sr = (unsigned)rr % (unsigned)a.S;
+            const unsigned pw = sr % (unsigned)a.W, t1 = sr / (unsigned)a.W, ph = t1 % (unsigned)a.H, pf = t1 / (unsigned)a.H;
+            const unsigned rem = ((unsigned)a.D % 6u) / 2u, rowb = (unsigned)nch * 16u;
+            const unsigned o0 = pf * rowb, o1 = ((unsigned)a.F + ph) * rowb, o2 = ((unsigned)(a.F + a.H) + pw) * rowb;
+            const char* dp = reinterpret_cast<const char*>(a.dict);
+#pragma unroll
+            for (int i = 0; i < NS; ++i) {
+                const unsigned c = min((unsigned)(sub + i * lpr), (unsigned)nch - 1u);
+                const unsigned r3 = (4u * c + 3u - rem) % 3u, cb = c * 16u;
+                const unsigned oa = r3 == 0 ? o0 : (r3 == 1 ? o1 : o2), ob = r3 == 0 ? o1 : (r3 == 1 ? o2 : o0), oc = r3 == 0 ? o2 : (r3 == 1 ? o0 : o1);
+                const f32x4 t = *reinterpret_cast<const f32x4*>(dp + (oa + cb));
+                e[i][0] = (f32x2){t[0], t[1]}; e[i][3] = (f32x2){t[2], t[3]};
+                e[i][1] = *reinterpret_cast<const f32x2*>(dp + (ob + cb));
+                e[i][2] = *reinterpret_cast<const f32x2*>(dp + (oc + cb));
+            }
+        } else {
+#pragma unroll
+            for (int i = 0; i < NS; ++i) {
+                const int c = sub + i * lpr;
+#pragma unroll
+                for (int j = 0; j < 4; ++j) { e[i][j] = (f32x2){1.0f, 0.0f}; if (c < nch) { e[i][j][0] = cs[c * 4 + j]; e[i][j][1] = sn[c * 4 + j]; } }
+            }
+        }
     }
     float rinv[2] = {0.f, 0.f};
 #pragma unroll
@@ -617,9 +653,8 @@
             if (rope) {
 #pragma unroll
                 for (int p = 0; p < 4; ++p) {
-                    const float re = f[2 * p], im = f[2 * p + 1];
-                    f[2 * p] = re * co[i][p] - im * si[i][p];
-                    f[2 * p + 1] = im * co[i][p] + re * si[i][p];
+                    const float cp = DICT ? e[DICT ? i : 0][p][0] : co[i][p], sp = DICT ? e[DICT ? i : 0][p][1] : si[i][p];
+                    rope_pair(p, f[2 * p], f[2 * p + 1], cp, sp);
                 }
             }
             Chunk16 o; f32_to_chunk<T>(f, o);
@@ -627,6 +662,40 @@
             __builtin_amdgcn_sched_barrier(0);
         }
     }
+}
+
+__global__ void rope_dict_kernel(const RopeDictArgs a) {
+    const int nch = a.D / 8, rem = (a.D % 6) / 2;
+    const int n = (a.F + a.H + a.W) * nch;
+    for (int i = blockIdx.x * blockDim.x + threadIdx.x; i < n; i += gridDim.x * blockDim.x) {
+        const int e = i / nch, c = i - e * nch;
+        const int ax = e < a.F ? 0 : (e < a.F + a.H ? 1 : 2);
+        const int idx = e - (ax == 0 ? 0 : (ax == 1 ? a.F : a.F + a.H));
+        float g;
+        if (a.coords) {
+            const int64_t row = ax == 0 ? (int64_t)idx * a.H * a.W : (ax == 1 ? (int64_t)idx * a.W : (int64_t)idx);
+            g = a.coords[row * 3 + ax] * a.gscale[ax];
+        } else {
+            g = (float)idx * a.gscale[ax];
+        }
+        const int r3 = (4 * c + 3 - rem) % 3, fi = 4 * c - rem + (ax - r3 + 3) % 3;
+        f32x4 o = {1.0f, 0.0f, 1.0f, 0.0f};
+        if (fi >= 0) { const float ang = a.freqs[fi / 3] * (g * 2.0f - 1.0f); o[0] = cosf(ang); o[1] = sinf(ang); }
+        if (ax == r3) { const float ang = a.freqs[(4 * c - rem + 3) / 3] * (g * 2.0f - 1.0f); o[2] = cosf(ang); o[3] = sinf(ang); }
+        *reinterpret_cast<f32x4*>(a.dict + 4 * (int64_t)i) = o;
+    }
+}
+
+__global__ void rope_dict_check_kernel(const unsigned* coords, int B, int S, int F, int H, int W, int* ok) {
+    if ((int64_t)F * H * W != S) { if (blockIdx.x == 0 && threadIdx.x == 0) *ok = 0; return; }
+    const int64_t total = (int64_t)B * S;
+    bool bad = false;
+    for (int64_t row = (int64_t)blockIdx.x * blockDim.x + threadIdx.x; row < total; row += (int64_t)gridDim.x * blockDim.x) {
+        const int s = (int)(row % S);
+        const int w = s % W, t1 = s / W, h = t1 % H, f = t1 / H;
+        bad |= coords[row * 3] != coords[(int64_t)f * H * W * 3] || coords[row * 3 + 1] != coords[(int64_t)h * W * 3 + 1] || coords[row * 3 + 2] != coords[(int64_t)w * 3 + 2];
+    }
+    if (bad) *ok = 0;
 }
 
 __global__ void rope_table_kernel(const RopeTableArgs a) {
@@ -916,10 +985,18 @@
     const int64_t rows_per_block = 4 * (64 / lpr);
     dim3 grid((unsigned)cdiv64(a.rows, rows_per_block)), block(256);
     const bool cached = nch <= NSLOT * lpr;
+    const bool dict = a.dict && a.dict_ok && a.cos && a.sin && a.F > 0 && a.H > 0 && a.W > 0 && a.S > 0 && a.rows < (int64_t)1 << 31 &&
+                      ((int64_t)a.F + a.H + a.W) * nch < (int64_t)1 << 27;
     if (dtype == LTX_DT_BF16) {
         if (a.rows <= 512 && nch > 64 && nch <= 512) hipLaunchKernelGGL((qknorm_rope_block_kernel<bf16_t>), dim3((unsigned)a.rows), block, 0, s, a);
-        else if (nch <= 4 * lpr) hipLaunchKernelGGL((qknorm_rope_fused_kernel<bf16_t, 4>), grid, block, 0, s, a, lpr);
-        else if (nch <= 8 * lpr && ltx_exp("qknorm_fused8", 1)) hipLaunchKernelGGL((qknorm_rope_fused_kernel<bf16_t, 8, 2>), grid, block, 0, s, a, lpr);
+        else if (nch <= 4 * lpr) {
+            if (dict) hipLaunchKernelGGL((qknorm_rope_fused_kernel<bf16_t, 4, 5, true>), grid, block, 0, s, a, lpr);
+            else hipLaunchKernelGGL((qknorm_rope_fused_kernel<bf16_t, 4>), grid, block, 0, s, a, lpr);
+        }
+        else if (nch <= 8 * lpr && ltx_exp("qknorm_fused8", 1)) {
+            if (dict) hipLaunchKernelGGL((qknorm_rope_fused_kernel<bf16_t, 8, 2, true>), grid, block, 0, s, a, lpr);
+            else hipLaunchKernelGGL((qknorm_rope_fused_kernel<bf16_t, 8, 2>), grid, block, 0, s, a, lpr);
+        }
         else if (cached) hipLaunchKernelGGL((qknorm_rope_kernel<bf16_t, true>), grid, block, 0, s, a, lpr);
         else hipLaunchKernelGGL((qknorm_rope_kernel<bf16_t, false>), grid, block, 0, s, a, lpr);
     } else {
@@ -984,6 +1061,29 @@
     return LTX_OK;
 }
 
+size_t ltx_rope_dict_bytes(int F, int H, int W, int D) { return ((size_t)F + H + W) * (size_t)(D / 8) * 4 * sizeof(float); }
+
+int ltx_launch_rope_dict(const RopeDictArgs& a, hipStream_t s) {
+    if (!a.dict || !a.ok || !a.freqs) LTX_FAIL(LTX_ERR_ARG, "rope_dict: null buffer");
+    if (a.D % 8 != 0 || a.D < 8 || a.B < 1 || a.S < 1 || ((uintptr_t)a.dict & 15)) LTX_FAIL(LTX_ERR_ARG, "rope_dict: dim must be a multiple of 8, the dictionary 16-byte aligned, B and S at least 1");
+    const bool raster = a.F > 0 && a.H > 0 && a.W > 0 && (int64_t)a.F * a.H * a.W == a.S;
+    if (!a.coords && !raster) LTX_FAIL(LTX_ERR_ARG, "rope_dict: F*H*W must equal S when coords is absent");
+    if (a.F < 1 || a.H < 1 || a.W < 1) { HIP_TRY(hipMemsetAsync(a.ok, 0, sizeof(int), s)); return LTX_OK; }
+    HIP_TRY(hipMemsetD32Async((hipDeviceptr_t)a.ok, 1, 1, s));
+    if (raster) {
+        const int64_t n = ((int64_t)a.F + a.H + a.W) * (a.D / 8);
+        if (n >= (int64_t)1 << 27) LTX_FAIL(LTX_ERR_ARG, "rope_dict: grid too large");
+        hipLaunchKernelGGL(rope_dict_kernel, dim3((unsigned)(n < 256 * 1024 ? cdiv64(n, 256) : 1024)), dim3(256), 0, s, a);
+    }
+    if (a.coords) {
+        const int64_t rows = (int64_t)a.B * a.S;
+        hipLaunchKernelGGL(rope_dict_check_kernel, dim3((unsigned)(rows < 256 * 1024 ? cdiv64(rows, 256) : 1024)), dim3(256), 0, s,
+                           reinterpret_cast<const unsigned*>(a.coords), a.B, a.S, a.F, a.H, a.W, a.ok);
+    }
+    LTX_CHECK_LAUNCH();
+    return LTX_OK;
+}
+
 int ltx_launch_rope_table(const RopeTableArgs& a, hipStream_t s) {
     if (a.D % 2 != 0 || a.D < 6) LTX_FAIL(LTX_ERR_ARG, "rope: dim must be even and >= 6");
     const int64_t total = (int64_t)a.B * a.F * a.H * a.W * (a.D / 2);
diff --git a/candle-video_amd/ltxhip/__init__.py b/candle-video_amd/ltxhip/__init__.py
--- a/candle-video_amd/ltxhip/__init__.py
+++ b/candle-video_amd/ltxhip/__init__.py
@@ -120,6 +120,8 @@
     "ltx_op_rownorm": [_vp, _vp, _i64, _i, _i, _f, _vp, _vp, _vp, _i64, _i, _i, _i, _vp],
     "ltx_op_qknorm_rope": [_vp, _i64, _i, _i, _vp, _f, _vp, _vp, _i, _vp],
     "ltx_op_rope_table": [_vp, _vp, _vp, _i, _i, _i, _i, _i, _vp, _vp],
+    "ltx_op_rope_dict": [_vp, _vp, _vp, _i, _i, _i, _i, _i, _i, _vp, _vp],
+    "ltx_op_qknorm_rope_dict": [_vp, _i64, _i, _i, _i64, _i, _vp, _vp, _f, _vp, _vp, _f, _vp, _vp, _i, _i, _i, _i, _i, _vp],
     "ltx_op_timestep_embedding": [_vp, _i, _i, _f, _i, _vp, _vp],
     "ltx_op_attention": [_vp, _vp, _vp, _vp, _i, _i, _i, _i, _i, _i, _i, _i, _i, _f, _vp, _i, _vp],
     "ltx_op_attention_prescaled": [_vp, _vp, _vp, _vp, _i, _i, _i, _i, _i, _i, _i, _i, _i, _vp],
@@ -1528,6 +1530,25 @@
         return cos, sin
 
     @staticmethod
+    def rope_dict(B, F, H, W, D, coords=None, rope_scale=None, S=None, device="cuda"):
+        d = torch.empty(F + H + W, D // 8, 4, dtype=torch.float32, device=device)
+        ok = torch.full((1,), -1, dtype=torch.int32, device=device)
+        _check(lib.ltx_op_rope_dict(_ptr(d), _ptr(ok), _ptr(coords), B, F * H * W if S is None else S, F, H, W, D,
+                                    _floats(rope_scale) if rope_scale is not None else None, _stream()))
+        return d, ok
+
+    @staticmethod
+    def qknorm_rope_qk(x, wq, wk, cos, sin, eps=1e-5, out_scale0=1.0, rope_dict=None, dict_ok=None, grid=None, S=None):
+        x = x.clone().contiguous()
+        rows, D2 = x.shape
+        D = D2 // 2
+        F, H, W = grid if grid is not None else (0, 0, 0)
+        _check(lib.ltx_op_qknorm_rope_dict(_ptr(x), C.c_int64(rows), D, D2, C.c_int64(D), 2, _ptr(wq), _ptr(wk), C.c_float(eps), _ptr(cos), _ptr(sin),
+                                           C.c_float(out_scale0), _ptr(rope_dict), _ptr(dict_ok), F, H, W, F * H * W if S is None else S,
+                                           _dt(x.dtype), _stream()))
+        return x
+
+    @staticmethod
     def attention(q, k, v, heads, scale, key_bias=None):
         B, Sq, D = q.shape
         Sk = k.shape[1]
diff --git a/include/ltxhip_ops.h b/include/ltxhip_ops.h
--- a/include/ltxhip_ops.h
+++ b/include/ltxhip_ops.h
@@ -50,6 +50,13 @@
 int ltx_op_rope_table(float* cos, float* sin, const float* coords, int B, int F, int H, int W, int D,
                       const float* rope_scale_host, ltx_stream stream);
 
+int ltx_op_rope_dict(float* dict, int* ok, const float* coords, int B, int S, int F, int H, int W, int D,
+                     const float* rope_scale_host, ltx_stream stream);
+
+int ltx_op_qknorm_rope_dict(void* x, int64_t rows, int D, int ld, int64_t seg_stride, int nseg, const void* w0, const void* w1, float eps,
+                            const float* cos, const float* sin, float out_scale0, const float* dict, const int* dict_ok,
+                            int F, int H, int W, int S, int dtype, ltx_stream stream);
+
 int ltx_op_attention(const void* q, const void* k, const void* v, void* o, int B, int Sq, int Sk, int heads, int hd,
                      int ldq, int ldk, int ldv, int ldo, float scale, const float* key_bias, int dtype, ltx_stream stream);
 int ltx_attention_fallback_counts(unsigned long long counts[2], int reset);
```

Measured after the change: 559.7 frames/sec (median of 6 runs). No clear change (+0.4%).
